# HKUST-Aerial-Robotics/MIND

Hardware: AMD Instinct MI355X
Metric: sim steps/sec (whole node) + scenario-tree nodes expanded/sec, AV2 demo scenes (higher is better)
Workload: dtype f32-class (bf16 hi+mid+lo split operands = 24 significand bits, six products, fp32 accumulate) pair kernel + ActorNet, f32 elsewhere in the predictor, f64 iLQR

## Files before the change

### include/mind_hip.h

```cpp
#ifndef MIND_HIP_H
#define MIND_HIP_H

#include <stddef.h>
#include <stdint.h>

#ifdef __cplusplus
extern "C" {
#endif

#define MIND_OK 0
#define MIND_EINVAL (-1)
#define MIND_ENOMEM (-2)
#define MIND_EHIP (-3)
#define MIND_ESTATE (-4)
#define MIND_ENOTFOUND (-5)

typedef struct mind_ctx mind_ctx;

int mind_ctx_create(int device, void *stream, mind_ctx **out);
int mind_ctx_destroy(mind_ctx *ctx);
const char *mind_last_error_string(mind_ctx *ctx);
int mind_ctx_synchronize(mind_ctx *ctx);

typedef struct {
  const char *name;
  const float *data;
  int64_t numel;
} mind_tensor_desc;

int mind_weights_load(mind_ctx *ctx, const mind_tensor_desc *tensors, int n_tensors);

typedef struct {
  int n_scenes;
  const int32_t *actor_off;
  const int32_t *lane_off;
  const float *actors;
  const float *lanes;
  const float *lane_feat;
  const float *actor_ctrs;
  const float *actor_vecs;
  const float *lane_ctrs;
  const float *lane_vecs;
  const float *const *rpe;
  const float *tgt_nodes;
  const float *tgt_rpe;
} mind_scene_batch;

typedef struct {
  float *cls;
  float *reg;
  float *vel;
  float *lane_feat;
  float *actor_emb;
  float *cls_emb;
} mind_pred_out;

int mind_predict_batch(mind_ctx *ctx, const mind_scene_batch *in, mind_pred_out *out);

typedef struct {
  float *cov_vel;
  float *param;
} mind_pred_aux;
int mind_predict_batch_aux(mind_ctx *ctx, const mind_scene_batch *in, mind_pred_out *out, const mind_pred_aux *aux);

#define MIND_BASIS_BEZIER 0
#define MIND_BASIS_MONOMIAL 1
int mind_set_decoder_basis(mind_ctx *ctx, int basis);
int mind_get_decoder_basis(mind_ctx *ctx);

#define MIND_CURVE_MAX_POINTS (1LL << 26)
int mind_curve_eval(mind_ctx *ctx, int basis, const float *param, long long n_rows, const double *tau, int n_tau,
                    float *reg, float *vel, float *cov_vel);
int mind_debug_curve_basis(int basis, const double *tau, int n_tau, float *T, float *Tp);

int mind_last_fusion_stats(mind_ctx *ctx, int *n_launches, float *total_ms, double *pairs_processed);
int mind_last_actor_stats(mind_ctx *ctx, int *layerwise, int *n_launches, int *n_chunks, float *total_ms);
int mind_last_token_stats(mind_ctx *ctx, int *layerwise, int *n_launches, int *n_chunks, float *total_ms);
int mind_last_token_stage_ms(mind_ctx *ctx, float *out_ms, int cap);
int mind_last_ilqr_stats(mind_ctx *ctx, float *kernel_ms, int *n_trees, int *workgroups_per_tree);
int mind_last_ilqr_profile(mind_ctx *ctx, double *out9);
int mind_last_ilqr_trace(mind_ctx *ctx, int tree, int phase, double *out, int cap_rows, int *n_rows);
int mind_set_profiling(mind_ctx *ctx, int enable);
int mind_debug_launch_times(mind_ctx *ctx, int kind, float *clock_ms, float *event_ms, int cap, int *n_clock, int *n_event);
int mind_debug_launch_clock(int n_blocks, int block_slots, int rate_khz, const long long *ops, int n_ops, const unsigned long long *stamps,
                            long long n_slots, double *out, int cap);

#define MIND_PAIR_F32 0
#define MIND_PAIR_BF16X3 1
#define MIND_PAIR_BF16 2
#define MIND_PAIR_BF16X6 3
int mind_set_pair_precision(mind_ctx *ctx, int mode);

int mind_set_tuning(mind_ctx *ctx, const char *name, int value);
int mind_get_tuning(mind_ctx *ctx, const char *name, int *value);
int mind_debug_tuning(int index, const char *name, const char *text, int value, const char **out_name, const char **out_env, int *out_value);
int mind_debug_live_handles(void);
int mind_get_pair_precision(mind_ctx *ctx);
int mind_debug_pack_bfrag(const float *w, int row_stride, uint32_t *out);

int mind_debug_pair_schedule(const int *scene_tokens, const int *scene_actors, int n_scenes, int n_cu, int last_layer, int *out_jobs, int cap,
                             int *out_info);

int mind_debug_predict_choice(const char *const *knob_names, const int *knob_values, int n_knobs, int pair_prec, int n_cu, int have_side,
                              const int *scene_actors, const int *scene_lanes, int n_scenes, long long *out, int cap);

int mind_debug_ilqr_plan(const char *const *knob_names, const int *knob_values, int n_knobs, int n_cu, int mode, int n_trees, const int *n_nodes,
                         const int32_t *parents, long long *out, int cap, int *bad);

int mind_debug_aime_book(int pred_len, int max_depth, int max_rounds, int n_agents, int world, int rank, int force, int n_rounds, const int *dec_len,
                         const float *dec, int n_tokens, int bytes_per_pair, int plan_chunk_mb, int per_scene, long long *out, int cap, char *msg,
                         int msg_cap);

int mind_debug_wait_word(const unsigned *word, unsigned want, double timeout_s, double (*clock)(void *user), void *user, int spins_per_look);

int mind_debug_actor_lw_plan(int n_actors, int np, int chunk, long long *out_launches, int cap, long long *out_info);

int mind_debug_token_lw_plan(int n_tokens, int mode, int chunk, long long *out_launches, int cap, long long *out_info);

int mind_debug_pack_conv_frag(const float *w, int co, int ci, int ksz, uint32_t *out, size_t cap);

int mind_debug_pack(const char *what, const float *w, int a, int b, int c, float *out, size_t cap);
int mind_debug_weight_image(const mind_tensor_desc *tensors, int n_tensors, float *blob, size_t blob_cap, char *names, size_t names_cap,
                            long long *entries, int entries_cap, long long *out_info, char *msg, int msg_cap);
int mind_debug_weight_bind(const mind_tensor_desc *tensors, int n_tensors, const char *drop, char *msg, int msg_cap);

int mind_debug_trig(mind_ctx *ctx, const double *x, int n, double *out);

int mind_debug_set_layers(mind_ctx *ctx, int n);
int64_t mind_debug_read(mind_ctx *ctx, const char *name, float *host, int64_t max_floats);

typedef struct {
  int n_nodes;
  const int32_t *parent;
  const float *prob;
  int n_agents;
  const float *agent_mean;
  const float *agent_cov;
  const double *field;
  const double *node_w;
} mind_cost_tree;

typedef struct {
  double dt, wheelbase;
  double w_des_state[6];
  double w_state_con[6];
  double state_lower[6], state_upper[6];
  double w_ctrl[2];
  double w_tgt, w_ego, w_ego_cov_offset, w_exo, w_exo_cov_offset, w_exo_cost_offset;
  double grid_res; int grid_w, grid_h;
  int max_iter;
} mind_ilqr_cfg;

typedef struct { int iterations; int converged; double J; double mu; } mind_ilqr_stats;

int mind_ilqr_solve_trees(mind_ctx *ctx, const mind_ilqr_cfg *cfg, const mind_cost_tree *trees,
                          int n_trees, const double *x0, const double *target_lane, int n_lane_pts,
                          double target_vel, int use_exo, const double *us_init, double *xs,
                          double *us, mind_ilqr_stats *stats);

int mind_ilqr_contingency(mind_ctx *ctx, const mind_ilqr_cfg *cfg_warm, const mind_ilqr_cfg *cfg_full,
                          const mind_cost_tree *trees, int n_trees, const double *x0,
                          const double *target_lane, int n_lane_pts, double target_vel, double *xs,
                          double *us, mind_ilqr_stats *stats_warm, mind_ilqr_stats *stats_full);
int mind_ilqr_contingency_begin(mind_ctx *ctx, const mind_ilqr_cfg *cfg_warm, const mind_ilqr_cfg *cfg_full,
                                const mind_cost_tree *trees, int n_trees, const double *x0,
                                const double *target_lane, int n_lane_pts, double target_vel, double *xs,
                                double *us, mind_ilqr_stats *stats_warm, mind_ilqr_stats *stats_full);
int mind_ilqr_contingency_begin_plan(mind_ctx *ctx, const mind_ilqr_cfg *cfg_warm, const mind_ilqr_cfg *cfg_full, const double *x0,
                                     const double *target_lane, int n_lane_pts, double target_vel, double *xs, double *us,
                                     mind_ilqr_stats *stats_warm, mind_ilqr_stats *stats_full);
int mind_ilqr_finish(mind_ctx *ctx);

typedef struct {
  int n_scenes;
  const int32_t *actor_off;
  const float *reg, *vel;
  const float *actor_ctrs, *actor_vecs;
  const float *rot, *orig;
  const float *cov_last;
  const int32_t *last;
  const float *target_lane;
  int n_lane_pts;
  const float *cls;
  const float *scen_prob;
  int lane_check;
  float dist_thres;
} mind_world_in;

typedef struct {
  float *world;
  float *topo;
  float *ego_end;
  float *sel, *sel_prob;
} mind_world_out;

int mind_aime_world(mind_ctx *ctx, const mind_world_in *in, const mind_world_out *out);

int mind_debug_aime_decide(mind_ctx *ctx, int n_scenes, const int32_t *actor_off, const int32_t *cmp, const float *cls, const float *scen_prob,
                           const float *topo, const float *ego_end, const float *world, int lane_check, float dist_thres, float prob_floor,
                           int fused, int by_value, float *sel, float *sel_prob, uint32_t *hit);

typedef struct {
  int n_scenes, n_agents, n_lanes;
  const float *pos, *ang, *vel;
  const float *types;
  const float *pad;
  const float *lane_ctrs, *lane_vecs;
  const float *target_lane;
  const float *target_lane_info;
  int n_lane_pts;
  float time_ahead, min_vel;
  const float *rows_dev;
  const int32_t *parent_slot;
  const int32_t *row0;
  const int32_t *dur;
  int prev_gen;
} mind_rebase_in;

typedef struct {
  float *actors;
  float *actor_ctrs, *actor_vecs;
  float *lane_ctrs, *lane_vecs;
  float *tgt_nodes, *tgt_rpe;
  float *frames;
  int32_t *gen;
} mind_rebase_out;

int mind_aime_rebase(mind_ctx *ctx, const mind_rebase_in *in, const mind_rebase_out *out);

typedef struct {
  int n_agents, n_lanes, n_lane_pts;
  const float *actors;
  const float *actor_ctrs, *actor_vecs;
  const float *lanes;
  const float *lane_ctrs, *lane_vecs;
  const float *tgt_nodes, *tgt_rpe;
  const float *rot, *orig, *tgt_pts;
  const float *hist;
  const float *types;
  const float *target_lane;
  const float *target_lane_info;
  float time_ahead, min_vel, dist_thres;
  int max_depth;
  int max_rounds;
  int pred_len;
  const float *raw_pos, *raw_ang, *raw_vel;
  const float *raw_pad;
  const double *lane_pts;
  const int32_t *lane_flags;
  float travel0;
  const float *script_cls, *script_reg, *script_vel;
  float prob_floor;
  const mind_ilqr_cfg *solve_cfg_warm, *solve_cfg_full;
  const double *solve_x0, *solve_lane;
  int solve_n_lane_pts;
  double solve_target_vel;
} mind_aime_plan_in;

#define MIND_AIME_BRANCH 1
#define MIND_AIME_END 2
#define MIND_AIME_TERMINATE 4
typedef struct {
  int round, scene, mode;
  int parent;
  float prob;
  int cur_t, end_t;
  int flags;
  int dur;
  int64_t row_off;
  float tgt_pts[22];
} mind_aime_node;

typedef struct {
  const mind_aime_node *nodes;
  int n_nodes;
  const float *rows;
  int64_t n_row_floats;
  int n_expanded, n_rounds;
  int root_flags;
// ... 235 lines not shown
```

### mind_amd/_lib.py

```python
import ctypes as C
import os

_HERE = os.path.dirname(os.path.abspath(__file__))
LIB_PATH = os.environ.get("MIND_HIP_LIB", os.path.join(_HERE, "libmind_hip.so"))

WAIT_CLOCK = C.CFUNCTYPE(C.c_double, C.c_void_p)
MIND_OK = 0
MIND_EINVAL, MIND_ENOMEM, MIND_EHIP, MIND_ESTATE, MIND_ENOTFOUND = -1, -2, -3, -4, -5


class TensorDesc(C.Structure):
    _fields_ = [("name", C.c_char_p), ("data", C.POINTER(C.c_float)), ("numel", C.c_int64)]


class SceneBatch(C.Structure):
    _fields_ = [("n_scenes", C.c_int), ("actor_off", C.POINTER(C.c_int32)), ("lane_off", C.POINTER(C.c_int32)),
                ("actors", C.c_void_p), ("lanes", C.c_void_p), ("lane_feat", C.c_void_p),
                ("actor_ctrs", C.c_void_p), ("actor_vecs", C.c_void_p), ("lane_ctrs", C.c_void_p),
                ("lane_vecs", C.c_void_p), ("rpe", C.POINTER(C.c_void_p)), ("tgt_nodes", C.c_void_p),
                ("tgt_rpe", C.c_void_p)]


class PredOut(C.Structure):
    _fields_ = [("cls", C.c_void_p), ("reg", C.c_void_p), ("vel", C.c_void_p), ("lane_feat", C.c_void_p),
# ... 48 lines not shown
class AuditRoadEpisodeOut(C.Structure):
    _fields_ = [("step_margin", C.POINTER(C.c_double)), ("step_corner", C.POINTER(C.c_int32)), ("step_ring", C.POINTER(C.c_int32)),
                ("step_edge", C.POINTER(C.c_int32)), ("ego_min", C.POINTER(C.c_double)), ("ego_step", C.POINTER(C.c_int32)),
                ("ego_corner", C.POINTER(C.c_int32)), ("ego_hits", C.POINTER(C.c_int32)), ("ego_first", C.POINTER(C.c_int32))]


class AuditTtcCfg(C.Structure):
    _fields_ = [("horizon", C.c_double), ("bound", C.c_double), ("lanes", C.c_int)]


class AuditTtcOut(C.Structure):
    _fields_ = [("step_ttc", C.POINTER(C.c_double)), ("step_track", C.POINTER(C.c_int32)), ("ego_min", C.POINTER(C.c_double)),
                ("ego_step", C.POINTER(C.c_int32)), ("ego_track", C.POINTER(C.c_int32)), ("ego_hits", C.POINTER(C.c_int32)),
                ("ego_first", C.POINTER(C.c_int32))]


class ForecastCfg(C.Structure):
    _fields_ = [("K", C.c_int), ("T", C.c_int), ("n_h", C.c_int), ("horizon", C.POINTER(C.c_int32)), ("miss_radius", C.c_double),
                ("disc_scale", C.c_double), ("disc_offset", C.c_double)]


FORECAST_OUT = (("ade", "f8", "a", True), ("fde", "f8", "a", True), ("cover", "i4", "a", True), ("first_out", "i4", "a", True),
                ("n_valid", "i4", "a", False), ("last", "i4", "a", False), ("k_ade", "i4", "a", False), ("k_fde", "i4", "a", False),
                ("brier_fde", "f8", "a", False), ("s_n_scored", "i4", "s", False), ("s_ade", "f8", "s", True), ("s_fde", "f8", "s", True),
                ("s_k_ade", "i4", "s", False), ("s_k_fde", "i4", "s", False), ("s_k_top", "i4", "s", False), ("s_brier_fde", "f8", "s", False),
                ("s_miss_rate", "f8", "s", False), ("s_miss_top", "f8", "s", False))


class ForecastOut(C.Structure):
    _fields_ = [(n, C.POINTER(C.c_double if dt == "f8" else C.c_int32)) for n, dt, _, _ in FORECAST_OUT]


class WorldIn(C.Structure):
    _fields_ = [("n_scenes", C.c_int), ("actor_off", C.POINTER(C.c_int32)), ("reg", C.c_void_p), ("vel", C.c_void_p),
                ("actor_ctrs", C.c_void_p), ("actor_vecs", C.c_void_p), ("rot", C.POINTER(C.c_float)),
                ("orig", C.POINTER(C.c_float)), ("cov_last", C.POINTER(C.c_float)), ("last", C.POINTER(C.c_int32)),
                ("target_lane", C.POINTER(C.c_float)), ("n_lane_pts", C.c_int), ("cls", C.c_void_p),
                ("scen_prob", C.POINTER(C.c_float)), ("lane_check", C.c_int), ("dist_thres", C.c_float)]


class WorldOut(C.Structure):
    _fields_ = [("world", C.c_void_p), ("topo", C.c_void_p), ("ego_end", C.c_void_p), ("sel", C.c_void_p), ("sel_prob", C.c_void_p)]


class RebaseIn(C.Structure):
    _fields_ = [("n_scenes", C.c_int), ("n_agents", C.c_int), ("n_lanes", C.c_int), ("pos", C.POINTER(C.c_float)),
                ("ang", C.POINTER(C.c_float)), ("vel", C.POINTER(C.c_float)), ("types", C.POINTER(C.c_float)),
                ("pad", C.POINTER(C.c_float)), ("lane_ctrs", C.POINTER(C.c_float)), ("lane_vecs", C.POINTER(C.c_float)),
                ("target_lane", C.POINTER(C.c_float)), ("target_lane_info", C.POINTER(C.c_float)), ("n_lane_pts", C.c_int),
                ("time_ahead", C.c_float), ("min_vel", C.c_float), ("rows_dev", C.c_void_p), ("parent_slot", C.POINTER(C.c_int32)),
                ("row0", C.POINTER(C.c_int32)), ("dur", C.POINTER(C.c_int32)), ("prev_gen", C.c_int)]


class RebaseOut(C.Structure):
    _fields_ = [("actors", C.c_void_p), ("actor_ctrs", C.c_void_p), ("actor_vecs", C.c_void_p), ("lane_ctrs", C.c_void_p),
                ("lane_vecs", C.c_void_p), ("tgt_nodes", C.c_void_p), ("tgt_rpe", C.c_void_p), ("frames", C.c_void_p),
                ("gen", C.POINTER(C.c_int32))]


class AimePlanIn(C.Structure):
    _fields_ = [("n_agents", C.c_int), ("n_lanes", C.c_int), ("n_lane_pts", C.c_int)] + \
               [(k, C.POINTER(C.c_float)) for k in ("actors", "actor_ctrs", "actor_vecs", "lanes", "lane_ctrs", "lane_vecs", "tgt_nodes", "tgt_rpe",
                                                    "rot", "orig", "tgt_pts", "hist", "types", "target_lane", "target_lane_info")] + \
               [("time_ahead", C.c_float), ("min_vel", C.c_float), ("dist_thres", C.c_float), ("max_depth", C.c_int), ("max_rounds", C.c_int), ("pred_len", C.c_int),
                ("raw_pos", C.POINTER(C.c_float)), ("raw_ang", C.POINTER(C.c_float)), ("raw_vel", C.POINTER(C.c_float)), ("raw_pad", C.POINTER(C.c_float)),
                ("lane_pts", C.POINTER(C.c_double)), ("lane_flags", C.POINTER(C.c_int32)), ("travel0", C.c_float),
                ("script_cls", C.c_void_p), ("script_reg", C.c_void_p), ("script_vel", C.c_void_p), ("prob_floor", C.c_float),
                ("solve_cfg_warm", C.c_void_p), ("solve_cfg_full", C.c_void_p), ("solve_x0", C.c_void_p), ("solve_lane", C.c_void_p),
                ("solve_n_lane_pts", C.c_int), ("solve_target_vel", C.c_double)]


class AimeNode(C.Structure):
    _fields_ = [("round", C.c_int), ("scene", C.c_int), ("mode", C.c_int), ("parent", C.c_int), ("prob", C.c_float),
                ("cur_t", C.c_int), ("end_t", C.c_int), ("flags", C.c_int), ("dur", C.c_int), ("row_off", C.c_int64),
                ("tgt_pts", C.c_float * 22)]


class AimePlanOut(C.Structure):
    _fields_ = [("nodes", C.POINTER(AimeNode)), ("n_nodes", C.c_int), ("rows", C.POINTER(C.c_float)), ("n_row_floats", C.c_int64),
                ("n_expanded", C.c_int), ("n_rounds", C.c_int), ("root_flags", C.c_int), ("round_scenes", C.c_int * 32),
                ("pair_ms", C.c_float), ("pair_launches", C.c_int), ("n_trees", C.c_int), ("tree_top", C.POINTER(C.c_int32)),
                ("tree_off", C.POINTER(C.c_int32)), ("flat_parent", C.POINTER(C.c_int32)), ("flat_prob", C.POINTER(C.c_float)),
                ("flat_mean", C.POINTER(C.c_float)), ("flat_cov", C.POINTER(C.c_float)), ("solves_begun", C.c_int)]


class IlqrCfg(C.Structure):
    _fields_ = [("dt", C.c_double), ("wheelbase", C.c_double), ("w_des_state", C.c_double * 6),
                ("w_state_con", C.c_double * 6), ("state_lower", C.c_double * 6), ("state_upper", C.c_double * 6),
                ("w_ctrl", C.c_double * 2), ("w_tgt", C.c_double), ("w_ego", C.c_double),
                ("w_ego_cov_offset", C.c_double), ("w_exo", C.c_double), ("w_exo_cov_offset", C.c_double),
                ("w_exo_cost_offset", C.c_double), ("grid_res", C.c_double), ("grid_w", C.c_int), ("grid_h", C.c_int),
                ("max_iter", C.c_int)]


class IlqrStats(C.Structure):
    _fields_ = [("iterations", C.c_int), ("converged", C.c_int), ("J", C.c_double), ("mu", C.c_double)]


LOOP_TAN_FN = C.CFUNCTYPE(C.c_double, C.c_double)
LOOP_SINCOS_FN = C.CFUNCTYPE(None, C.c_double, C.POINTER(C.c_double))


class LoopDesc(C.Structure):
    _fields_ = [("n_tracks", C.c_int), ("n_steps", C.c_int), ("clamp_last", C.c_int), ("ego_state", C.c_void_p), ("ego_state_is_f32", C.c_int), ("ego_obs", C.c_void_p), ("ego_trig32", C.c_void_p),
                ("tan_fn", C.c_void_p), ("sincos_fn", C.c_void_p), ("exo_obs", C.c_void_p),
                ("exo_valid", C.c_void_p), ("timestep", C.c_void_p), ("type_slot", C.c_void_p),
                ("sim_step", C.c_double), ("plan_step", C.c_double), ("enable_time", C.c_double),
                ("wheelbase", C.c_double), ("max_speed", C.c_double), ("max_steer", C.c_double), ("max_acc", C.c_double), ("max_dec", C.c_double),
                ("n_lanes", C.c_int), ("lane_pts", C.c_void_p), ("lane_flags", C.c_void_p),
                ("n_lane_pts", C.c_int), ("target_lane", C.c_void_p), ("target_lane_info", C.c_void_p),
                ("time_ahead", C.c_double), ("min_vel", C.c_float), ("dist_thres", C.c_float), ("max_depth", C.c_int), ("max_rounds", C.c_int),
                ("pred_len", C.c_int), ("prob_floor", C.c_float),
                ("cfg_warm", C.c_void_p), ("cfg_full", C.c_void_p), ("solve_n_lane_pts", C.c_int), ("solve_lane", C.c_void_p), ("target_vel", C.c_double),
                ("eval_n_lane_pts", C.c_int), ("eval_lane_is_f32", C.c_int), ("eval_lane", C.c_void_p), ("speculative", C.c_int)]


class LoopTotals(C.Structure):
    _fields_ = [("plans", C.c_longlong), ("expansions", C.c_longlong), ("scen_trees", C.c_longlong), ("rounds", C.c_longlong),
                ("aime_s", C.c_double), ("ilqr_s", C.c_double), ("total_s", C.c_double),
                ("iterations", C.c_longlong), ("node_iterations", C.c_longlong), ("node_iterations_exo", C.c_longlong),
                ("warm_speculated", C.c_longlong), ("warm_hits", C.c_longlong),
                ("pair_ms", C.c_double), ("pair_launches", C.c_longlong), ("scene_n2", C.c_double), ("scene_n_a1", C.c_double),
                ("ilqr_ms", C.c_double), ("ilqr_launches", C.c_longlong), ("ilqr_trees", C.c_longlong), ("ilqr_workgroups_per_tree", C.c_int),
                ("ilqr_prof", C.c_double * 9), ("ilqr_node_steps", C.c_double)]


class LoopOut(C.Structure):
    _fields_ = [("planned", C.c_int), ("enabled", C.c_int), ("n_steps", C.c_longlong), ("n_plans", C.c_longlong), ("episode_steps", C.c_longlong),
                ("sim_time", C.c_double), ("last_trigger", C.c_double), ("state", C.c_double * 4), ("ctrl", C.c_double * 2),
                ("n_agents", C.c_int), ("n_trees", C.c_int), ("best", C.c_int), ("n_expanded", C.c_int), ("n_rounds", C.c_int), ("n_traj_nodes", C.c_int),
                ("costs", C.POINTER(C.c_double)), ("aime_s", C.c_double), ("ilqr_s", C.c_double), ("total_s", C.c_double),
                ("tot", LoopTotals)]


PLANNER_EGO_KEY = -(1 << 63)


class PlannerDesc(C.Structure):
    _fields_ = [("time_ahead", C.c_double), ("min_vel", C.c_float), ("dist_thres", C.c_float), ("max_depth", C.c_int), ("max_rounds", C.c_int),
                ("pred_len", C.c_int), ("prob_floor", C.c_float), ("cfg_warm", C.c_void_p), ("cfg_full", C.c_void_p), ("speculative", C.c_int),
                ("ego_type_slot", C.c_int)]


class PlannerOut(C.Structure):
    _fields_ = [("n_plans", C.c_longlong),
                ("n_agents", C.c_int), ("n_trees", C.c_int), ("best", C.c_int), ("n_expanded", C.c_int), ("n_rounds", C.c_int), ("n_traj_nodes", C.c_int),
                ("costs", C.POINTER(C.c_double)), ("ctrl", C.c_double * 2), ("aime_s", C.c_double), ("ilqr_s", C.c_double), ("total_s", C.c_double),
                ("tot", LoopTotals)]


EXPORTS = ["mind_ctx_create", "mind_ctx_destroy", "mind_last_error_string", "mind_ctx_synchronize",
           "mind_weights_load", "mind_predict_batch", "mind_last_fusion_stats", "mind_last_actor_stats", "mind_debug_actor_lw_plan", "mind_last_token_stats", "mind_last_token_stage_ms", "mind_debug_token_lw_plan", "mind_set_profiling", "mind_debug_launch_times", "mind_debug_launch_clock",
           "mind_ilqr_solve_trees", "mind_ilqr_contingency", "mind_ilqr_solve_fields", "mind_cost_eval", "mind_ilqr_score_trees", "mind_ilqr_gains", "mind_ilqr_policy_rollouts", "mind_lane_dist_field", "mind_aime_world", "mind_aime_rebase", "mind_debug_aime_decide", "mind_debug_set_layers",
           "mind_debug_read", "mind_set_pair_precision", "mind_get_pair_precision", "mind_debug_pack_bfrag", "mind_debug_pack_conv_frag", "mind_debug_pack", "mind_debug_weight_image", "mind_debug_weight_bind", "mind_debug_pair_schedule", "mind_debug_predict_choice", "mind_debug_ilqr_plan", "mind_debug_aime_book", "mind_set_tuning", "mind_get_tuning", "mind_debug_tuning", "mind_debug_live_handles", "mind_last_ilqr_stats", "mind_aime_plan", "mind_last_ilqr_profile", "mind_eval_traj_trees", "mind_last_ilqr_trace", "mind_ilqr_contingency_begin", "mind_ilqr_finish", "mind_fill_tracks", "mind_ilqr_contingency_begin_plan", "mind_debug_trig", "mind_aime_plan_begin", "mind_aime_plan_poll", "mind_aime_plan_finish", "mind_ctx_busy", "mind_ilqr_finish_plan",
           "mind_set_exchange", "mind_last_exchange_stats", "mind_debug_wait_word",
           "mind_predict_batch_aux", "mind_set_decoder_basis", "mind_get_decoder_basis", "mind_curve_eval", "mind_debug_curve_basis",
           "mind_audit_plan", "mind_audit_episode", "mind_debug_box_clearance",
           "mind_forecast_score", "mind_debug_forecast_score",
           "mind_audit_road_plan", "mind_audit_road_episode", "mind_debug_road_margin",
           "mind_audit_ttc", "mind_debug_box_ttc",
           "mind_loop_create", "mind_loop_destroy", "mind_loop_reset", "mind_loop_advance", "mind_loop_state", "mind_loop_last_plan", "mind_loop_export",
           "mind_planner_create", "mind_planner_destroy", "mind_planner_reset", "mind_planner_observe", "mind_planner_set_lanes", "mind_planner_set_target_lane",
           "mind_planner_set_solve_lane", "mind_planner_set_eval_lane", "mind_planner_plan", "mind_planner_last_plan", "mind_planner_export"]

EXCHANGE_FN = C.CFUNCTYPE(C.c_int, C.c_void_p, C.c_int, C.c_void_p, C.c_void_p, C.c_int64)
XCHG_ALLGATHER, XCHG_ALLREDUCE, XCHG_ALLTOALLV = 0, 1, 2

_lib = None


def load():
    global _lib
    if _lib is not None:
        return _lib
    if not os.path.exists(LIB_PATH):
        raise ImportError(f"{LIB_PATH} is missing: the HIP extension must be built (hipcc --offload-arch=gfx950); "
                          "there is no CPU fallback for the product path")
    lib = C.CDLL(LIB_PATH)
    lib.mind_ctx_create.argtypes = [C.c_int, C.c_void_p, C.POINTER(C.c_void_p)]
    lib.mind_ctx_destroy.argtypes = [C.c_void_p]
    lib.mind_last_error_string.argtypes = [C.c_void_p]
    lib.mind_last_error_string.restype = C.c_char_p
    lib.mind_ctx_synchronize.argtypes = [C.c_void_p]
    lib.mind_weights_load.argtypes = [C.c_void_p, C.POINTER(TensorDesc), C.c_int]
    lib.mind_predict_batch.argtypes = [C.c_void_p, C.POINTER(SceneBatch), C.POINTER(PredOut)]
    lib.mind_predict_batch_aux.argtypes = [C.c_void_p, C.POINTER(SceneBatch), C.POINTER(PredOut), C.POINTER(PredAux)]
    lib.mind_set_decoder_basis.argtypes = [C.c_void_p, C.c_int]
    lib.mind_get_decoder_basis.argtypes = [C.c_void_p]
    lib.mind_curve_eval.argtypes = [C.c_void_p, C.c_int, C.c_void_p, C.c_longlong, C.POINTER(C.c_double), C.c_int, C.c_void_p, C.c_void_p, C.c_void_p]
    lib.mind_debug_curve_basis.argtypes = [C.c_int, C.POINTER(C.c_double), C.c_int, C.POINTER(C.c_float), C.POINTER(C.c_float)]
    lib.mind_last_fusion_stats.argtypes = [C.c_void_p, C.POINTER(C.c_int), C.POINTER(C.c_float), C.POINTER(C.c_double)]
    lib.mind_last_actor_stats.argtypes = [C.c_void_p, C.POINTER(C.c_int), C.POINTER(C.c_int), C.POINTER(C.c_int), C.POINTER(C.c_float)]
    lib.mind_debug_actor_lw_plan.argtypes = [C.c_int, C.c_int, C.c_int, C.POINTER(C.c_longlong), C.c_int, C.POINTER(C.c_longlong)]
    lib.mind_last_token_stats.argtypes = [C.c_void_p, C.POINTER(C.c_int), C.POINTER(C.c_int), C.POINTER(C.c_int), C.POINTER(C.c_float)]
    lib.mind_last_token_stage_ms.argtypes = [C.c_void_p, C.POINTER(C.c_float), C.c_int]
    lib.mind_debug_token_lw_plan.argtypes = [C.c_int, C.c_int, C.c_int, C.POINTER(C.c_longlong), C.c_int, C.POINTER(C.c_longlong)]
    lib.mind_set_profiling.argtypes = [C.c_void_p, C.c_int]
    lib.mind_debug_launch_times.argtypes = [C.c_void_p, C.c_int, C.POINTER(C.c_float), C.POINTER(C.c_float), C.c_int, C.POINTER(C.c_int), C.POINTER(C.c_int)]
    lib.mind_debug_launch_clock.argtypes = [C.c_int, C.c_int, C.c_int, C.POINTER(C.c_longlong), C.c_int, C.POINTER(C.c_ulonglong), C.c_longlong,
                                            C.POINTER(C.c_double), C.c_int]
    lib.mind_ilqr_solve_trees.argtypes = [C.c_void_p, C.POINTER(IlqrCfg), C.POINTER(CostTree), C.c_int,
                                          C.POINTER(C.c_double), C.POINTER(C.c_double), C.c_int, C.c_double, C.c_int,
                                          C.POINTER(C.c_double), C.POINTER(C.c_double), C.POINTER(C.c_double),
                                          C.POINTER(IlqrStats)]
    lib.mind_ilqr_contingency.argtypes = [C.c_void_p, C.POINTER(IlqrCfg), C.POINTER(IlqrCfg), C.POINTER(CostTree), C.c_int,
                                          C.POINTER(C.c_double), C.POINTER(C.c_double), C.c_int, C.c_double,
                                          C.POINTER(C.c_double), C.POINTER(C.c_double), C.POINTER(IlqrStats), C.POINTER(IlqrStats)]
    lib.mind_ilqr_contingency_begin.argtypes = [C.c_void_p, C.POINTER(IlqrCfg), C.POINTER(IlqrCfg), C.POINTER(CostTree), C.c_int,
                                          C.POINTER(C.c_double), C.POINTER(C.c_double), C.c_int, C.c_double,
                                          C.POINTER(C.c_double), C.POINTER(C.c_double), C.POINTER(IlqrStats), C.POINTER(IlqrStats)]
    lib.mind_ilqr_finish.argtypes = [C.c_void_p]
    lib.mind_ilqr_contingency_begin_plan.argtypes = [C.c_void_p, C.POINTER(IlqrCfg), C.POINTER(IlqrCfg), C.c_void_p, C.c_void_p, C.c_int, C.c_double,
                                                     C.c_void_p, C.c_void_p, C.c_void_p, C.c_void_p]
    lib.mind_fill_tracks.argtypes = [C.c_void_p, C.c_int, C.c_int, C.c_void_p, C.c_void_p, C.c_void_p, C.c_void_p, C.c_void_p, C.c_void_p]
    lib.mind_ilqr_solve_fields.argtypes = [C.c_void_p, C.POINTER(IlqrCfg), C.POINTER(FieldGrid), C.POINTER(CostTree), C.c_int,
                                           C.POINTER(C.c_double), C.POINTER(C.c_double), C.POINTER(C.c_double),
                                           C.POINTER(C.c_double), C.POINTER(IlqrStats)]
    lib.mind_cost_eval.argtypes = [C.c_void_p, C.POINTER(IlqrCfg), C.POINTER(FieldGrid), C.POINTER(CostTree),
                                   C.POINTER(C.c_double), C.POINTER(C.c_double), C.c_int, C.c_double, C.c_int, C.c_int,
                                   C.POINTER(C.c_int32), C.POINTER(C.c_double), C.POINTER(C.c_double), C.POINTER(C.c_double)]
    lib.mind_ilqr_score_trees.argtypes = [C.c_void_p, C.POINTER(IlqrCfg), C.POINTER(FieldGrid), C.POINTER(CostTree), C.c_int,
                                          C.POINTER(C.c_double), C.POINTER(C.c_double), C.c_int, C.c_double, C.c_int, C.c_int,
                                          C.POINTER(C.c_double), C.POINTER(C.c_double), C.POINTER(C.c_double), C.POINTER(C.c_double)]
    lib.mind_ilqr_gains.argtypes = [C.c_void_p, C.POINTER(IlqrCfg), C.POINTER(FieldGrid), C.POINTER(CostTree), C.c_int,
                                    C.POINTER(C.c_double), C.POINTER(C.c_double), C.c_int, C.c_double, C.c_int,
                                    C.POINTER(C.c_double), C.POINTER(C.c_double), C.POINTER(IlqrGainsOut)]
    lib.mind_ilqr_policy_rollouts.argtypes = [C.c_void_p, C.POINTER(IlqrCfg), C.POINTER(FieldGrid), C.POINTER(CostTree), C.c_int,
                                              C.POINTER(C.c_double), C.POINTER(C.c_double), C.c_int, C.c_double, C.c_int,
                                              C.POINTER(C.c_double), C.POINTER(C.c_double), C.POINTER(C.c_double), C.c_int,
                                              C.POINTER(C.c_double), C.POINTER(C.c_double), C.POINTER(C.c_double), C.POINTER(C.c_double),
                                              C.POINTER(C.c_double), C.POINTER(C.c_double)]
    lib.mind_lane_dist_field.argtypes = [C.c_void_p, C.POINTER(C.c_double), C.POINTER(C.c_double), C.c_int, C.c_int, C.c_int,
                                         C.c_double] + [C.POINTER(C.c_double)] * 4
    lib.mind_aime_world.argtypes = [C.c_void_p, C.POINTER(WorldIn), C.POINTER(WorldOut)]
    lib.mind_aime_rebase.argtypes = [C.c_void_p, C.POINTER(RebaseIn), C.POINTER(RebaseOut)]
    lib.mind_debug_aime_decide.argtypes = [C.c_void_p, C.c_int, C.POINTER(C.c_int32), C.POINTER(C.c_int32), C.c_void_p, C.POINTER(C.c_float), C.c_void_p,
                                           C.c_void_p, C.c_void_p, C.c_int, C.c_float, C.c_float, C.c_int, C.c_int, C.c_void_p, C.c_void_p, C.c_void_p]
    lib.mind_aime_plan.argtypes = [C.c_void_p, C.POINTER(AimePlanIn), C.POINTER(AimePlanOut)]
    lib.mind_aime_plan_begin.argtypes = [C.c_void_p, C.POINTER(AimePlanIn)]
    lib.mind_aime_plan_poll.argtypes = [C.c_void_p]
    lib.mind_aime_plan_finish.argtypes = [C.c_void_p, C.POINTER(AimePlanOut)]
    lib.mind_ctx_busy.argtypes = [C.c_void_p]
    lib.mind_ilqr_finish_plan.argtypes = [C.c_void_p, C.c_int, C.c_int, C.c_void_p, C.c_void_p, C.c_void_p, C.c_void_p]
    lib.mind_set_pair_precision.argtypes = [C.c_void_p, C.c_int]
    lib.mind_set_tuning.argtypes = [C.c_void_p, C.c_char_p, C.c_int]
    lib.mind_get_tuning.argtypes = [C.c_void_p, C.c_char_p, C.POINTER(C.c_int)]
    lib.mind_debug_tuning.argtypes = [C.c_int, C.c_char_p, C.c_char_p, C.c_int, C.POINTER(C.c_char_p), C.POINTER(C.c_char_p), C.POINTER(C.c_int)]
    lib.mind_debug_live_handles.argtypes = []
    lib.mind_last_ilqr_stats.argtypes = [C.c_void_p, C.POINTER(C.c_float), C.POINTER(C.c_int), C.POINTER(C.c_int)]
    lib.mind_last_ilqr_profile.argtypes = [C.c_void_p, C.POINTER(C.c_double)]
    lib.mind_last_ilqr_trace.argtypes = [C.c_void_p, C.c_int, C.c_int, C.POINTER(C.c_double), C.c_int, C.POINTER(C.c_int)]
    lib.mind_eval_traj_trees.argtypes = [C.POINTER(C.c_double), C.POINTER(C.c_double), C.POINTER(C.c_int32), C.c_int, C.c_void_p, C.c_int, C.c_int,
                                         C.c_double, C.POINTER(C.c_double)]
    lib.mind_get_pair_precision.argtypes = [C.c_void_p]
    lib.mind_debug_pack_bfrag.argtypes = [C.POINTER(C.c_float), C.c_int, C.POINTER(C.c_uint32)]
    lib.mind_debug_pair_schedule.argtypes = [C.POINTER(C.c_int), C.POINTER(C.c_int), C.c_int, C.c_int, C.c_int, C.POINTER(C.c_int), C.c_int, C.POINTER(C.c_int)]
    lib.mind_debug_predict_choice.argtypes = [C.POINTER(C.c_char_p), C.POINTER(C.c_int), C.c_int, C.c_int, C.c_int, C.c_int, C.POINTER(C.c_int), C.POINTER(C.c_int),
                                              C.c_int, C.POINTER(C.c_longlong), C.c_int]
    lib.mind_debug_ilqr_plan.argtypes = [C.POINTER(C.c_char_p), C.POINTER(C.c_int), C.c_int, C.c_int, C.c_int, C.c_int, C.POINTER(C.c_int), C.POINTER(C.c_int32),
                                         C.POINTER(C.c_longlong), C.c_int, C.POINTER(C.c_int)]
    lib.mind_debug_wait_word.argtypes = [C.POINTER(C.c_uint), C.c_uint, C.c_double, WAIT_CLOCK, C.c_void_p, C.c_int]
    lib.mind_debug_aime_book.argtypes = [C.c_int] * 8 + [C.POINTER(C.c_int), C.POINTER(C.c_float)] + [C.c_int] * 4 + [C.POINTER(C.c_longlong), C.c_int, C.c_char_p, C.c_int]
    lib.mind_debug_trig.argtypes = [C.c_void_p, C.POINTER(C.c_double), C.c_int, C.POINTER(C.c_double)]
    lib.mind_debug_pack_conv_frag.argtypes = [C.POINTER(C.c_float), C.c_int, C.c_int, C.c_int, C.POINTER(C.c_uint32), C.c_size_t]
    lib.mind_debug_pack.argtypes = [C.c_char_p, C.POINTER(C.c_float), C.c_int, C.c_int, C.c_int, C.POINTER(C.c_float), C.c_size_t]
    lib.mind_debug_weight_image.argtypes = [C.POINTER(TensorDesc), C.c_int, C.POINTER(C.c_float), C.c_size_t, C.c_char_p, C.c_size_t,
                                            C.POINTER(C.c_longlong), C.c_int, C.POINTER(C.c_longlong), C.c_char_p, C.c_int]
    lib.mind_debug_weight_bind.argtypes = [C.POINTER(TensorDesc), C.c_int, C.c_char_p, C.c_char_p, C.c_int]
    lib.mind_debug_set_layers.argtypes = [C.c_void_p, C.c_int]
    lib.mind_debug_read.argtypes = [C.c_void_p, C.c_char_p, C.POINTER(C.c_float), C.c_int64]
    lib.mind_set_exchange.argtypes = [C.c_void_p, C.c_int, C.c_int, EXCHANGE_FN, C.c_void_p, C.c_int]
    lib.mind_last_exchange_stats.argtypes = [C.c_void_p, C.POINTER(C.c_longlong), C.POINTER(C.c_longlong)]
    lib.mind_loop_create.argtypes = [C.c_void_p, C.POINTER(LoopDesc), C.POINTER(C.c_void_p)]
    lib.mind_loop_destroy.argtypes = [C.c_void_p]
    lib.mind_loop_reset.argtypes = [C.c_void_p]
    lib.mind_loop_advance.argtypes = [C.c_void_p, C.c_int, C.c_double, C.c_longlong, C.POINTER(LoopOut)]
    lib.mind_loop_state.argtypes = [C.c_void_p, C.POINTER(LoopOut)]
    lib.mind_loop_last_plan.argtypes = [C.c_void_p, C.POINTER(AimePlanOut)] + [C.POINTER(C.c_void_p)] * 6 + [C.c_void_p]
    lib.mind_loop_export.argtypes = [C.c_void_p, C.c_int, C.POINTER(C.c_int), C.c_void_p, C.c_void_p, C.c_void_p]
    lib.mind_planner_create.argtypes = [C.c_void_p, C.POINTER(PlannerDesc), C.POINTER(C.c_void_p)]
    lib.mind_planner_destroy.argtypes = [C.c_void_p]
    lib.mind_planner_reset.argtypes = [C.c_void_p]
    lib.mind_planner_observe.argtypes = [C.c_void_p, C.c_int, C.c_void_p, C.c_int, C.c_void_p, C.c_void_p, C.c_void_p]
    lib.mind_planner_set_lanes.argtypes = [C.c_void_p, C.c_int, C.c_void_p, C.c_void_p]
    lib.mind_planner_set_target_lane.argtypes = [C.c_void_p, C.c_int, C.c_void_p, C.c_void_p]
    lib.mind_planner_set_solve_lane.argtypes = [C.c_void_p, C.c_int, C.c_void_p, C.c_double]
    lib.mind_planner_set_eval_lane.argtypes = [C.c_void_p, C.c_int, C.c_void_p, C.c_int]
    lib.mind_planner_plan.argtypes = [C.c_void_p, C.c_void_p, C.c_void_p, C.POINTER(PlannerOut)]
    lib.mind_planner_last_plan.argtypes = [C.c_void_p, C.POINTER(AimePlanOut)] + [C.POINTER(C.c_void_p)] * 6 + [C.c_void_p]
    lib.mind_planner_export.argtypes = [C.c_void_p, C.c_int, C.POINTER(C.c_int), C.c_void_p, C.c_void_p, C.c_void_p]
    lib.mind_audit_plan.argtypes = [C.c_void_p, C.POINTER(AuditBox), C.c_double, C.POINTER(CostTree), C.c_int, C.c_int, C.POINTER(C.c_double),
                                    C.POINTER(AuditPlanOut)]
    lib.mind_audit_episode.argtypes = [C.c_void_p, C.POINTER(AuditBox), C.c_int, C.c_int, C.c_int, C.POINTER(C.c_double), C.POINTER(C.c_double),
                                       C.POINTER(C.c_uint8), C.POINTER(C.c_double), C.POINTER(AuditEpisodeOut)]
    lib.mind_debug_box_clearance.argtypes = [C.c_int, C.c_int, C.POINTER(C.c_double), C.POINTER(C.c_double), C.POINTER(C.c_double), C.POINTER(C.c_double)]
    fc_tail = [C.POINTER(ForecastCfg), C.c_int, C.POINTER(C.c_int32), C.c_void_p, C.c_void_p, C.POINTER(C.c_double), C.POINTER(C.c_uint8),
               C.POINTER(C.c_uint8), C.POINTER(ForecastOut)]
    lib.mind_forecast_score.argtypes = [C.c_void_p] + fc_tail
    lib.mind_debug_forecast_score.argtypes = fc_tail
    road = [C.POINTER(C.c_double), C.POINTER(C.c_int32), C.c_int]
    lib.mind_audit_road_plan.argtypes = [C.c_void_p, C.POINTER(AuditBox)] + road + [C.POINTER(CostTree), C.c_int, C.c_int, C.POINTER(C.c_double),
                                                                                   C.POINTER(AuditRoadPlanOut)]
    lib.mind_audit_road_episode.argtypes = [C.c_void_p, C.POINTER(AuditBox)] + road + [C.c_int, C.c_int, C.POINTER(C.c_double),
                                                                                      C.POINTER(AuditRoadEpisodeOut)]
    lib.mind_debug_road_margin.argtypes = [C.c_int, C.POINTER(C.c_double), C.POINTER(AuditBox)] + road + [C.POINTER(C.c_double), C.POINTER(C.c_double)] + \
        [C.POINTER(C.c_int32)] * 3
    lib.mind_audit_ttc.argtypes = [C.c_void_p, C.POINTER(AuditBox), C.POINTER(AuditTtcCfg), C.c_int, C.c_int, C.c_int, C.POINTER(C.c_double),
                                   C.POINTER(C.c_double), C.POINTER(C.c_uint8), C.POINTER(C.c_double), C.POINTER(AuditTtcOut)]
    lib.mind_debug_box_ttc.argtypes = [C.c_int, C.POINTER(C.c_double), C.POINTER(C.c_double), C.POINTER(C.c_double), C.POINTER(C.c_double)]
    for n in EXPORTS:
        getattr(lib, n)
        if n not in ("mind_last_error_string", "mind_debug_read"):
            getattr(lib, n).restype = C.c_int
    lib.mind_debug_read.restype = C.c_int64
    _lib = lib
    return lib


PRED_CHOICE_FIELDS = ("header", "n_runs", "np", "actor_form", "actor_arg", "actor_grid", "actor_chunk", "actor_chunks", "actor_launches", "qsplit", "qk_stride",
                      "tiled", "edge_bf16", "edge_pair_bytes", "tok_chunk", "tok_lw", "tok_chunks", "pair_family", "pair_np", "l5_jobs5", "xcd_lanes",
                      "xcd_lanes5", "dec_actor", "dec_np", "fp32_dec", "split_dec", "want_mw", "mw_blocks", "cls_on_side", "tgt_wait_first",
                      "dec_head_ra")
PAIR_PREC = ("f32", "bf16x3", "bf16", "bf16x6")


def predict_choice(knobs, prec, scenes, n_cu=256, have_side=True):
    lib = load()
    names = (C.c_char_p * max(1, len(knobs)))(*[k.encode() for k in knobs])
    vals = (C.c_int * max(1, len(knobs)))(*[int(v) for v in knobs.values()])
    sa = (C.c_int * len(scenes))(*[a for a, _ in scenes])
    sl = (C.c_int * len(scenes))(*[l for _, l in scenes])
    cap = 32 + 6 * len(scenes)
    out = (C.c_longlong * cap)()
    n = lib.mind_debug_predict_choice(names, vals, len(knobs), PAIR_PREC.index(prec) if isinstance(prec, str) else prec, n_cu, int(have_side),
                                      sa, sl, len(scenes), out, cap)
    if n == MIND_EINVAL:
        return None
    assert 0 < n <= cap and out[0] == 32 and n == 32 + 6 * out[1], n
    d = dict(zip(PRED_CHOICE_FIELDS, out[:31]))
    d["runs"] = [tuple(out[32 + 6 * i:38 + 6 * i]) for i in range(out[1])]
    return d


def knobs():
    lib = load()
    name, env, val = C.c_char_p(), C.c_char_p(), C.c_int()
    rows = []
    while not rows or len(rows) < n:
        n = lib.mind_debug_tuning(len(rows), None, None, 0, C.byref(name), C.byref(env), C.byref(val))
        assert n > 0, n
        rows.append((name.value.decode(), env.value.decode() if env.value else None, val.value))
    return rows


def knob_stored(name, value=None, text=None):
    val = C.c_int()
    rc = load().mind_debug_tuning(-1, name.encode(), None if text is None else text.encode(), 0 if value is None else int(value), None, None, C.byref(val))
    return val.value if rc == MIND_OK else None


ILQR_PLAN_FIELDS = ("header", "n_trees", "form", "G", "GS", "spec", "nslot", "grid", "workgroups_per_tree", "host_out", "early", "starve_followers")
ILQR_TREE_FIELDS = ("M", "nl", "nseg", "nsl", "maxls", "nfs")
ILQR_TREE_TABLES = ("level_start", "level_nodes", "child_start", "child_list", "seg_start", "seg_nodes", "slevel_start", "slevel_segs", "seg_rec",
                    "fstep_start", "fstep_items", "fstep_q1", "fstep_nstart", "fstep_nodes")


def ilqr_plan(knobs, parents, n_cu=256, generic=False, evaluate=False, two_fits=False):
    lib = load()
    names = (C.c_char_p * max(1, len(knobs)))(*[k.encode() for k in knobs])
    vals = (C.c_int * max(1, len(knobs)))(*[int(v) for v in knobs.values()])
    nn = (C.c_int * len(parents))(*[len(p) for p in parents])
    flat = [int(v) for p in parents for v in p]
    par = (C.c_int32 * max(1, len(flat)))(*flat)
    bad = (C.c_int * 2)()
    mode = int(generic) | int(evaluate) << 1 | int(two_fits) << 2
    n = lib.mind_debug_ilqr_plan(names, vals, len(knobs), n_cu, mode, len(parents), nn, par, None, 0, bad)
    if n == MIND_EINVAL:
        return {"bad": (bad[0], bad[1])} if bad[0] >= 0 else None
    out = (C.c_longlong * n)()
    assert lib.mind_debug_ilqr_plan(names, vals, len(knobs), n_cu, mode, len(parents), nn, par, out, n, bad) == n and out[0] == 16
    d = dict(zip(ILQR_PLAN_FIELDS, out[:12]))
    d["trees"], o = [], 16
    for _ in parents:
        tr = dict(zip(ILQR_TREE_FIELDS, out[o:o + 6]))
        lens, o = out[o + 6:o + 20], o + 20
        for name, ln in zip(ILQR_TREE_TABLES, lens):
            tr[name], o = list(out[o:o + ln]), o + ln
        d["trees"].append(tr)
    assert o == n
    return d


AIME_ROUND_FIELDS = ("B", "lo", "hi", "Bmax", "chunk", "S", "s0", "Sm", "any")
AIME_NODE_FIELDS = ("round", "scene", "mode", "parent", "prob", "cur_t", "end_t", "flags", "dur", "row_off", "owner", "lscene")


def aime_book(pred_len, max_depth, n_agents, rounds, world=1, rank=0, force=False, max_rounds=32, n_tokens=0, bytes_per_pair=512, plan_chunk_mb=96 * 1024,
              per_scene=1):
    import numpy as np
    lib = load()
    arrs = [np.ascontiguousarray(r, np.float32).ravel() for r in rounds]
    lens = (C.c_int * max(1, len(arrs)))(*[a.size for a in arrs])
    dec = np.concatenate(arrs + [np.zeros(1, np.float32)])
    msg = C.create_string_buffer(256)
    args = [pred_len, max_depth, max_rounds, n_agents, world, rank, int(force), len(arrs), lens, dec.ctypes.data_as(C.POINTER(C.c_float)), n_tokens,
            bytes_per_pair, plan_chunk_mb, per_scene]
    n = lib.mind_debug_aime_book(*args, None, 0, msg, 256)
    if n == MIND_EINVAL:
        return None
    out = (C.c_longlong * n)()
    assert lib.mind_debug_aime_book(*args, out, n, msg, 256) == n and out[0] == 16
    o, take = [16], lambda k: (list(out[o[0]:o[0] + k]), o.__setitem__(0, o[0] + k))[0]
    d = dict(code=out[1], error=msg.value.decode() if out[1] else None, args=(out[2], out[3]), n_rows=out[8], root_flags=out[9], rounds=[])
    for _ in range(out[4]):
        r = dict(zip(AIME_ROUND_FIELDS, take(9)))
        for k, ln in (("todo", r["S"]), ("cnt_r", world), ("s0_r", world + 1), ("win", 3 * r["Sm"]), ("tab", 2 * world), ("snd", 2 * world), ("rcv", 2 * world)):
            r[k] = take(ln)
        d["rounds"].append(r)
    if not out[1]:
        d["nodes"] = [dict(zip(AIME_NODE_FIELDS, take(12))) for _ in range(out[5])]
        for name in ("gather", "flat"):
            nj, nb, nbytes = take(3)
            d[name] = dict(jobs=[tuple(take(5)) for _ in range(nj)], job_of_block=take(nb), agent_of_block=take(nb), bytes=nbytes)
        d["tree_top"], d["tree_off"], d["flat_parent"], d["flat_prob"] = take(out[6]), take(out[6] + 1), take(out[7]), take(out[7])
    assert o[0] == n
    return d


def tensor_descs(sd):
    import numpy as np
    descs = (TensorDesc * max(1, len(sd)))()
    keep = []
    for i, (k, v) in enumerate(sd.items()):
        a = np.ascontiguousarray(v.detach().cpu().numpy() if hasattr(v, "detach") else np.asarray(v), dtype=np.float32)
        keep.append(a)
        descs[i].name = k.encode()
        descs[i].data = a.ctypes.data_as(C.POINTER(C.c_float))
        descs[i].numel = a.size
    return descs, keep


def weight_image(sd):
    import numpy as np
    lib = load()
    descs, keep = tensor_descs(sd)
    msg = C.create_string_buffer(256)
    info = (C.c_longlong * 3)()
    rc = lib.mind_debug_weight_image(descs, len(sd), None, 0, None, 0, None, 0, info, msg, 256)
    if rc == MIND_ENOTFOUND:
        raise KeyError(msg.value.decode())
    assert rc == MIND_OK, rc
    ne, nf, nb = info
    blob, names, ents = np.zeros(nf, np.float32), C.create_string_buffer(nb), (C.c_longlong * (2 * ne))()
    assert lib.mind_debug_weight_image(descs, len(sd), blob.ctypes.data_as(C.POINTER(C.c_float)), nf, names, nb, ents, ne, info, msg, 256) == MIND_OK
    keys = names.value.decode().split("\n")[:-1]
    assert len(keys) == ne
    return blob, [(k, ents[2 * i], ents[2 * i + 1]) for i, k in enumerate(keys)]


def curve_basis(basis, tau):
    import numpy as np
    lib = load()
    tau = np.ascontiguousarray(tau, np.float64).ravel()
    b = BASIS.index(basis) if isinstance(basis, str) else int(basis)
    T, Tp = np.zeros((max(1, tau.size), 8), np.float32), np.zeros((max(1, tau.size), 7), np.float32)
    rc = lib.mind_debug_curve_basis(b, tau.ctypes.data_as(C.POINTER(C.c_double)), tau.size, T.ctypes.data_as(C.POINTER(C.c_float)),
                                    Tp.ctypes.data_as(C.POINTER(C.c_float)))
    if rc == MIND_EINVAL:
        raise ValueError(f"mind_debug_curve_basis rejects basis {basis!r}, tau {tau!r}")
    assert rc == MIND_OK, rc
    return T[:tau.size], Tp[:tau.size]


def weight_bind(sd, drop=None):
    lib = load()
    descs, keep = tensor_descs(sd)
    msg = C.create_string_buffer(256)
    rc = lib.mind_debug_weight_bind(descs, len(sd), drop.encode() if drop else None, msg, 256)
    assert rc in (MIND_OK, MIND_ENOTFOUND), rc
    return None if rc == MIND_OK else msg.value.decode()


def pack(what, w, a=0, b=0, c=0, cap=1 << 20):
    import numpy as np
    lib = load()
    w = np.ascontiguousarray(w, np.float32)
    out = np.zeros(cap, np.float32)
    n = lib.mind_debug_pack(what.encode(), w.ctypes.data_as(C.POINTER(C.c_float)), a, b, c, out.ctypes.data_as(C.POINTER(C.c_float)), cap)
    assert n > 0, (what, n)
    return out[:n].copy()


def box_clearance(kind, a, b, trig=None):
    import numpy as np
# ... 139 lines not shown
```

### mind_amd/csrc/encdec_kernels.hip

```cpp
#include <hip/hip_runtime.h>
#include <stdint.h>

#include "weight_tables.h"
#include "dec_curve.h"
#include "launch_clock.h"

typedef float f32x4 __attribute__((ext_vector_type(4)));

#define NT 256

__device__ __forceinline__ float wave_sum(float v) {
  v += __shfl_xor(v, 32, 64);
  v += __shfl_xor(v, 16, 64);
  v += __shfl_xor(v, 8, 64);
  v += __shfl_xor(v, 4, 64);
  v += __shfl_xor(v, 2, 64);
  v += __shfl_xor(v, 1, 64);
  return v;
}

__device__ __forceinline__ float block_sum(float v, float *red) {
  v = wave_sum(v);
  __syncthreads();
  if ((threadIdx.x & 63) == 0) red[threadIdx.x >> 6] = v;
  __syncthreads();
  return red[0] + red[1] + red[2] + red[3];
}

#ifndef DB
#define DB 16
#endif
#define DENSE_ROW_FENCE() __builtin_amdgcn_sched_barrier(0)
#define DBQ 8
template <int R>
__device__ __forceinline__ void dense_quads(const float *in, int ldi, int K, const float *__restrict__ WT,
                                            const float *__restrict__ b, int NOUT, float *out, int ldo,
                                            float *part, int part_floats) {
  const int nthr = blockDim.x;
  const int NQ = NOUT >> 2;
  int KP = 1;
  while (KP * 2 * NQ <= nthr && KP * 2 * R * NOUT <= part_floats && KP * 2 <= (K >> 2)) KP *= 2;
  const int Kc = ((K / 4 + KP - 1) / KP) * 4;
  for (int item = threadIdx.x; item < KP * NQ; item += nthr) {
    const int kp = item / NQ, o = (item % NQ) * 4;
    float acc[R][4];
#pragma unroll
    for (int r = 0; r < R; ++r)
#pragma unroll
      for (int c = 0; c < 4; ++c) acc[r][c] = (KP == 1 && b) ? b[o + c] : 0.f;
    const int k0 = kp * Kc, k1 = min(K, k0 + Kc);
    int k = k0;
    for (; k + DBQ <= k1; k += DBQ) {
      f32x4 w[DBQ];
#pragma unroll
      for (int q = 0; q < DBQ; ++q) w[q] = *(const f32x4 *)(WT + (size_t)(k + q) * NOUT + o);
#pragma unroll
      for (int r = 0; r < R; ++r) {
#pragma unroll
        for (int q4 = 0; q4 < DBQ / 4; ++q4) {
          const f32x4 x = *(const f32x4 *)(in + r * ldi + k + 4 * q4);
#pragma unroll
          for (int j = 0; j < 4; ++j)
#pragma unroll
            for (int c = 0; c < 4; ++c) acc[r][c] = fmaf(w[4 * q4 + j][c], x[j], acc[r][c]);
        }
        DENSE_ROW_FENCE();
      }
    }
    for (; k < k1; k += 4) {
#pragma unroll
      for (int j = 0; j < 4; ++j) {
        const f32x4 w = *(const f32x4 *)(WT + (size_t)(k + j) * NOUT + o);
#pragma unroll
        for (int r = 0; r < R; ++r) {
          const float x = in[r * ldi + k + j];
#pragma unroll
          for (int c = 0; c < 4; ++c) acc[r][c] = fmaf(w[c], x, acc[r][c]);
        }
      }
    }
#pragma unroll
    for (int r = 0; r < R; ++r)
#pragma unroll
      for (int c = 0; c < 4; ++c) {
        if (KP == 1) out[r * ldo + o + c] = acc[r][c];
        else part[(kp * R + r) * NOUT + o + c] = acc[r][c];
      }
  }
  if (KP == 1) return;
  __syncthreads();
  for (int i = threadIdx.x; i < R * NOUT; i += nthr) {
    const int r = i / NOUT, oo = i % NOUT;
    float v = b ? b[oo] : 0.f;
    for (int q = 0; q < KP; ++q) v += part[(q * R + r) * NOUT + oo];
    out[r * ldo + oo] = v;
  }
}

#ifndef DT
#define DT 1024
#endif
template <int R>
__device__ __forceinline__ void dense_quads_part(const float *in, int ldi, int K, const float *__restrict__ WT, const float *__restrict__ b, int NOUT,
                                                 float *out, int ldo, float *part, int part_floats, int wg, int G) {
  const int nthr = blockDim.x;
  const int NQ = NOUT >> 2;
  int KP = 1;
  while (KP * 2 * NQ <= DT && KP * 2 * R * NOUT <= part_floats && KP * 2 <= (K >> 2)) KP *= 2;
  const int Kc = ((K / 4 + KP - 1) / KP) * 4;
  const int q_lo = NQ * wg / G, q_hi = NQ * (wg + 1) / G, NQg = q_hi - q_lo;
  for (int item = threadIdx.x; item < KP * NQg; item += nthr) {
    const int kp = item / NQg, o = (q_lo + item % NQg) * 4;
    float acc[R][4];
#pragma unroll
    for (int r = 0; r < R; ++r)
#pragma unroll
      for (int c = 0; c < 4; ++c) acc[r][c] = (KP == 1 && b) ? b[o + c] : 0.f;
    const int k0 = kp * Kc, k1 = min(K, k0 + Kc);
    int k = k0;
    for (; k + DBQ <= k1; k += DBQ) {
      f32x4 w[DBQ];
#pragma unroll
      for (int q = 0; q < DBQ; ++q) w[q] = *(const f32x4 *)(WT + (size_t)(k + q) * NOUT + o);
#pragma unroll
      for (int r = 0; r < R; ++r) {
#pragma unroll
        for (int q4 = 0; q4 < DBQ / 4; ++q4) {
          const f32x4 x = *(const f32x4 *)(in + r * ldi + k + 4 * q4);
#pragma unroll
          for (int j = 0; j < 4; ++j)
#pragma unroll
            for (int c = 0; c < 4; ++c) acc[r][c] = fmaf(w[4 * q4 + j][c], x[j], acc[r][c]);
        }
        DENSE_ROW_FENCE();
      }
    }
    for (; k < k1; k += 4) {
#pragma unroll
      for (int j = 0; j < 4; ++j) {
        const f32x4 w = *(const f32x4 *)(WT + (size_t)(k + j) * NOUT + o);
#pragma unroll
        for (int r = 0; r < R; ++r) {
          const float x = in[r * ldi + k + j];
#pragma unroll
          for (int c = 0; c < 4; ++c) acc[r][c] = fmaf(w[c], x, acc[r][c]);
        }
      }
    }
#pragma unroll
    for (int r = 0; r < R; ++r)
#pragma unroll
      for (int c = 0; c < 4; ++c) {
        if (KP == 1) out[r * ldo + o + c] = acc[r][c];
        else part[(kp * R + r) * NOUT + o + c] = acc[r][c];
      }
  }
  if (KP == 1) return;
  __syncthreads();
// ... 404 lines not shown
__device__ __forceinline__ float block_sum_a(float v, float *red, int flip) {
  v = wave_sum(v);
  float *r = red + (flip & 1) * 16;
  if ((threadIdx.x & 63) == 0) r[threadIdx.x >> 6] = v;
  __syncthreads();
  float s = 0.f;
#pragma unroll
  for (int w = 0; w < AT / 64; ++w) s += r[w];
  return s;
}

#define GN_NE 6
__device__ __forceinline__ void gn(float *buf, int C, int T, const float *__restrict__ g,
                                   const float *__restrict__ b, const float *resid, bool relu, float *red) {
  const int n = C * T;
  float x[GN_NE], gg[GN_NE], bb[GN_NE];
  float s = 0.f;
#pragma unroll
  for (int e = 0; e < GN_NE; ++e) {
    const int i = threadIdx.x + e * AT;
    if (i < n) {
      const int c = i / T;
      x[e] = buf[i];
      gg[e] = g[c];
      bb[e] = b[c];
      s += x[e];
    }
  }
  const float mean = block_sum_a(s, red, 0) / (float)n;
  float v = 0.f;
#pragma unroll
  for (int e = 0; e < GN_NE; ++e)
    if ((int)threadIdx.x + e * AT < n) { const float d = x[e] - mean; v = fmaf(d, d, v); }
  const float rstd = 1.0f / sqrtf(block_sum_a(v, red, 1) / (float)n + 1e-5f);
#pragma unroll
  for (int e = 0; e < GN_NE; ++e) {
    const int i = threadIdx.x + e * AT;
    if (i < n) {
      float y = (x[e] - mean) * rstd * gg[e] + bb[e];
      if (resid) y += resid[i];
      if (relu) y = fmaxf(y, 0.f);
      buf[i] = y;
    }
  }
  __syncthreads();
}

__device__ __forceinline__ void res1d(const float *in, int Cin, int Tin, const ResW &w, int Cout, int stride,
                                      float *out, float *t1, float *t2, float *red, float *part, int pf) {
  const int Tout = Tin / stride;
  if (stride == 1) conv<1, 3>(in, Cin, Tin, w.c1, Cout, Tout, t1, part, pf);
  else conv<2, 3>(in, Cin, Tin, w.c1, Cout, Tout, t1, part, pf);
  __syncthreads();
  gn(t1, Cout, Tout, w.g1, w.b1, nullptr, true, red);
  conv<1, 3>(t1, Cout, Tout, w.c2, Cout, Tout, out, part, pf);
  __syncthreads();
  const float *resid = in;
  if (w.ds) {
    if (stride == 1) conv<1, 1>(in, Cin, Tin, w.ds, Cout, Tout, t2, part, pf);
    else conv<2, 1>(in, Cin, Tin, w.ds, Cout, Tout, t2, part, pf);
    __syncthreads();
      gn(t2, Cout, Tout, w.gd, w.bd, nullptr, false, red);
      resid = t2;
  }
  gn(out, Cout, Tout, w.g2, w.b2, resid, true, red);
}

#define ACT_PART 12288
#define ACT_LDS_FLOATS (672 + 7 * 1536 + 2 * 6144 + 32 + ACT_PART)
__global__ __launch_bounds__(AT) void k_actor_net(const float *__restrict__ actors, int n_actors,
                                                  float *__restrict__ out, ActorW W, LcSlot *clk) {
  lc_stamp_in(clk);
  extern __shared__ float sm[];
  float *xin = sm;
  float *o0 = sm + 672, *o1 = o0 + 1536, *o2 = o1 + 1536, *o3 = o2 + 1536;
  float *ta = o3 + 1536, *tb = ta + 1536, *tc = tb + 1536;
  float *fa = tc + 1536, *fb = fa + 6144;
  float *red = fb + 6144;
  float *part = red + 32;
  const int pf = ACT_PART;
  float *fo = o0;
  const int tid = threadIdx.x;
  const int a = blockIdx.x;
  if (a >= n_actors) { lc_stamp_both(clk); return; }
#ifdef MIND_ENC_TRACE
  long long at_[12], aq_ = clock64();
  int an_ = 0;
#define AT_MARK() do { const long long n_ = clock64(); at_[an_++] = n_ - aq_; aq_ = n_; } while (0)
#else
#define AT_MARK() do {} while (0)
#endif
  for (int i = tid; i < 14 * 48; i += AT) xin[i] = actors[(size_t)a * 14 * 48 + i];
  __syncthreads();
  AT_MARK();
  res1d(xin, 14, 48, W.res[0], 32, 1, ta, tb, tc, red, part, pf);
  res1d(ta, 32, 48, W.res[1], 32, 1, o0, tb, tc, red, part, pf);
  AT_MARK();
  res1d(o0, 32, 48, W.res[2], 64, 2, ta, tb, tc, red, part, pf);
  res1d(ta, 64, 24, W.res[3], 64, 1, o1, tb, tc, red, part, pf);
  AT_MARK();
  res1d(o1, 64, 24, W.res[4], 128, 2, ta, tb, tc, red, part, pf);
  res1d(ta, 128, 12, W.res[5], 128, 1, o2, tb, tc, red, part, pf);
  AT_MARK();
  res1d(o2, 128, 12, W.res[6], 256, 2, ta, tb, tc, red, part, pf);
  res1d(ta, 256, 6, W.res[7], 256, 1, o3, tb, tc, red, part, pf);
  AT_MARK();
  conv<1, 3>(o3, 256, 6, W.latW[3], 128, 6, fa, part, pf);
  __syncthreads();
  gn(fa, 128, 6, W.latG[3], W.latB[3], nullptr, false, red);
  float *cur = fa, *nxt = fb;
  for (int g = 2; g >= 0; --g) {
    const float *src_o = g == 2 ? o2 : (g == 1 ? o1 : o0);
    const int C = g == 2 ? 128 : (g == 1 ? 64 : 32);
    const int T = g == 2 ? 12 : (g == 1 ? 24 : 48);
    const int Th = T / 2;
    conv<1, 3>(src_o, C, T, W.latW[g], 128, T, nxt, part, pf);
    __syncthreads();
    gn(nxt, 128, T, W.latG[g], W.latB[g], nullptr, false, red);
    for (int i = tid; i < 128 * T; i += AT) {
      const int c = i / T, t = i % T;
      float src = (t + 0.5f) * 0.5f - 0.5f;
      src = src < 0.f ? 0.f : src;
      const int i0 = (int)src;
      const int i1 = i0 + 1 < Th ? i0 + 1 : Th - 1;
      const float l1 = src - (float)i0;
      nxt[i] += (1.0f - l1) * cur[c * Th + i0] + l1 * cur[c * Th + i1];
    }
    __syncthreads();
    float *t = cur; cur = nxt; nxt = t;
  }
  AT_MARK();
  {
    const ResW &w = W.res[8];
    conv<1, 3>(cur, 128, 48, w.c1, 128, 48, nxt, part, pf);
    __syncthreads();
    gn(nxt, 128, 48, w.g1, w.b1, nullptr, true, red);
    conv<1, 3>(nxt, 128, 48, w.c2, 128, 48, fo, part, pf);
    __syncthreads();
    gn(fo, 128, 48, w.g2, w.b2, cur, true, red);
  }
  AT_MARK();
  if (tid < 128) out[(size_t)a * 128 + tid] = fo[tid * 48 + 47];
#ifdef MIND_ENC_TRACE
  if (a == 0 && tid == 0)
    printf("[k_actor_net n=%d] cycles: load %lld group0 %lld group1 %lld group2 %lld group3 %lld fpn %lld out-res %lld\n", n_actors, at_[0], at_[1], at_[2],
           at_[3], at_[4], at_[5], at_[6]);
#endif
  lc_stamp_out(clk);
}
extern "C" size_t mind_actor_lds_bytes() { return (size_t)ACT_LDS_FLOATS * sizeof(float); }

#define DEC_SCENE_PART 24576
#define DEC_SCENE_LDS_FLOATS (256 + 768 + 768 + 2304 + 768 + 9216 + 768 + 144 + DEC_SCENE_PART)
__global__ __launch_bounds__(DT) void k_dec_tgt(const float *__restrict__ tgt_feat , const float *__restrict__ tgt_rpe ,
                                                float *__restrict__ tgt_out , DecW W) {
  extern __shared__ __attribute__((aligned(16))) float dsm[];
  float (*v0)[256] = (float (*)[256])(dsm);
  float (*v1)[768] = (float (*)[768])(dsm + 256);
  float *part = dsm + 14992;
  const int PF = DEC_SCENE_PART;
  const int tid = threadIdx.x;
  const int b = blockIdx.x;
  if (tid < 20) v1[0][tid] = tgt_rpe[(size_t)b * 20 + tid];
  __syncthreads();
  dense<1>(&v1[0][0], 768, 20, W.rpeW, W.rpeb, 128, &v0[0][128], 256, part, PF);
  if (tid < 128) v0[0][tid] = tgt_feat[(size_t)b * 128 + tid];
  __syncthreads();
  ln_rows(&v0[0][128], 256, 1, 128, W.rpeg, W.rpebe, true);
  __syncthreads();
  dense<1>(&v0[0][0], 256, 256, W.t0W, W.t0b, 128, &v1[0][0], 768, part, PF);
  __syncthreads();
  ln_rows(&v1[0][0], 768, 1, 128, W.t0g, W.t0be, true);
  __syncthreads();
  dense<1>(&v1[0][0], 768, 128, W.t3W, W.t3b, 128, &v0[0][0], 256, part, PF);
  __syncthreads();
  ln_rows(&v0[0][0], 256, 1, 128, W.t3g, W.t3be, true);
  __syncthreads();
  if (tid < 128) tgt_out[(size_t)b * 128 + tid] = v0[0][tid];
}

#ifdef MIND_DEC_TRACE
__device__ long long dec_tr_[64];
__device__ int dec_trn_;
#define DEC_MARK() do { if (blockIdx.x == 0 && threadIdx.x == 0) { dec_tr_[dec_trn_ & 63] = clock64(); ++dec_trn_; } } while (0)
#else
#define DEC_MARK() do {} while (0)
#endif
template <bool MW, int PART = 0>
__device__ __forceinline__ void k_dec_scene_body(const float *__restrict__ x ,
                                                 const int *__restrict__ cls_row ,
                                                 float *__restrict__ Cout ,
                                                 float *__restrict__ cls_out , const DecW &W, int b, int wg, int G,
                                                 float *xbuf, unsigned *bar, unsigned *abort_word) {
  extern __shared__ __attribute__((aligned(16))) float dsm[];
  float (*v0)[256] = (float (*)[256])(dsm);
  float (*v1)[768] = (float (*)[768])(dsm + 256);
  float (*C)[128] = (float (*)[128])(dsm + 1024);
  float (*qkv)[384] = (float (*)[384])(dsm + 1792);
  float (*att)[128] = (float (*)[128])(dsm + 4096);
  float (*ff)[1536] = (float (*)[1536])(dsm + 4864);
  float (*t2)[128] = (float (*)[128])(dsm + 14080);
  float (*sc)[6][6] = (float (*)[6][6])(dsm + 14848);
  float *part = dsm + 14992;
  const int PF = DEC_SCENE_PART;
  const int tid = threadIdx.x;
  int xstage = 0;
  float *xb0 = xbuf, *xb1 = xbuf + 6 * 1536;
#ifdef MIND_DEC_TRACE
  if (blockIdx.x == 0 && tid == 0) dec_trn_ = 0;
#endif
  DEC_MARK();
  if (PART == 2) {
    for (int i = tid; i < 768; i += blockDim.x) C[i / 128][i % 128] = Cout[(size_t)b * 768 + i];
    __syncthreads();
  }
  if (PART != 2) {
  if (tid < 128) v0[0][tid] = x[(size_t)cls_row[b] * 128 + tid];
  __syncthreads();
  dense<1>(&v0[0][0], 256, 128, W.c0W, W.c0b, 384, &v1[0][0], 768, part, PF);
  DEC_MARK();
  __syncthreads();
  ln_rows(&v1[0][0], 768, 1, 384, W.c0g, W.c0be, true);
  DEC_MARK();
  __syncthreads();
  if (MW) {
    dense_quads_part<1>(&v1[0][0], 768, 384, W.c3W, W.c3b, 768, &ff[0][0], 1536, part, PF, wg, G);
    if (dec_exchange<1>(&ff[0][0], 1536, 768, wg, G, (xstage++ & 1) ? xb1 : xb0, bar, abort_word)) return;
  } else
    dense<1>(&v1[0][0], 768, 384, W.c3W, W.c3b, 768, &ff[0][0], 1536, part, PF);
  DEC_MARK();
  __syncthreads();
  ln_rows(&ff[0][0], 1536, 1, 768, W.c3g, W.c3be, true);
  DEC_MARK();
  __syncthreads();
  for (int i = tid; i < 768; i += blockDim.x) C[i / 128][i % 128] = ff[0][i];
  __syncthreads();
  for (int L = 0; L < 2; ++L) {
    dense<6>(&C[0][0], 128, 128, W.inW[L], W.inb[L], 384, &qkv[0][0], 384, part, PF);
  DEC_MARK();
    __syncthreads();
    if (tid < 4 * 36) {
      const int hd = tid / 36, s = (tid % 36) / 6, t = tid % 6;
      float d = 0.f;
      for (int k = 0; k < 32; ++k) d = fmaf(qkv[s][hd * 32 + k], qkv[t][128 + hd * 32 + k], d);
      sc[hd][s][t] = d / sqrtf(32.0f);
    }
    __syncthreads();
    if (tid < 24) {
      const int hd = tid / 6, s = tid % 6;
      float m = -INFINITY;
      for (int t = 0; t < 6; ++t) m = fmaxf(m, sc[hd][s][t]);
      float e[6], sum = 0.f;
      for (int t = 0; t < 6; ++t) { e[t] = expf(sc[hd][s][t] - m); sum += e[t]; }
      for (int t = 0; t < 6; ++t) sc[hd][s][t] = e[t] / sum;
    }
    __syncthreads();
    for (int i = tid; i < 6 * 128; i += blockDim.x) {
      const int s = i / 128, c = i % 128, hd = c / 32;
      float o = 0.f;
      for (int t = 0; t < 6; ++t) o = fmaf(sc[hd][s][t], qkv[t][256 + c], o);
      att[s][c] = o;
    }
    __syncthreads();
    dense<6>(&att[0][0], 128, 128, W.outW[L], W.outb[L], 128, &t2[0][0], 128, part, PF);
  DEC_MARK();
    __syncthreads();
    for (int i = tid; i < 768; i += blockDim.x) C[i / 128][i % 128] += t2[i / 128][i % 128];
    __syncthreads();
    ln_rows(&C[0][0], 128, 6, 128, W.n1g[L], W.n1b[L], false);
  DEC_MARK();
    __syncthreads();
    if (MW) {
      dense_quads_part<6>(&C[0][0], 128, 128, W.l1W[L], W.l1b[L], 1536, &ff[0][0], 1536, part, PF, wg, G);
      if (dec_exchange<6>(&ff[0][0], 1536, 1536, wg, G, (xstage++ & 1) ? xb1 : xb0, bar, abort_word)) return;
    } else
      dense<6>(&C[0][0], 128, 128, W.l1W[L], W.l1b[L], 1536, &ff[0][0], 1536, part, PF);
  DEC_MARK();
    __syncthreads();
    for (int i = tid; i < 6 * 1536; i += blockDim.x) ff[i / 1536][i % 1536] = fmaxf(ff[i / 1536][i % 1536], 0.f);
    __syncthreads();
    if (MW) {
      dense_quads_part<6>(&ff[0][0], 1536, 1536, W.l2W[L], W.l2b[L], 128, &t2[0][0], 128, part, PF, wg, G);
      if (dec_exchange<6>(&t2[0][0], 128, 128, wg, G, (xstage++ & 1) ? xb1 : xb0, bar, abort_word)) return;
    } else
      dense<6>(&ff[0][0], 1536, 1536, W.l2W[L], W.l2b[L], 128, &t2[0][0], 128, part, PF);
  DEC_MARK();
    __syncthreads();
    for (int i = tid; i < 768; i += blockDim.x) C[i / 128][i % 128] += t2[i / 128][i % 128];
    __syncthreads();
    ln_rows(&C[0][0], 128, 6, 128, W.n2g[L], W.n2b[L], false);
  DEC_MARK();
    __syncthreads();
  }
  if (!MW || wg == 0)
    for (int i = tid; i < 768; i += blockDim.x) Cout[(size_t)b * 768 + i] = C[i / 128][i % 128];
  }
  if (PART == 1) return;
  dense<6>(&C[0][0], 128, 128, W.k0W, W.k0b, 128, &att[0][0], 128, part, PF);
  DEC_MARK();
  __syncthreads();
  ln_rows(&att[0][0], 128, 6, 128, W.k0g, W.k0be, true);
  DEC_MARK();
  __syncthreads();
  dense<6>(&att[0][0], 128, 128, W.k3W, W.k3b, 128, &t2[0][0], 128, part, PF);
  DEC_MARK();
  __syncthreads();
  ln_rows(&t2[0][0], 128, 6, 128, W.k3g, W.k3be, true);
  DEC_MARK();
  __syncthreads();
  for (int k = tid >> 6; k < 6; k += (int)(blockDim.x >> 6)) {
    const int lane = tid & 63;
    float s = t2[k][lane] * W.k6W[lane] + t2[k][lane + 64] * W.k6W[lane + 64];
    s = wave_sum(s);
    if (lane == 0) sc[0][0][k] = s + W.k6b[0];
  }
  __syncthreads();
  if (tid == 0 && (!MW || wg == 0)) {
    float m = -INFINITY;
    for (int k = 0; k < 6; ++k) m = fmaxf(m, sc[0][0][k]);
    float e[6], sum = 0.f;
    for (int k = 0; k < 6; ++k) { e[k] = expf(sc[0][0][k] - m); sum += e[k]; }
    for (int k = 0; k < 6; ++k) cls_out[(size_t)b * 6 + k] = e[k] / sum;
  }
  DEC_MARK();
#ifdef MIND_DEC_TRACE
  if (blockIdx.x == 0 && tid == 0) {
    printf("[k_dec_scene] cycles between marks (dense / LayerNorm stages in program order):");
    for (int q = 1; q < dec_trn_ && q < 64; ++q) printf(" %lld", dec_tr_[q] - dec_tr_[q - 1]);
    printf("\n");
  }
#endif
}

__global__ __launch_bounds__(DT) void k_dec_scene(const float *__restrict__ x, const int *__restrict__ cls_row, float *__restrict__ Cout,
                                                  float *__restrict__ cls_out, DecW W) {
  k_dec_scene_body<false>(x, cls_row, Cout, cls_out, W, (int)blockIdx.x, 0, 1, nullptr, nullptr, nullptr);
}
__global__ __launch_bounds__(DT) void k_dec_scene_c(const float *__restrict__ x, const int *__restrict__ cls_row, float *__restrict__ Cout, DecW W) {
  k_dec_scene_body<false, 1>(x, cls_row, Cout, nullptr, W, (int)blockIdx.x, 0, 1, nullptr, nullptr, nullptr);
}
__global__ __launch_bounds__(DT) void k_dec_cls(float *__restrict__ Cout, float *__restrict__ cls_out, DecW W) {
  k_dec_scene_body<false, 2>(nullptr, nullptr, Cout, cls_out, W, (int)blockIdx.x, 0, 1, nullptr, nullptr, nullptr);
}
#define DEC_MW_G 8
__global__ __launch_bounds__(DT) void k_dec_scene_mw(const float *__restrict__ x, const int *__restrict__ cls_row, float *__restrict__ Cout,
                                                     float *__restrict__ cls_out, DecW W, int n_scenes, float *__restrict__ xbuf,
                                                     unsigned *__restrict__ bars, unsigned *abort_word) {
  const int r = (int)blockIdx.x % (8 * DEC_MW_G);
  const int b = 8 * ((int)blockIdx.x / (8 * DEC_MW_G)) + (r & 7), wg = r >> 3;
  if (b >= n_scenes) return;
  k_dec_scene_body<true>(x, cls_row, Cout, cls_out, W, b, wg, DEC_MW_G, xbuf + (size_t)b * 2 * 6 * 1536, bars + 4 * (size_t)b, abort_word);
}

#define RA 4
#define DEC_ACTOR_LDS_FLOATS (512 + 1536 + 3072 + 3072 + 3072 + 960 + 6144)
template <int PART, int RAT = RA>
__global__ __launch_bounds__(DT) void k_dec_actor(const float *__restrict__ x ,
                                                  const int *__restrict__ actor_row ,
                                                  const int *__restrict__ actor_scene , int n_actors,
                                                  const float *__restrict__ Cmode ,
                                                  const float *__restrict__ tgt ,
                                                  float *__restrict__ reg, float *__restrict__ vel, DecW W, float *__restrict__ h2g,
                                                  float *__restrict__ cov_vel , float *__restrict__ param ) {
  extern __shared__ __attribute__((aligned(16))) float dsm[];
  float (*xin)[128] = (float (*)[128])(dsm);
  float (*h1)[384] = (float (*)[384])(dsm + 512);
  float (*h2)[768] = (float (*)[768])(dsm + 2048);
  float (*E)[128] = (float (*)[128])(dsm + 5120);
  float (*t1)[128] = (float (*)[128])(dsm + 8192);
  float (*prm)[40] = (float (*)[40])(dsm + 11264);
  float *part = dsm + 12224;
  const int PF = 6144;
  static_assert(RAT == RA || (PART == 2 && (RAT == 1 || RAT == 2)), "only the head runs with fewer agents per workgroup");
  constexpr int HEAD_KP = dense_scalar_kp(RA * 6, 128, 128, DT, 6144);
  const int tid = threadIdx.x;
  const int a0 = blockIdx.x * RAT;
  if (PART != 2) {
    for (int i = tid; i < RAT * 128; i += blockDim.x) {
      const int r = i / 128, a = a0 + r;
      xin[r][i % 128] = a < n_actors ? x[(size_t)actor_row[a] * 128 + i % 128] : 0.f;
    }
    __syncthreads();
    dense<RAT>(&xin[0][0], 128, 128, W.a0W, W.a0b, 384, &h1[0][0], 384, part, PF);
    __syncthreads();
    ln_rows(&h1[0][0], 384, RAT, 384, W.a0g, W.a0be, true);
    __syncthreads();
    dense<RAT>(&h1[0][0], 384, 384, W.a3W, W.a3b, 768, &h2[0][0], 768, part, PF);
    __syncthreads();
    ln_rows(&h2[0][0], 768, RAT, 768, W.a3g, W.a3be, true);
    __syncthreads();
    if (PART == 1) {
      for (int i = tid; i < RAT * 768; i += blockDim.x) {
        const int r = i / 768, a = a0 + r;
        if (a < n_actors) h2g[(size_t)a * 768 + i % 768] = h2[r][i % 768];
      }
      return;
    }
  } else {
    for (int i = tid; i < RAT * 768; i += blockDim.x) {
      const int r = i / 768, a = a0 + r;
      h2[r][i % 768] = a < n_actors ? h2g[(size_t)a * 768 + i % 768] : 0.f;
    }
    __syncthreads();
  }
  for (int i = tid; i < RAT * 768; i += blockDim.x) {
    const int r = i / 768, k = (i % 768) / 128, c = i % 128;
    const int a = a0 + r;
    float v = 0.f;
    if (a < n_actors) {
      const int sc = actor_scene[a];
      v = h2[r][k * 128 + c] + Cmode[((size_t)sc * 6 + k) * 128 + c];
      if (k == 0) v += tgt[(size_t)sc * 128 + c];
    }
    E[r * 6 + k][c] = v;
  }
  __syncthreads();
  if (RAT == RA) dense<RA * 6>(&E[0][0], 128, 128, W.r0W, W.r0b, 128, &t1[0][0], 128, part, PF);
  else dense_ksplit<RAT * 6, RAT + 1>(&E[0][0], 128, 128, W.r0W, W.r0b, 128, &t1[0][0], 128, part, HEAD_KP);
  __syncthreads();
  ln_rows(&t1[0][0], 128, RAT * 6, 128, W.r0g, W.r0be, true);
  __syncthreads();
  if (RAT == RA) dense<RA * 6>(&t1[0][0], 128, 128, W.r3W, W.r3b, 128, &E[0][0], 128, part, PF);
  else dense_ksplit<RAT * 6, RAT + 1>(&t1[0][0], 128, 128, W.r3W, W.r3b, 128, &E[0][0], 128, part, HEAD_KP);
  __syncthreads();
  ln_rows(&E[0][0], 128, RAT * 6, 128, W.r3g, W.r3be, true);
  __syncthreads();
  for (int i = tid; i < RAT * 6 * 40; i += blockDim.x) {
    const int r = i / 40, o = i % 40;
    float acc = W.r6b[o];
    for (int k = 0; k < 128; ++k) acc = fmaf(W.r6W[k * 40 + o], E[r][k], acc);
    prm[r][o] = acc;
  }
  __syncthreads();
  if (param)
    for (int i = tid; i < RAT * 6 * 40; i += blockDim.x) {
      const int r = i / 40, a = a0 + r / 6;
      if (a < n_actors) param[((size_t)a * 6 + r % 6) * 40 + i % 40] = prm[r][i % 40];
    }
  for (int i = tid; i < RAT * 6 * 60; i += blockDim.x) {
    const int r = i / 60, t = i % 60;
    const int a = a0 + r / 6, k = r % 6;
    if (a >= n_actors) continue;
    const size_t o = ((size_t)a * 6 + k) * 60 + t;
    dec_curve_point(&prm[r][0], W.T + t * 8, W.Tp + t * 7, W.monomial, reg + o * 5, vel + o * 2, cov_vel ? cov_vel + o * 3 : nullptr);
  }
}

extern "C" size_t mind_dec_scene_lds_bytes() { return (size_t)DEC_SCENE_LDS_FLOATS * sizeof(float); }
extern "C" size_t mind_dec_actor_lds_bytes() { return (size_t)DEC_ACTOR_LDS_FLOATS * sizeof(float); }
```

### mind_amd/csrc/mind_hip.hip

```cpp
#include <hip/hip_runtime.h>

#include <cmath>
#include <cstdarg>
#include <cstdio>
#include <cstdlib>
#include <algorithm>
#include <cstring>
#include <map>
#include <memory>
#include <string>
#include <thread>
#include <atomic>
#include <functional>
#include <vector>

#include "../../include/mind_hip.h"
#include "encdec_kernels.hip"
#include "fusion_kernels.hip"
#include "pair_bf16_kernels.hip"
#include "pair_tile_kernels.hip"
#include "pair_tile6_kernels.hip"
#include "token_mfma_kernels.hip"
#include "actor_mfma_kernels.hip"
#include "actor_lw_kernels.hip"
#include "token_lw_kernels.hip"
#include "actor_f32_kernels.hip"
#include "dec_mfma_kernels.hip"
#include "dec_curve_kernels.hip"
#include "ilqr_kernels.hip"
#include "ilqr_score_kernels.hip"
#include "ilqr_policy_kernels.hip"
#include "audit_kernels.hip"
#include "forecast_kernels.hip"
#include "road_kernels.hip"
#include "ttc_kernels.hip"
#include "pair_jobs.h"
#include "pred_choice.h"
#include "ilqr_choice.h"
#include "aime_book.h"
#include "audit_arena.h"
#include "weight_pack.h"
#include "aime_kernels.hip"

static_assert(TN_RA == RA && TN_IL_SLOTS == IL_SLOTS, "tuning.h restates the two kernel constants its clamps need");

static std::atomic<long> live_handles{0};

template <class H, hipError_t (*Release)(H)> struct Owned {
  H p = nullptr;
  size_t cap = 0;
  Owned() = default;
  Owned(Owned &&o) noexcept : p(o.p), cap(o.cap) { o.p = nullptr; o.cap = 0; }
  Owned &operator=(Owned &&o) noexcept { if (this != &o) { reset(); p = o.p; cap = o.cap; o.p = nullptr; o.cap = 0; } return *this; }
  ~Owned() { reset(); }
  operator H() const { return p; }
  template <class T> T *as() const { return (T *)p; }
  void reset() {
    if (p) { (void)Release(p); live_handles.fetch_sub(1, std::memory_order_relaxed); }
    p = nullptr; cap = 0;
  }
  hipError_t took(hipError_t e, size_t bytes = 0) {
    if (e == hipSuccess) { live_handles.fetch_add(1, std::memory_order_relaxed); cap = bytes; } else p = nullptr;
    return e;
  }
};
struct Event : Owned<hipEvent_t, hipEventDestroy> { hipError_t create(unsigned flags = hipEventDefault) { reset(); return took(hipEventCreateWithFlags(&p, flags)); } };
struct Stream : Owned<hipStream_t, hipStreamDestroy> { hipError_t create() { reset(); return took(hipStreamCreateWithFlags(&p, hipStreamNonBlocking)); } };
struct Pinned : Owned<void *, hipHostFree> {
  hipError_t alloc(size_t bytes, unsigned flags = hipHostMallocDefault) { reset(); return took(hipHostMalloc(&p, bytes, flags), bytes); }
};
struct DevBuf : Owned<void *, hipFree> {
  hipError_t alloc(size_t bytes) { reset(); return took(hipMalloc(&p, bytes), bytes); }
};

struct TableSet {
  std::vector<int> key;
  DevBuf meta, jobs, jobs5, rows;
  std::vector<int> actor_row, cls_row, scene_n;
  long long edge_pairs = 0, edge_pairs_t = 0, stamp = 0;
  int ntok = 0, slot = 0, njobs = 0, njobs5 = 0;
  double pairs_full = 0, pairs_l5 = 0;
};
#define MIND_TABLE_SETS 8

struct mind_ctx {
  int device = 0;
  hipStream_t stream = nullptr;
  Stream side;
  Event ev_side, ev_main, ev_stage, ev_tgt, ev_cls;
  std::vector<char> aime_stage;
  bool aime_stage_busy = false;
  std::string err;
  DevBuf wdev;
  bool have_weights = false;
  WeightTables W = {};
  PredTuning pt; IlqrTuning it; CtxTuning ct;
  TnRefs knobs() { return {&pt, &it, &ct}; }
  int dec_basis = MIND_BASIS_BEZIER;
  DevBuf curve_tab;
  std::vector<double> curve_tau;
  int curve_tab_basis = -1;
  DevBuf tok_lw_arena;
  std::vector<TlLaunch> tok_lw_plan;
  int last_tok_lw = 0, last_tok_launches = 0, last_tok_chunks = 0;
  float tok_ms = 0.f, tok_stage_ms[TL_NSTAGE + 1] = {};
  std::vector<Event> ev_tok;
  std::vector<int> ev_tok_tag;
  TableSet tabs[MIND_TABLE_SETS];
  long long tab_clock = 0;
  long long n_table_hits = 0;
  unsigned dec_gen = 0;
  DevBuf pl_cnt;
  std::function<int(hipStream_t)> enc_pre, enc_post;
  std::vector<IlTables> il_tab;
  struct IlImage { std::vector<double> hD; std::vector<float> hF; std::vector<int> hI; } il_img;
  struct IlEarly { const double *xs = nullptr, *us = nullptr; volatile unsigned *done = nullptr; unsigned gen = 0; int n_trees = 0; long nodes = 0; } il_early;
  unsigned il_gen = 0;
  long long il_spec_req = 0, il_spec_hit = 0;
  DevBuf actor_lw_arena;
  std::vector<LwLaunch> actor_lw_plan;
  int last_actor_lw = 0, last_actor_launches = 0, last_actor_chunks = 0;
  float actor_ms = 0.f;
  Event ev_act0, ev_act1;
  int pair_prec = 3;
  std::vector<int> last_scene_n;
  bool last_edge_tiled = false, last_edge_bf16 = false;
  DevBuf edge, x, ST, QK, part, tokpos, meta, jobs, actor_feat, lane_feat, tgt_feat, cmode, tgt_emb,
      rows, rpe_ptrs;
  DevBuf ilqr_dev, aime_dev, rebase_dev2[2], dec_h2;
  DevBuf audit_dev;
  DevBuf pl_root, pl_in[2], pl_lf, pl_lrep, pl_pred, pl_small, pl_tab[2], pl_win[2];
  std::vector<DevBuf> pl_world;
  Pinned pl_pin[8];
  Event ev_pl, ev_tab, ev_root;
  DevBuf il_field;
  Pinned il_field_pin;
  Event ev_field;
  bool il_field_valid = false;
  double il_field_key[5] = {0, 0, 0, 0, 0};
  std::vector<double> il_field_lane;
  int xr = 0, xw = 1;
  mind_exchange_fn xfn = nullptr;
  void *xuser = nullptr;
  bool xforce = false;
  DevBuf x_send, x_recv, x_seg;
  long long x_collectives = 0, x_bytes = 0;
  Stream pl_copy;
  std::vector<double> pl_sol_xs, pl_sol_us;
  std::vector<mind_ilqr_stats> pl_sol_stw, pl_sol_stf;
  std::thread pa_thread;
  std::atomic<int> pa_state{0};
  mind_aime_plan_in pa_in;
  mind_aime_plan_out pa_out;
  int pa_rc = 0;
  struct Plan {
    AimeBook book;
    int agents = 0;
    long long gen = 0;
    const float *rows_p = nullptr, *fmean_p = nullptr, *fcov_p = nullptr;
    const float *dev_fmean = nullptr, *dev_fcov = nullptr;
  } plan;
  DevBuf pl_flat;
  DevBuf dec_xbuf, dec_bars;
  Pinned dec_abort;
  int rb_cur = 0, rb_gen = 0;
  size_t rb_S = 0, rb_a = 0;
  bool profiling = false;
  Event ev_il0, ev_il1;
  float ilqr_ms = 0.f;
  int ilqr_multi = 0, ilqr_trees = 0;
  std::function<int()> il_finish;
  bool il_finish_owned = false;
  Event ev_rows;
  std::vector<const double *> il_trace_dev;
  std::vector<int> il_trace_its;
  int il_trace_cap = 0, il_trace_phases = 0;
  double il_prof[9] = {0, 0, 0, 0, 0, 0, 0, 0, 0};
  long long n_ilqr_fallbacks = 0;
  int n_pair_launch = 0;
  float pair_ms = 0.f;
  double pairs_done = 0.0;
  std::vector<Event> ev;
  bool ev_defer = false;
  std::vector<Event> ev_pool;
  size_t ev_pool_used = 0;
  std::vector<size_t> ev_pending;
  int wall_khz = 0;
  LcRing lc;
  DevBuf lc_dev;
  Pinned lc_host;
  double lc_carry_ms[LC_KINDS] = {0, 0, 0};
  int lc_carry_n[LC_KINDS] = {0, 0, 0};
  std::vector<float> lc_last[LC_KINDS], ev_last[LC_KINDS];
  int n_cu = 256;
  int debug_layers = 6;
  int last_ntok = 0;
  size_t il_dbg[6] = {0, 0, 0, 0, 0, 0};
  long long last_edge_pairs = 0;
  int last_slots = 0, last_A = 0, last_B = 0;
};

static int fail(mind_ctx *c, int code, const char *fmt, ...) {
  char buf[512];
  va_list ap;
  va_start(ap, fmt);
  vsnprintf(buf, sizeof(buf), fmt, ap);
  va_end(ap);
  if (c) c->err = buf;
  return code;
}

#define HIPCHK(c, call)                                                                        \
  do {                                                                                         \
    hipError_t e_ = (call);                                                                    \
    if (e_ != hipSuccess)                                                                      \
      return fail(c, MIND_EHIP, "%s failed: %s (%s:%d)", #call, hipGetErrorString(e_), __FILE__, __LINE__); \
  } while (0)

static int ensure(mind_ctx *c, DevBuf &b, size_t bytes) {
  if (bytes <= b.cap) return MIND_OK;
  b.reset();
  const size_t want = bytes < ((size_t)64 << 20) ? std::max<size_t>(2 * bytes, (size_t)1 << 20) : bytes + bytes / 4 + 4096;
  if (b.alloc(want) != hipSuccess) {
    const hipError_t e = b.alloc(bytes);
    if (e != hipSuccess) return fail(c, MIND_ENOMEM, "hipMalloc(%zu) failed: %s", bytes, hipGetErrorString(e));
  }
  return MIND_OK;
}

static int ensure_exact(mind_ctx *c, DevBuf &b, size_t bytes, const char *what) {
  if (bytes <= b.cap) return MIND_OK;
  HIPCHK(c, hipStreamSynchronize(c->stream));
  if (b.alloc(bytes) != hipSuccess) return fail(c, MIND_ENOMEM, "hipMalloc(%zu) for %s failed", bytes, what);
  return MIND_OK;
}

struct KernelLds {
  const void *kernel; size_t bytes;
  template <class K> KernelLds(K *k, size_t b) : kernel((const void *)k), bytes(b) {}
};
static void set_kernel_attributes() {
  const size_t pair = mind_pair_lds_bytes(), pair_bf = mind_pair_bf_lds_bytes(), actor_m = mind_actor_mfma_lds_bytes(), dec_m = mind_dec_actor_mfma_lds_bytes(),
               il = il_lds_bytes(0), tok_m = mind_token_mfma_lds_bytes(), dec_s = mind_dec_scene_lds_bytes(), dec_a = mind_dec_actor_lds_bytes();
  const KernelLds lds[] = {
      {k_pair<0>, pair}, {k_pair<1>, pair}, {k_pair_bf<0, 3>, pair_bf}, {k_pair_bf<1, 3>, pair_bf}, {k_pair_bf<0, 1>, pair_bf}, {k_pair_bf<1, 1>, pair_bf},
      {k_pair_t<0, 3>, pair_bf}, {k_pair_t<1, 3>, pair_bf}, {k_pair_t<0, 1>, pair_bf}, {k_pair_t<1, 1>, pair_bf}, {k_pair_t6<0>, pair_bf}, {k_pair_t6<1>, pair_bf},
      {k_actor_net, mind_actor_lds_bytes()}, {k_actor_mfma<3>, actor_m}, {k_actor_mfma<6>, actor_m}, {k_actor_mfma<1>, actor_m},
      {k_dec_actor_mfma<1>, dec_m}, {k_dec_actor_mfma<3>, dec_m}, {k_dec_actor_mfma<6>, dec_m}, {k_actor_f32<1>, mind_actor_f32_lds_bytes(1)}, {k_actor_f32<2>, mind_actor_f32_lds_bytes(2)},
      {k_ilqr<true, 0>, il}, {k_ilqr<false, 1>, il}, {k_ilqr<false, 0>, il}, {k_ilqr<false, 2>, il}, {k_token_mfma<0>, tok_m}, {k_token_mfma<1>, tok_m},
      {k_dec_scene, dec_s}, {k_dec_scene_mw, dec_s}, {k_dec_scene_c, dec_s}, {k_dec_cls, dec_s}, {k_dec_tgt, dec_s},
      {k_dec_actor<0>, dec_a}, {k_dec_actor<1>, dec_a}, {k_dec_actor<2>, dec_a}, {k_dec_actor<2, 1>, dec_a}, {k_dec_actor<2, 2>, dec_a},
  };
  for (const KernelLds &k : lds) (void)hipFuncSetAttribute(k.kernel, hipFuncAttributeMaxDynamicSharedMemorySize, (int)k.bytes);
  lw_set_attributes();
}

static const char *const PAIR_PREC_NAMES[4] = {"f32", "bf16x3", "bf16", "bf16x6"};

extern "C" int mind_ctx_create(int device, void *stream, mind_ctx **out) {
  if (!out) return MIND_EINVAL;
  *out = nullptr;
  int n = 0;
  if (hipGetDeviceCount(&n) != hipSuccess || n <= 0) return MIND_EHIP;
  if (device < 0 || device >= n) return MIND_EINVAL;
  std::unique_ptr<mind_ctx> c(new mind_ctx());
  c->device = device;
  if (hipSetDevice(device) != hipSuccess) return MIND_EHIP;
  c->stream = (hipStream_t)stream;
  if (c->side.create() != hipSuccess || c->ev_side.create(hipEventDisableTiming) != hipSuccess || c->ev_main.create(hipEventDisableTiming) != hipSuccess ||
      c->ev_tgt.create(hipEventDisableTiming) != hipSuccess)
    c->side.reset();
  if (c->ev_stage.create(hipEventDisableTiming) != hipSuccess) return MIND_EHIP;
  hipDeviceProp_t prop;
  if (hipGetDeviceProperties(&prop, device) == hipSuccess) c->n_cu = prop.multiProcessorCount;
  if (hipDeviceGetAttribute(&c->wall_khz, hipDeviceAttributeWallClockRate, device) != hipSuccess || c->wall_khz < 0) c->wall_khz = 0;
  set_kernel_attributes();
  tn_apply_env(c->knobs(), [](const char *name) -> const char * { return getenv(name); });
  if (const char *pe = getenv("MIND_PAIR_PREC"))
    for (int m = 0; m < 4; ++m)
      if (!strcmp(pe, PAIR_PREC_NAMES[m]) || (pe[0] == '0' + m && !pe[1])) (void)mind_set_pair_precision(c.get(), m);
  *out = c.release();
  return MIND_OK;
}

extern "C" int mind_ctx_destroy(mind_ctx *c) {
  if (!c) return MIND_EINVAL;
  if (c->pa_thread.joinable()) c->pa_thread.join();
  (void)hipSetDevice(c->device);
  (void)hipStreamSynchronize(c->stream);
  if (c->side) (void)hipStreamSynchronize(c->side);
  if (c->pl_copy) (void)hipStreamSynchronize(c->pl_copy);
  c->il_finish = nullptr;
  delete c;
  return MIND_OK;
}

extern "C" const char *mind_last_error_string(mind_ctx *c) { return c ? c->err.c_str() : "null context"; }

extern "C" int mind_ctx_synchronize(mind_ctx *c) {
  if (!c) return MIND_EINVAL;
  HIPCHK(c, hipStreamSynchronize(c->stream));
  return MIND_OK;
}

extern "C" int mind_set_tuning(mind_ctx *c, const char *name, int value) {
  if (!c || !name) return MIND_EINVAL;
  if (!tn_set(c->knobs(), name, value)) return fail(c, MIND_EINVAL, "mind_set_tuning: unknown knob '%s'", name);
  return MIND_OK;
}

extern "C" int mind_get_tuning(mind_ctx *c, const char *name, int *value) {
  if (!c || !name || !value) return MIND_EINVAL;
  if (!tn_get(c->knobs(), name, value)) return fail(c, MIND_EINVAL, "mind_get_tuning: unknown knob '%s'", name);
  return MIND_OK;
}

extern "C" int mind_debug_tuning(int index, const char *name, const char *text, int value, const char **out_name, const char **out_env, int *out_value) {
  PredTuning pt; IlqrTuning it; CtxTuning ct;
  const TnRefs fresh{&pt, &it, &ct};
  const TnRow *row = name ? tn_find(name) : (index >= 0 && index < TN_ROWS) ? &TN_TABLE[index] : nullptr;
  if (!row || !out_value || (name && text && !row->env)) return MIND_EINVAL;
  if (name && text) tn_apply_env(fresh, [&](const char *var) { return strcmp(var, row->env) ? nullptr : text; });
  else if (name) (void)tn_set(fresh, name, value);
  if (out_name) *out_name = row->name;
  if (out_env) *out_env = row->env;
  (void)tn_get(fresh, row->name, out_value);
  return name ? MIND_OK : TN_ROWS;
}

extern "C" int mind_debug_live_handles(void) { return (int)live_handles.load(std::memory_order_relaxed); }

extern "C" int mind_set_exchange(mind_ctx *c, int rank, int world, mind_exchange_fn fn, void *user, int force) {
  if (!c) return MIND_EINVAL;
  if (fn && (world < 1 || rank < 0 || rank >= world)) return fail(c, MIND_EINVAL, "mind_set_exchange: rank %d of %d", rank, world);
  c->xfn = fn; c->xuser = user;
  c->xr = fn ? rank : 0; c->xw = fn ? world : 1; c->xforce = fn && force != 0;
  return MIND_OK;
}

extern "C" int mind_last_exchange_stats(mind_ctx *c, long long *collectives, long long *bytes) {
  if (!c) return MIND_EINVAL;
  if (collectives) *collectives = c->x_collectives;
  if (bytes) *bytes = c->x_bytes;
  return MIND_OK;
}

extern "C" int mind_set_pair_precision(mind_ctx *c, int mode) {
  if (!c || mode < 0 || mode > 3) return MIND_EINVAL;
  c->pair_prec = mode;
  return MIND_OK;
}

extern "C" int mind_get_pair_precision(mind_ctx *c) { return c ? c->pair_prec : MIND_EINVAL; }

extern "C" int mind_debug_pack_bfrag(const float *w, int row_stride, uint32_t *out) {
  if (!w || !out || row_stride < 128) return MIND_EINVAL;
  std::vector<float> v(w, w + (size_t)127 * row_stride + 128);
  v.resize((size_t)128 * row_stride, 0.f);
  const std::vector<float> t = pack_bfrag(v, row_stride);
  memcpy(out, t.data(), 16384 * sizeof(uint32_t));
  return MIND_OK;
}

static int lc_reserve(mind_ctx *c, int records, int grid);
extern "C" int mind_set_profiling(mind_ctx *c, int enable) {
  if (!c) return MIND_EINVAL;
  c->profiling = enable != 0;
  if (c->profiling && c->ct.prof_clock != 0 && c->wall_khz > 0 && c->lc.n_blocks == 0) {
    HIPCHK(c, hipSetDevice(c->device));
    return lc_reserve(c, 12, c->n_cu);
  }
  return MIND_OK;
}

extern "C" int mind_last_ilqr_stats(mind_ctx *c, float *kernel_ms, int *n_trees, int *workgroups_per_tree) {
  if (!c) return MIND_EINVAL;
  if (kernel_ms) *kernel_ms = c->ilqr_ms;
  if (n_trees) *n_trees = c->ilqr_trees;
  if (workgroups_per_tree) *workgroups_per_tree = c->ilqr_multi;
  return MIND_OK;
}

extern "C" int mind_last_ilqr_trace(mind_ctx *c, int tree, int phase, double *out, int cap_rows, int *n_rows) {
  if (!c || !n_rows || (cap_rows > 0 && !out)) return MIND_EINVAL;
  if (tree < 0 || tree >= (int)c->il_trace_dev.size() || phase < 0 || phase >= c->il_trace_phases || !c->il_trace_dev[tree])
    return fail(c, MIND_ESTATE, "mind_last_ilqr_trace: no trace for tree %d phase %d (the last tree-iLQR call had %d trees, %d phases)", tree, phase,
                (int)c->il_trace_dev.size(), c->il_trace_phases);
  const int rows = std::min(c->il_trace_its[2 * tree + phase], c->il_trace_cap);
  *n_rows = rows;
  const int take = std::min(rows, cap_rows);
  if (take > 0) {
    HIPCHK(c, hipMemcpyAsync(out, c->il_trace_dev[tree] + (size_t)phase * c->il_trace_cap * IL_TRACE_W, (size_t)take * IL_TRACE_W * sizeof(double),
                             hipMemcpyDeviceToHost, c->stream));
    HIPCHK(c, hipStreamSynchronize(c->stream));
  }
  return MIND_OK;
}

extern "C" int mind_last_ilqr_profile(mind_ctx *c, double *out9) {
  if (!c || !out9) return MIND_EINVAL;
  memcpy(out9, c->il_prof, sizeof(c->il_prof));
  return MIND_OK;
}
// ... 521 lines not shown
    for (i = 8; i < n - (n % 8); i += 8)
      for (int j = 0; j < 8; ++j) r[j] += a[i + j];
    double res = ((r[0] + r[1]) + (r[2] + r[3])) + ((r[4] + r[5]) + (r[6] + r[7]));
    for (; i < n; ++i) res += a[i];
    return res;
  }
  long n2 = n / 2;
  n2 -= n2 % 8;
  return np_pairwise(a, n2) + np_pairwise(a + n2, n - n2);
}
template <class T>
void eval_nodes(const double *st, const double *ct, long N, const T *lane, int P, double tv, double *per_node) {
  const int S = P - 1;
  std::vector<T> dx(S), dy(S), l2(S);
  for (int q = 0; q < S; ++q) {
    dx[q] = lane[2 * q + 2] - lane[2 * q];
    dy[q] = lane[2 * q + 3] - lane[2 * q + 1];
    l2[q] = dx[q] * dx[q] + dy[q] * dy[q];
  }
  constexpr int BS = 8;
  const int NB = (S + BS - 1) / BS;
  std::vector<double> sx_(S), sy_(S), sr_(S), bx(NB), by(NB), br(NB);
  for (int q = 0; q < S; ++q) {
    const double ax = (double)lane[2 * q], ay = (double)lane[2 * q + 1], ex = (double)lane[2 * q + 2], ey = (double)lane[2 * q + 3];
    sx_[q] = 0.5 * (ax + ex); sy_[q] = 0.5 * (ay + ey);
    sr_[q] = 0.5 * sqrt((ex - ax) * (ex - ax) + (ey - ay) * (ey - ay)) * (1.0 + 1e-9) + 1e-9;
  }
  for (int b = 0; b < NB; ++b) {
    const int q0 = b * BS, q1 = std::min(S, q0 + BS);
    double cx = 0.0, cy = 0.0;
    for (int q = q0; q < q1; ++q) { cx += sx_[q]; cy += sy_[q]; }
    cx /= (double)(q1 - q0); cy /= (double)(q1 - q0);
    double r = 0.0;
    for (int q = q0; q < q1; ++q) r = std::max(r, sqrt((sx_[q] - cx) * (sx_[q] - cx) + (sy_[q] - cy) * (sy_[q] - cy)) + sr_[q]);
    bx[b] = cx; by[b] = cy; br[b] = r * (1.0 + 1e-9) + 1e-9;
  }
  int b_prev = 0;
  for (long i = 0; i < N; ++i) {
    const double px = st[6 * i], py = st[6 * i + 1];
    double emin = INFINITY, rmin = INFINITY;
    bool saw_nan = false;
    int b_best = b_prev;
    auto price_block = [&](int b) {
      const int q0 = b * BS, q1 = std::min(S, q0 + BS);
      for (int q = q0; q < q1; ++q) {
        if (emin < INFINITY) {
          const double cxq = px - sx_[q], cyq = py - sy_[q], lim = rmin + sr_[q];
          if (cxq * cxq + cyq * cyq > lim * lim) continue;
        }
        const double sx = (double)lane[2 * q], sy = (double)lane[2 * q + 1], ddx = (double)dx[q], ddy = (double)dy[q];
        double t = ((px - sx) * ddx + (py - sy) * ddy) / (double)l2[q];
        t = t < 0.0 ? 0.0 : (t > 1.0 ? 1.0 : t);
        const double ex = px - (sx + t * ddx), ey = py - (sy + t * ddy);
        const double e = ex * ex + ey * ey;
        if (e < emin) { emin = e; rmin = sqrt(e) * (1.0 + 1e-9) + 1e-9; b_best = b; }
        else if (e != e) saw_nan = true;
      }
    };
    price_block(b_prev);
    for (int b = 0; b < NB; ++b) {
      if (b == b_prev) continue;
      if (emin < INFINITY) {
        const double cxb = px - bx[b], cyb = py - by[b], lim = rmin + br[b];
        if (cxb * cxb + cyb * cyb > lim * lim) continue;
      }
      price_block(b);
    }
    b_prev = b_best;
    const double dmin = saw_nan ? (double)NAN : sqrt(emin);
    const double c0 = ct[2 * i], c1 = ct[2 * i + 1], dv = tv - st[6 * i + 2];
    per_node[i] = ((0.1 * (c0 * c0) + 5.0 * (c1 * c1)) + 0.01 * (dv * dv)) + 0.01 * dmin;
  }
}
}

extern "C" int mind_fill_tracks(const double *raw , int a, int T, const int32_t *slot ,
                                float *pos , float *ang , float *vel , int16_t *typ ,
                                int16_t *have ) {
  if (!raw || !slot || !pos || !ang || !vel || !typ || !have || a < 0 || T <= 0) return MIND_EINVAL;
  for (int i = 0; i < a; ++i) {
    const double *r = raw + (size_t)i * T * 6;
    int first = 0;
    for (int t = 0; t < T; ++t)
      if (r[t * 6] != 0.0) { first = t; break; }
    int src = -1;
    for (int t = 0; t < T; ++t) {
      const bool h = r[t * 6] != 0.0;
      if (h) src = t;
      const int f = src < 0 ? first : src;
      const bool hf = r[f * 6] != 0.0;
      const size_t o = (size_t)i * T + t;
      pos[2 * o] = hf ? (float)r[f * 6 + 1] : 0.f;
      pos[2 * o + 1] = hf ? (float)r[f * 6 + 2] : 0.f;
      ang[o] = hf ? (float)r[f * 6 + 3] : 0.f;
      vel[2 * o] = h ? (float)r[t * 6 + 4] : 0.f;
      vel[2 * o + 1] = h ? (float)r[t * 6 + 5] : 0.f;
      have[o] = h ? 1 : 0;
      for (int k = 0; k < 7; ++k) typ[o * 7 + k] = (h && k == slot[i]) ? 1 : 0;
    }
  }
  return MIND_OK;
}

extern "C" int mind_eval_traj_trees(const double *states, const double *ctrls, const int32_t *counts, int n_trees, const void *lane,
                                    int lane_is_f32, int n_lane_pts, double target_vel, double *out) {
  if (!states || !ctrls || !counts || n_trees <= 0 || !lane || n_lane_pts < 2 || !out) return MIND_EINVAL;
  long N = 0;
  for (int t = 0; t < n_trees; ++t) { if (counts[t] <= 0) return MIND_EINVAL; N += counts[t]; }
  std::vector<double> per(N);
  auto run = [&](long lo, long hi) {
    if (lane_is_f32) eval_nodes<float>(states + 6 * lo, ctrls + 2 * lo, hi - lo, (const float *)lane, n_lane_pts, target_vel, per.data() + lo);
    else eval_nodes<double>(states + 6 * lo, ctrls + 2 * lo, hi - lo, (const double *)lane, n_lane_pts, target_vel, per.data() + lo);
  };
  const long nth = std::min<long>(std::min<long>(8, (long)std::max(1u, std::thread::hardware_concurrency())), N / 8192);
  if (nth <= 1) run(0, N);
  else {
    std::vector<std::thread> th;
    for (long k = 0; k < nth; ++k) th.emplace_back(run, N * k / nth, N * (k + 1) / nth);
    for (std::thread &t : th) t.join();
  }
  long o = 0;
  for (int t = 0; t < n_trees; ++t) {
    const long n = counts[t];
    out[t] = (n > 1 ? per[o] + np_pairwise(per.data() + o + 1, n - 1) : per[o]) / (double)n;
    o += n;
  }
  return MIND_OK;
}

__global__ void k_debug_trig(const double *__restrict__ x, int n, double *__restrict__ out) {
  const int i = blockIdx.x * blockDim.x + threadIdx.x;
  const double v = i < n ? x[i] : 0.0;
  double s, c, t, c2;
  mind_sincos(v, &s, &c);
  mind_tan_cos(v, &t, &c2);
  if (i < n) { out[4 * i] = s; out[4 * i + 1] = c; out[4 * i + 2] = t; out[4 * i + 3] = c2; }
}
extern "C" int mind_debug_trig(mind_ctx *c, const double *x, int n, double *out) {
  if (!c || !x || !out || n <= 0) return MIND_EINVAL;
  HIPCHK(c, hipSetDevice(c->device));
  double *d = nullptr;
  HIPCHK(c, hipMalloc((void **)&d, (size_t)n * 5 * sizeof(double)));
  hipError_t e = hipMemcpy(d, x, (size_t)n * sizeof(double), hipMemcpyHostToDevice);
  if (e == hipSuccess) {
    hipLaunchKernelGGL(k_debug_trig, dim3((n + 63) / 64), dim3(64), 0, c->stream, d, n, d + n);
    e = hipStreamSynchronize(c->stream);
  }
  if (e == hipSuccess) e = hipMemcpy(out, d + n, (size_t)n * 4 * sizeof(double), hipMemcpyDeviceToHost);
  (void)hipFree(d);
  if (e != hipSuccess) return fail(c, MIND_EHIP, "mind_debug_trig: %s", hipGetErrorString(e));
  return MIND_OK;
}

extern "C" int mind_debug_set_layers(mind_ctx *c, int n) {
  if (!c || n < 0 || n > 6) return MIND_EINVAL;
  c->debug_layers = n;
  return MIND_OK;
}
extern "C" int64_t mind_debug_read(mind_ctx *c, const char *name, float *host, int64_t max_floats) {
  if (!c || !name) return MIND_EINVAL;
  const void *src = nullptr;
  int64_t n = 0;
  std::string k = name;
  if (k == "x") { src = c->x.p; n = (int64_t)c->last_ntok * 128; }
  else if (k == "ST") { src = c->ST.p; n = (int64_t)c->last_ntok * 256; }
  else if (k == "QK") { src = c->QK.p; n = (int64_t)c->last_ntok * 1024; }
  else if (k == "edge") { src = c->edge.p; n = c->last_edge_pairs * 128; }
  else if (k == "part") { src = c->part.p; n = (int64_t)c->last_slots * PART_STRIDE; }
  else if (k == "actor_feat") { src = c->actor_feat.p; n = (int64_t)c->last_A * 128; }
  else if (k == "tokpos") { src = c->tokpos.p; n = (int64_t)c->last_ntok * 4; }
  else if (k == "cmode") { src = c->cmode.p; n = (int64_t)c->last_B * 768; }
  else if (k == "tgt_emb") { src = c->tgt_emb.p; n = (int64_t)c->last_B * 128; }
  else if (k == "tgt_feat") { src = c->tgt_feat.p; n = (int64_t)c->last_B * 128; }
  else if (k == "pl_root") { src = c->pl_root.p; n = (int64_t)(c->pl_root.cap / sizeof(float)); }
  else if (k == "il_spec") {
    if (!host) return 2;
    if (max_floats < 2) return MIND_EINVAL;
    host[0] = (float)c->il_spec_req; host[1] = (float)c->il_spec_hit;
    return 2;
  }
  else if (k.rfind("il_", 0) == 0 && c->il_dbg[5]) {
    const size_t M = c->il_dbg[5];
    int w = -1; size_t per = 0;
    if (k == "il_L") { w = 0; per = 1; } else if (k == "il_Lx") { w = 1; per = 6; } else if (k == "il_Lxx") { w = 2; per = 36; }
    else if (k == "il_Fx") { w = 3; per = 36; } else if (k == "il_xs") { w = 4; per = 6; }
    if (w < 0) return MIND_EINVAL;
    src = (const char *)c->ilqr_dev.p + c->il_dbg[w];
    n = (int64_t)(M * per * 2);
  }
  else return MIND_EINVAL;
  if (!host) return n;
  if (n > max_floats) n = max_floats;
  if (hipStreamSynchronize(c->stream) != hipSuccess) return MIND_EHIP;
  if (k == "edge" && c->last_edge_tiled) {
    long long pt = 0;
    for (int N : c->last_scene_n) pt += (long long)N * (((N + 15) / 16) * 16);
    const bool eb = c->last_edge_bf16;
    std::vector<float> raw((size_t)pt * (eb ? 64 : 128));
    if (hipMemcpy(raw.data(), src, raw.size() * sizeof(float), hipMemcpyDeviceToHost) != hipSuccess) return MIND_EHIP;
    int64_t o = 0;
    size_t sb = 0;
    for (int N : c->last_scene_n) {
      const int rows = ((N + 15) / 16) * 16;
      for (int j = 0; j < N; ++j)
        for (int i = 0; i < N; ++i)
          for (int f = 0; f < 128 && o < n; ++f, ++o) {
            const int t = i >> 4, pp = i & 15, b = f >> 4, qq = (f >> 2) & 3, r = f & 3;
            const size_t tile0 = sb + (size_t)j * rows + (size_t)t * 16;
            if (!eb) host[o] = raw[tile0 * 128 + ((b * 64 + qq * 16 + pp) * 4 + r)];
            else {
              uint32_t w;
              memcpy(&w, &raw[tile0 * 64 + (((b >> 1) * 64 + qq * 16 + pp) * 4 + 2 * (b & 1) + (r >> 1))], 4);
              w = (r & 1) ? (w & 0xffff0000u) : (w << 16);
              memcpy(&host[o], &w, 4);
            }
          }
      sb += (size_t)N * rows;
    }
    return n;
  }
  if (hipMemcpy(host, src, (size_t)n * sizeof(float), hipMemcpyDeviceToHost) != hipSuccess) return MIND_EHIP;
  return n;
}

#include "loop.hip"

#include "audit_host.hip"

#include "forecast_host.hip"

#include "road_host.hip"

#include "ttc_host.hip"
```

### mind_amd/csrc/pred_choice.h

```cpp
#pragma once
#include <vector>

#include "tuning.h"

static inline int pred_mfma_parts(const PredTuning &t, int pair_prec) {
  return (pair_prec == 3 || (pair_prec == 1 && t.actor_np == 6)) ? 6 : (pair_prec == 1 ? 3 : 1);
}

static inline bool pred_edge_tiled(const PredTuning &t, int pair_prec) { return pair_prec == 3 || (pair_prec != 0 && t.pair_tile); }

static inline int pred_edge_pair_bytes(const PredTuning &t, int pair_prec) { return pred_edge_tiled(t, pair_prec) && pair_prec == 2 ? 256 : 512; }

enum PredActorForm { PRED_ACTOR_VALU = 0, PRED_ACTOR_F32 = 1, PRED_ACTOR_MFMA = 2, PRED_ACTOR_LW = 3 };
enum PredPairFamily { PRED_PAIR_F32 = 0, PRED_PAIR_BF = 1, PRED_PAIR_T = 2, PRED_PAIR_T6 = 3 };
enum PredDecActor { PRED_DEC_ONE = 0, PRED_DEC_SPLIT = 1, PRED_DEC_MFMA = 2 };

struct PredTokRun {
  int t0, n, kind;
  bool layerwise;
  bool small, merged;
};

struct PredChoice {
  int np = 1;
  int actor_form = PRED_ACTOR_VALU, actor_arg = 0, actor_grid = 0, actor_chunk = 0, actor_chunks = 1, actor_launches = 1;
  int qsplit = 0, qk_stride = 1024;
  bool tiled = false, edge_bf16 = false;
  std::vector<PredTokRun> tok_runs;
  int tok_chunk = 0;
  bool tok_lw = false;
  int last_tok_chunks = 0;
  int pair_family = PRED_PAIR_F32, pair_np = 0;
  bool l5_jobs5 = false;
  int xcd_lanes = 1, xcd_lanes5 = 1;
  int dec_actor = PRED_DEC_ONE;
  int dec_head_ra = RA;
  bool fp32_dec = true, split_dec = false, want_mw = false, cls_side = false;
  int mw_blocks = 0;
  bool tgt_wait_first = false;
};

static PredChoice pred_choose(const PredTuning &t, int pair_prec, int n_cu, bool have_side, int n_scenes, const int *scene_actors, const int *scene_lanes) {
  PredChoice ch;
  int A = 0;
  for (int b = 0; b < n_scenes; ++b) A += scene_actors[b];
  ch.np = pred_mfma_parts(t, pair_prec);

  ch.actor_grid = A;
  if (t.actor_f32 && A >= (pair_prec == 0 ? t.actor_f32_pair_min : t.actor_f32_min)) {
    ch.actor_form = PRED_ACTOR_F32; ch.actor_arg = 2; ch.actor_grid = (A + 1) / 2;
  } else if (pair_prec == 0 && t.actor_f32 && t.enc_mfma) {
    ch.actor_form = PRED_ACTOR_F32; ch.actor_arg = 1;
  } else if (pair_prec == 0 || !t.enc_mfma) {
    ch.actor_form = PRED_ACTOR_VALU;
  } else if (A >= t.actor_lw_min) {
    ch.actor_form = PRED_ACTOR_LW; ch.actor_arg = ch.np;
    ch.actor_chunk = t.actor_lw_chunk > 0 ? t.actor_lw_chunk : LW_CHUNK;
    ch.actor_chunks = (A + ch.actor_chunk - 1) / ch.actor_chunk;
    ch.actor_grid = ch.actor_chunks;
    ch.actor_launches = ch.actor_chunks * (1 + 2 * LW_NSTAGE);
  } else {
    ch.actor_form = PRED_ACTOR_MFMA; ch.actor_arg = ch.np;
  }

  ch.qsplit = pair_prec == 3 ? 48 : pair_prec != 0 ? 16 : 0;
  ch.qk_stride = pair_prec == 3 ? P6_QK_STRIDE : 1024;
  ch.tiled = pred_edge_tiled(t, pair_prec);
  ch.edge_bf16 = pred_edge_pair_bytes(t, pair_prec) == 256;

  ch.tok_chunk = t.tok_lw_chunk > 0 ? t.tok_lw_chunk : TL_CHUNK;
  long long njobs = 0, njobs5 = 0;
  int t0 = 0;
  for (int b = 0; b < n_scenes; ++b) {
    const int N = scene_actors[b] + scene_lanes[b] + 1;
    const int kind = t.tok_mfma ? 1 : (pair_prec != 0 && pair_prec != 3 && t.tok_bf_min_n > 0 && N >= t.tok_bf_min_n) ? 2 : N >= t.tok_lw_min_n ? 1 : 0;
    if (!ch.tok_runs.empty() && ch.tok_runs.back().kind == kind) ch.tok_runs.back().n += N;
    else ch.tok_runs.push_back({t0, N, kind, false, false, false});
    t0 += N;
    njobs += (long long)N * pair_column_splits(N);
    njobs5 += (long long)(scene_actors[b] + 1) * pair_column_splits(N);
  }
  for (PredTokRun &r : ch.tok_runs) {
    r.layerwise = r.kind == 1 && r.n >= t.tok_lw_min;
    r.small = r.kind == 0 && r.n <= t.tok_small_max;
    r.merged = r.small && t.tok_merge;
    if (r.layerwise) {
      ch.tok_lw = true;
      ch.last_tok_chunks += (r.n + ch.tok_chunk - 1) / ch.tok_chunk;
    }
  }

  ch.pair_family = pair_prec == 0 ? PRED_PAIR_F32 : pair_prec == 3 ? PRED_PAIR_T6 : ch.tiled ? PRED_PAIR_T : PRED_PAIR_BF;
  ch.pair_np = (ch.pair_family == PRED_PAIR_T || ch.pair_family == PRED_PAIR_BF) ? (pair_prec == 1 ? 3 : 1) : 0;
  ch.l5_jobs5 = ch.tiled;
  ch.xcd_lanes = pair_xcd_lanes(t.xcd_order, n_scenes, pair_grid(njobs, n_cu));
  ch.xcd_lanes5 = pair_xcd_lanes(t.xcd_order, n_scenes, pair_grid(njobs5, n_cu));

  ch.fp32_dec = pair_prec == 0 || !t.enc_mfma || A < t.dec_mfma_min;
  ch.split_dec = ch.fp32_dec && have_side && t.dec_overlap;
  ch.dec_actor = ch.split_dec ? PRED_DEC_SPLIT : ch.fp32_dec ? PRED_DEC_ONE : PRED_DEC_MFMA;
  if (ch.split_dec) ch.dec_head_ra = t.dec_head_ra ? t.dec_head_ra : A <= n_cu ? 1 : (A + 1) / 2 <= n_cu ? 2 : RA;
  ch.mw_blocks = ((n_scenes + 7) / 8) * 8 * DEC_MW_G;
  ch.want_mw = t.dec_mw && ch.mw_blocks <= n_cu;
  ch.cls_side = ch.split_dec && t.dec_cls_side;
  ch.tgt_wait_first = have_side && !t.tgt_side;
  return ch;
}
```

### mind_amd/csrc/predict.hip

```cpp
__global__ void k_tokpos(const TokMeta *__restrict__ meta, int n_tok, const float *__restrict__ actr,
                         const float *__restrict__ avec, const float *__restrict__ lctr,
                         const float *__restrict__ lvec, float *__restrict__ tokpos) {
  const int t = blockIdx.x * blockDim.x + threadIdx.x;
  if (t >= n_tok) return;
  const TokMeta m = meta[t];
  float4 o = make_float4(0.f, 0.f, 0.f, 0.f);
  if (m.type == 0 && actr) o = make_float4(actr[m.src * 2], actr[m.src * 2 + 1], avec[m.src * 2], avec[m.src * 2 + 1]);
  if (m.type == 1 && lctr) o = make_float4(lctr[m.src * 2], lctr[m.src * 2 + 1], lvec[m.src * 2], lvec[m.src * 2 + 1]);
  ((float4 *)tokpos)[t] = o;
}

struct PairTables {
  std::vector<TokMeta> meta;
  std::vector<PairJob> jobs, jobs5;
  std::vector<int> actor_row, actor_scene, cls_row, scene_n;
  long long edge_pairs = 0, edge_pairs_t = 0;
  int ntok = 0, slot = 0;
  double pairs_full = 0, pairs_l5 = 0;
};

static void pair_tables_build(int Bn, const int *scene_actors, const int *scene_lanes, bool xcd_order, int n_cu, PairTables &T) {
  int A = 0;
  for (int b = 0; b < Bn; ++b) A += scene_actors[b];
  T.actor_row.assign(A, 0); T.actor_scene.assign(A, 0); T.cls_row.assign(Bn, 0); T.scene_n.assign(Bn, 0);
  int a0 = 0, l0 = 0;
  for (int b = 0; b < Bn; ++b) {
    const int a = scene_actors[b], l = scene_lanes[b];
    const int N = a + l + 1;
    const int tiles = (N + 15) / 16;
    const int ns = pair_column_splits(N);
    for (int j = 0; j < N; ++j) {
      TokMeta m;
      memset(&m, 0, sizeof(m));
      m.type = j < a ? 0 : (j < a + l ? 1 : 2);
      m.src = j < a ? a0 + j : (j < a + l ? l0 + (j - a) : 0);
      m.slot0 = T.slot;
      m.nsplit = ns;
      m.flags = (j < a || j == N - 1) ? 1 : 0;
      T.meta.push_back(m);
      for (int s_ = 0; s_ < ns; ++s_) {
        PairJob J;
        memset(&J, 0, sizeof(J));
        J.edge_base = T.edge_pairs;
        J.edge_base_t = T.edge_pairs_t;
        J.N = N;
        J.j = j;
        pair_job_range(tiles, ns, s_, &J.t0, &J.t1);
        J.tok_base = T.ntok;
        J.slot = T.slot++;
        J.flags = m.flags;
        J.scene = b;
        T.jobs.push_back(J);
      }
      if (j < a) { T.actor_row[a0 + j] = T.ntok + j; T.actor_scene[a0 + j] = b; }
    }
    T.cls_row[b] = T.ntok + N - 1;
    T.scene_n[b] = N;
    T.ntok += N;
    T.edge_pairs += (long long)N * N;
    T.edge_pairs_t += (long long)N * tiles * 16;
    T.pairs_full += (double)N * N;
    T.pairs_l5 += (double)N * (a + 1);
    a0 += a; l0 += l;
  }
  for (const PairJob &J : T.jobs)
    if (J.flags & 1) T.jobs5.push_back(J);
  for (std::vector<PairJob> *jl : {&T.jobs, &T.jobs5}) {
    const int grid = pair_grid((long long)jl->size(), n_cu);
    pair_jobs_deal(*jl, grid, PAIR_WAVES, pair_xcd_lanes(xcd_order, Bn, grid));
  }
}

extern "C" int mind_debug_pair_schedule(const int *scene_tokens, const int *scene_actors, int n_scenes, int n_cu, int last_layer, int *out_jobs, int cap,
                                        int *out_info) {
  if (!scene_tokens || !scene_actors || n_scenes <= 0 || n_cu <= 0 || !out_jobs || !out_info) return MIND_EINVAL;
  std::vector<int> lanes(n_scenes);
  for (int b = 0; b < n_scenes; ++b) {
    const int N = scene_tokens[b], a = scene_actors[b];
    if (N <= 0 || a < 0 || a >= N) return MIND_EINVAL;
    lanes[b] = N - a - 1;
  }
  PairTables T;
  pair_tables_build(n_scenes, scene_actors, lanes.data(), true, n_cu, T);
  const std::vector<PairJob> &jl = last_layer ? T.jobs5 : T.jobs;
  const int grid = pair_grid((long long)jl.size(), n_cu);
  const int stride = grid * PAIR_WAVES;
  int n = 0;
  for (size_t i = 0; i < jl.size(); ++i) {
    const PairJob &J = jl[i];
    if (J.t1 <= J.t0) continue;
    if (n < cap) {
      int *o = out_jobs + (size_t)6 * n;
      o[0] = J.scene; o[1] = J.j; o[2] = J.t0; o[3] = J.t1; o[4] = J.slot; o[5] = (int)(i % stride);
    }
    ++n;
  }
  out_info[0] = pair_column_splits(scene_tokens[0]); out_info[1] = grid; out_info[2] = (int)jl.size(); out_info[3] = n;
  return n;
}

#define PRED_CHOICE_HEADER 32
extern "C" int mind_debug_predict_choice(const char *const *knob_names, const int *knob_values, int n_knobs, int pair_prec, int n_cu, int have_side,
                                         const int *scene_actors, const int *scene_lanes, int n_scenes, long long *out, int cap) {
  if (n_knobs < 0 || (n_knobs > 0 && (!knob_names || !knob_values)) || pair_prec < 0 || pair_prec > 3 || n_cu <= 0 || !scene_actors || !scene_lanes ||
      n_scenes <= 0 || cap < 0 || (cap > 0 && !out))
    return MIND_EINVAL;
  PredTuning t;
  const TnRefs own{&t, nullptr, nullptr};
  for (int k = 0; k < n_knobs; ++k)
    if (!knob_names[k] || !tn_set(own, knob_names[k], knob_values[k])) return MIND_EINVAL;
  for (int b = 0; b < n_scenes; ++b)
    if (scene_actors[b] <= 0 || scene_lanes[b] < 0) return MIND_EINVAL;
  const PredChoice ch = pred_choose(t, pair_prec, n_cu, have_side != 0, n_scenes, scene_actors, scene_lanes);
  const bool mfma_dec = ch.dec_actor == PRED_DEC_MFMA;
  const long long head[PRED_CHOICE_HEADER] = {
      PRED_CHOICE_HEADER, (long long)ch.tok_runs.size(), ch.np, ch.actor_form, ch.actor_arg, ch.actor_grid, ch.actor_chunk, ch.actor_chunks,
      ch.actor_launches, ch.qsplit, ch.qk_stride, ch.tiled, ch.edge_bf16, pred_edge_pair_bytes(t, pair_prec), ch.tok_chunk, ch.tok_lw,
      ch.last_tok_chunks, ch.pair_family, ch.pair_np, ch.l5_jobs5, ch.xcd_lanes, ch.xcd_lanes5, ch.dec_actor, mfma_dec ? ch.np : 0,
      ch.fp32_dec, ch.split_dec, ch.want_mw, ch.mw_blocks, ch.cls_side && !ch.want_mw, ch.tgt_wait_first, ch.split_dec ? ch.dec_head_ra : 0, 0};
  std::vector<long long> rec(head, head + PRED_CHOICE_HEADER);
  for (const PredTokRun &r : ch.tok_runs) rec.insert(rec.end(), {r.t0, r.n, r.kind, r.layerwise, r.small, r.merged});
  for (size_t i = 0; i < rec.size() && (int)i < cap; ++i) out[i] = rec[i];
  return (int)rec.size();
}

static bool lc_on(const mind_ctx *c) { return c->profiling && c->ct.prof_clock != 0 && c->wall_khz > 0; }
static bool lc_events(const mind_ctx *c) { return c->profiling && !(c->ct.prof_clock == 1 && c->wall_khz > 0); }

static void lc_account(mind_ctx *c, const LcRecord &r, double (&ms)[LC_KINDS], int (&n)[LC_KINDS]) {
  const double t = lc_ticks_ms(lc_reduce(c->lc_host.as<LcSlot>() + c->lc.slot_of(r.block), r.grid), c->wall_khz);
  ms[r.kind] += t; n[r.kind] += 1;
  c->lc_last[r.kind].push_back((float)t);
}

static int lc_flush(mind_ctx *c, bool keep) {
  const int n = (int)c->lc.pending.size();
  if (n > 0) {
    HIPCHK(c, hipStreamSynchronize(c->stream));
    if (c->pl_copy) HIPCHK(c, hipStreamSynchronize(c->pl_copy));
    int first[2], count[2];
    const int runs = c->lc.pending_runs(0, n, first, count);
    for (int k = 0; k < runs; ++k) {
      const size_t o = c->lc.slot_of(first[k]), b = (size_t)count[k] * c->lc.block_slots * sizeof(LcSlot);
      HIPCHK(c, hipMemcpy(c->lc_host.as<LcSlot>() + o, (const LcSlot *)c->lc_dev.p + o, b, hipMemcpyDeviceToHost));
    }
    if (keep)
      for (const LcRecord &r : c->lc.pending) lc_account(c, r, c->lc_carry_ms, c->lc_carry_n);
    c->lc.drained(n);
  }
  return MIND_OK;
}

static int lc_reserve(mind_ctx *c, int records, int grid) {
  if (c->lc.fits(records, grid)) return MIND_OK;
  int rc, blocks, slots;
  if ((rc = lc_flush(c, true))) return rc;
  c->lc.grown(records, grid, blocks, slots);
  if (blocks != c->lc.n_blocks || slots != c->lc.block_slots) {
    const size_t bytes = (size_t)blocks * slots * sizeof(LcSlot);
    if ((rc = ensure_exact(c, c->lc_dev, bytes, "the launch clock's ring"))) return rc;
    if (c->lc_host.alloc(bytes) != hipSuccess) { c->lc.reset(0, 0); return fail(c, MIND_ENOMEM, "hipHostMalloc(%zu) for the launch clock failed", bytes); }
    c->lc.reset(blocks, slots);
  }
  return MIND_OK;
}

static LcSlot *lc_take(mind_ctx *c, int grid, int kind) {
  if (!lc_on(c)) return nullptr;
  const int b = c->lc.take(grid, kind);
  return b < 0 ? nullptr : (LcSlot *)c->lc_dev.p + c->lc.slot_of(b);
}

static int lc_copy_async(mind_ctx *c, hipStream_t s, int i0, int n) {
  int first[2], count[2];
  const int runs = c->lc.pending_runs(i0, n, first, count);
  for (int k = 0; k < runs; ++k) {
    const size_t o = c->lc.slot_of(first[k]), b = (size_t)count[k] * c->lc.block_slots * sizeof(LcSlot);
    HIPCHK(c, hipMemcpyAsync(c->lc_host.as<LcSlot>() + o, (const LcSlot *)c->lc_dev.p + o, b, hipMemcpyDeviceToHost, s));
  }
  if (runs > 0) c->lc.mark_copied(i0, n);
  return MIND_OK;
}

static int lc_resolve(mind_ctx *c, int n, unsigned kinds, double (&ms)[LC_KINDS], int (&cnt)[LC_KINDS]) {
  for (int k = 0; k < LC_KINDS; ++k) {
    ms[k] = 0.0; cnt[k] = 0;
    if (kinds >> k & 1u) c->lc_last[k].clear();
  }
  if (n < 0 || n > (int)c->lc.pending.size()) n = (int)c->lc.pending.size();
  if (!c->lc.copied(n)) {
    int rc;
    if ((rc = lc_flush(c, true))) return rc;
  } else {
    for (int i = 0; i < n; ++i) lc_account(c, c->lc.pending[i], c->lc_carry_ms, c->lc_carry_n);
    c->lc.drained(n);
  }
  for (int k = 0; k < LC_KINDS; ++k)
    if (kinds >> k & 1u) { ms[k] = c->lc_carry_ms[k]; cnt[k] = c->lc_carry_n[k]; c->lc_carry_ms[k] = 0.0; c->lc_carry_n[k] = 0; }
  return MIND_OK;
}

struct PredCall {
  mind_ctx *c;
  const mind_scene_batch *in;
  mind_pred_out *out;
  const mind_pred_aux *aux;
  const PredChoice &ch;
  int Bn, A, Ltot;
  hipStream_t st, ss;
  TableSet *ts = nullptr;
  const float *lane_feat = nullptr;
  const float *const *rpe_dev = nullptr;
  Event *evs = nullptr;
  bool tok_timed = false;
  bool act_ev = false, pair_ev = false;
  bool pair_clk = false;
  size_t ev_tok_used = 0;
  float *x() const { return (float *)c->x.p; }
  const int *rows() const { return (const int *)ts->rows.p; }
};

static int pred_tables(PredCall &p, const int *scene_actors, const int *scene_lanes) {
  mind_ctx *c = p.c;
  const int Bn = p.Bn, A = p.A;
  std::vector<int> key;
  key.reserve(2 * Bn + 3);
  key.push_back(Bn);
  for (int b = 0; b <= Bn; ++b) key.push_back(p.in->actor_off[b]);
  for (int b = 0; b <= Bn; ++b) key.push_back(p.in->lane_off[b]);
  TableSet *ts = nullptr;
  for (TableSet &t : c->tabs)
    if (t.key == key) ts = &t;
  const bool tab_hit = ts != nullptr;
  if (!ts) {
    ts = &c->tabs[0];
    for (TableSet &t : c->tabs)
      if (t.stamp < ts->stamp) ts = &t;
  }
  ts->stamp = ++c->tab_clock;
  p.ts = ts;
  if (tab_hit) {
    c->n_table_hits++;
    return MIND_OK;
  }
  PairTables T;
  pair_tables_build(Bn, scene_actors, scene_lanes, c->pt.xcd_order, c->n_cu, T);
  int rc;
  ts->key.clear();
  if ((rc = ensure(c, ts->meta, T.meta.size() * sizeof(TokMeta)))) return rc;
  if ((rc = ensure(c, ts->jobs, T.jobs.size() * sizeof(PairJob)))) return rc;
  if ((rc = ensure(c, ts->jobs5, T.jobs5.size() * sizeof(PairJob)))) return rc;
  if ((rc = ensure(c, ts->rows, (size_t)(2 * A + Bn) * sizeof(int)))) return rc;
  HIPCHK(c, hipMemcpyAsync(ts->meta.p, T.meta.data(), T.meta.size() * sizeof(TokMeta), hipMemcpyHostToDevice, p.st));
  HIPCHK(c, hipMemcpyAsync(ts->jobs.p, T.jobs.data(), T.jobs.size() * sizeof(PairJob), hipMemcpyHostToDevice, p.st));
  HIPCHK(c, hipMemcpyAsync(ts->jobs5.p, T.jobs5.data(), T.jobs5.size() * sizeof(PairJob), hipMemcpyHostToDevice, p.st));
  std::vector<int> rows(2 * A + Bn);
  memcpy(rows.data(), T.actor_row.data(), A * sizeof(int));
  memcpy(rows.data() + A, T.actor_scene.data(), A * sizeof(int));
  memcpy(rows.data() + 2 * A, T.cls_row.data(), Bn * sizeof(int));
  HIPCHK(c, hipMemcpyAsync(ts->rows.p, rows.data(), rows.size() * sizeof(int), hipMemcpyHostToDevice, p.st));
  HIPCHK(c, hipStreamSynchronize(p.st));
  ts->actor_row.swap(T.actor_row);
  ts->cls_row.swap(T.cls_row);
  ts->scene_n.swap(T.scene_n);
  ts->edge_pairs = T.edge_pairs; ts->edge_pairs_t = T.edge_pairs_t; ts->ntok = T.ntok; ts->slot = T.slot; ts->njobs = (int)T.jobs.size();
  ts->njobs5 = (int)T.jobs5.size();
  ts->pairs_full = T.pairs_full; ts->pairs_l5 = T.pairs_l5;
  ts->key.swap(key);
  return MIND_OK;
}

static int pred_workspaces(PredCall &p) {
// ... 88 lines not shown
  }
  p.lane_feat = in->lane_feat;
  if (!p.lane_feat) {
    float *lf = p.out->lane_feat ? p.out->lane_feat : (float *)c->lane_feat.p;
    if (Ltot > 0)
      hipLaunchKernelGGL(k_lane_net, dim3((Ltot + PL - 1) / PL), dim3(DT), 0, ss, in->lanes, Ltot, lf, c->W.lane);
    p.lane_feat = lf;
  } else if (p.out->lane_feat && p.out->lane_feat != in->lane_feat && Ltot > 0) {
    HIPCHK(c, hipMemcpyAsync(p.out->lane_feat, in->lane_feat, (size_t)Ltot * 128 * sizeof(float), hipMemcpyDeviceToDevice, ss));
  }
  hipLaunchKernelGGL(k_tokpos, dim3((ntok + 255) / 256), dim3(256), 0, ss, (const TokMeta *)p.ts->meta.p, ntok, in->actor_ctrs, in->actor_vecs,
                     in->lane_ctrs, in->lane_vecs, (float *)c->tokpos.p);
  if (c->side) {
    HIPCHK(c, hipEventRecord(c->ev_side, c->side));
    HIPCHK(c, hipStreamWaitEvent(st, c->ev_side, 0));
  }
  hipLaunchKernelGGL(k_lane_net, dim3((Bn + PL - 1) / PL), dim3(DT), 0, ss, in->tgt_nodes, Bn, (float *)c->tgt_feat.p, c->W.lane);
  hipLaunchKernelGGL(k_dec_tgt, dim3(Bn), dim3(DT), mind_dec_scene_lds_bytes(), ss, (const float *)c->tgt_feat.p, in->tgt_rpe, (float *)c->tgt_emb.p,
                     c->W.dec);
  if (c->enc_post) {
    const std::function<int(hipStream_t)> post = std::move(c->enc_post);
    c->enc_post = nullptr;
    if ((rc = post(ss))) return rc;
  }
  if (c->side) HIPCHK(c, hipEventRecord(c->ev_tgt, c->side));
  if (p.ch.tgt_wait_first) HIPCHK(c, hipStreamWaitEvent(st, c->ev_tgt, 0));
  return MIND_OK;
}

static hipError_t ev_grow(std::vector<Event> &v, size_t n) {
  hipError_t rc = hipSuccess;
  for (Event e; v.size() < n && (rc = e.create()) == hipSuccess;) v.push_back(std::move(e));
  return rc;
}

static hipError_t pred_tok_mark(PredCall &p, int tag) {
  mind_ctx *c = p.c;
  if (!p.tok_timed) return hipSuccess;
  if (p.ev_tok_used == c->ev_tok.size()) {
    const hipError_t rc_ = ev_grow(c->ev_tok, p.ev_tok_used + 1);
    if (rc_ != hipSuccess) return rc_;
    c->ev_tok_tag.push_back(0);
  }
  c->ev_tok_tag[p.ev_tok_used] = tag;
  return hipEventRecord(c->ev_tok[p.ev_tok_used++], p.st);
}

static int pred_token_step(PredCall &p, int mode, int Lw) {
  mind_ctx *c = p.c;
  hipStream_t st = p.st;
  const size_t qk_stride = p.ch.qk_stride, tokm_lds = mind_token_mfma_lds_bytes();
  const float *actor_feat = (const float *)c->actor_feat.p, *lane_feat = p.lane_feat;
  float *part = (float *)c->part.p;
  HIPCHK(c, pred_tok_mark(p, -1));
  for (const PredTokRun &r : p.ch.tok_runs) {
    const TokMeta *m_ = (const TokMeta *)p.ts->meta.p + r.t0;
    float *x_ = p.x() + (size_t)r.t0 * 128, *ST_ = (float *)c->ST.p + (size_t)r.t0 * 256, *QK_ = (float *)c->QK.p + (size_t)r.t0 * qk_stride;
    if (r.layerwise) {
      tl_build_plan(r.n, mode, p.ch.tok_chunk, c->n_cu, c->tok_lw_plan);
      for (const TlLaunch &L : c->tok_lw_plan) {
        if (tl_launch(L, st, mode, m_, actor_feat, lane_feat, x_, part, ST_, QK_, qk_stride, c->W.tok[Lw], c->W.tokM[Lw], (float *)c->tok_lw_arena.p, p.ch.tok_chunk))
          return fail(c, MIND_ESTATE, "layer-wise token stage: a stage has no kernel");
        HIPCHK(c, pred_tok_mark(p, L.stage));
      }
      c->last_tok_launches += (int)c->tok_lw_plan.size();
      continue;
    }
    c->last_tok_launches++;
    if (r.kind == 0) {
      const int tpw = r.small ? TOK_TPW_SMALL : TOK_TPW_BIG;
      hipLaunchKernelGGL(r.small ? (r.merged ? k_token_m : k_token<TOK_TPW_SMALL>) : k_token<TOK_TPW_BIG>, dim3((r.n + tpw - 1) / tpw), dim3(TT_THREADS), 0,
                         st, m_, r.n, mode, actor_feat, lane_feat, x_, part, ST_, QK_, c->W.tok[Lw]);
    } else if (r.kind == 1) {
      hipLaunchKernelGGL(k_token_mfma<0>, dim3((r.n + TM_TOK - 1) / TM_TOK), dim3(TM_THREADS), tokm_lds, st, m_, r.n, mode, actor_feat, lane_feat, x_,
                         part, ST_, QK_, c->W.tok[Lw], c->W.tokM[Lw]);
    } else {
      hipLaunchKernelGGL(k_token_mfma<1>, dim3((r.n + TM_TOK - 1) / TM_TOK), dim3(TM_THREADS), tokm_lds, st, m_, r.n, mode, actor_feat, lane_feat, x_,
                         part, ST_, QK_, c->W.tok[Lw], c->W.tokB[Lw]);
    }
    HIPCHK(c, pred_tok_mark(p, TL_NSTAGE));
  }
  return MIND_OK;
}

static int pred_pair_layer(PredCall &p, int L) {
  mind_ctx *c = p.c;
  const PredChoice &ch = p.ch;
  const TableSet *ts = p.ts;
  const bool last = L == 5, own5 = last && ch.l5_jobs5;
  const int um = L < 4 ? 0 : (L == 4 ? 1 : 2);
  const PairJob *jl = (const PairJob *)(own5 ? ts->jobs5.p : ts->jobs.p);
  const int nj = own5 ? ts->njobs5 : ts->njobs;
  const dim3 grid(pair_grid(nj, c->n_cu)), block(PAIR_THREADS);
  float *edge = (float *)c->edge.p, *ST = (float *)c->ST.p, *QK = (float *)c->QK.p, *part = (float *)c->part.p, *tokpos = (float *)c->tokpos.p;
  const size_t ldsb = mind_pair_bf_lds_bytes();
  const u32 *we = c->W.pair.WBe[L], *wp = last ? c->W.pair.WBe[L] : c->W.pair.WBp[L];
  LcSlot *clk = p.pair_clk ? lc_take(c, (int)grid.x, LC_PAIR) : nullptr;
  if (p.pair_ev) HIPCHK(c, hipEventRecord(p.evs[2 * L], p.st));
#define PAIR_GO(K0, K1, LDS, ...)                                                                                                             \
  do {                                                                                                                                        \
    if (L == 0) hipLaunchKernelGGL(K0, grid, block, LDS, p.st, jl, nj, edge, ST, QK, part, __VA_ARGS__, c->W.pair.vtab[L], c->W.pair.rtab, tokpos, p.rpe_dev, um, clk); \
    else hipLaunchKernelGGL(K1, grid, block, LDS, p.st, jl, nj, edge, ST, QK, part, __VA_ARGS__, c->W.pair.vtab[L], c->W.pair.rtab, tokpos, p.rpe_dev, um, clk);   \
  } while (0)
  switch (ch.pair_family) {
  case PRED_PAIR_F32: PAIR_GO((k_pair<0>), (k_pair<1>), mind_pair_lds_bytes(), c->W.pair.WAe[L], last ? c->W.pair.WAe[L] : c->W.pair.WAp[L]); break;
  case PRED_PAIR_T6: PAIR_GO((k_pair_t6<0>), (k_pair_t6<1>), ldsb, we, wp, c->W.pair.WLe[L], last ? c->W.pair.WLe[L] : c->W.pair.WLp[L]); break;
  case PRED_PAIR_T:
    if (ch.pair_np == 3) PAIR_GO((k_pair_t<0, 3>), (k_pair_t<1, 3>), ldsb, we, wp);
    else PAIR_GO((k_pair_t<0, 1>), (k_pair_t<1, 1>), ldsb, we, wp);
    break;
  default:
    if (ch.pair_np == 3) PAIR_GO((k_pair_bf<0, 3>), (k_pair_bf<1, 3>), ldsb, we, wp);
    else PAIR_GO((k_pair_bf<0, 1>), (k_pair_bf<1, 1>), ldsb, we, wp);
  }
#undef PAIR_GO
  if (p.pair_ev) HIPCHK(c, hipEventRecord(p.evs[2 * L + 1], p.st));
  c->n_pair_launch++;
  c->pairs_done += last ? ts->pairs_l5 : ts->pairs_full;
  return MIND_OK;
}

static int pred_fusion(PredCall &p) {
  mind_ctx *c = p.c;
  const PredChoice &ch = p.ch;
  const TableSet *ts = p.ts;
  int rc;
  c->last_tok_lw = ch.tok_lw; c->last_tok_launches = 0; c->last_tok_chunks = ch.last_tok_chunks; c->tok_ms = 0.f;
  for (float &v : c->tok_stage_ms) v = 0.f;
  if (ch.tok_lw && (rc = ensure_exact(c, c->tok_lw_arena, tl_arena_bytes(ch.tok_chunk), "the layer-wise token stage's arena"))) return rc;
  p.tok_timed = c->profiling && !c->ev_defer;
  if ((rc = pred_token_step(p, 1 | 4 | ch.qsplit, 0))) return rc;
  c->n_pair_launch = 0;
  c->pairs_done = 0;
  p.pair_clk = lc_on(c);
  p.pair_ev = lc_events(c);
  if (p.pair_clk && (rc = lc_reserve(c, c->debug_layers, std::max(pair_grid(ts->njobs, c->n_cu), pair_grid(ts->njobs5, c->n_cu))))) return rc;
  if (p.pair_ev) HIPCHK(c, ev_grow(c->ev, 12));
  p.evs = c->ev.data();
  if (p.pair_ev && c->ev_defer) {
    HIPCHK(c, ev_grow(c->ev_pool, c->ev_pool_used + 12));
    p.evs = c->ev_pool.data() + c->ev_pool_used;
    c->ev_pending.push_back(c->ev_pool_used);
    c->ev_pool_used += 12;
  }
  c->last_ntok = ts->ntok; c->last_edge_pairs = ts->edge_pairs; c->last_slots = ts->slot; c->last_A = p.A; c->last_B = p.Bn;
  c->last_scene_n = ts->scene_n; c->last_edge_tiled = ch.tiled; c->last_edge_bf16 = ch.edge_bf16;
  for (int L = 0; L < c->debug_layers; ++L) {
    if ((rc = pred_pair_layer(p, L))) return rc;
    if ((rc = pred_token_step(p, 2 | (L < 5 ? 4 : 8) | ch.qsplit, L + 1))) return rc;
  }
  return MIND_OK;
}

static int pred_decoder(PredCall &p) {
  mind_ctx *c = p.c;
  const PredChoice &ch = p.ch;
  mind_pred_out *out = p.out;
  hipStream_t st = p.st;
  const int A = p.A, Bn = p.Bn;
  const float *x = p.x();
  const int *d_actor_row = p.rows(), *d_actor_scene = d_actor_row + A, *d_cls_row = d_actor_row + 2 * A;
  const float *cmode = (const float *)c->cmode.p, *tgt_emb = (const float *)c->tgt_emb.p;
  const dim3 agrid((A + RA - 1) / RA), mgrid((A + DM_RA - 1) / DM_RA);
  float *cov_vel = p.aux ? p.aux->cov_vel : nullptr, *param = p.aux ? p.aux->param : nullptr;
  int rc;
  if (ch.split_dec) {
    if ((rc = ensure(c, c->dec_h2, (size_t)A * 768 * sizeof(float)))) return rc;
    HIPCHK(c, hipEventRecord(c->ev_main, st));
    HIPCHK(c, hipStreamWaitEvent(c->side, c->ev_main, 0));
    hipLaunchKernelGGL(k_dec_actor<1>, agrid, dim3(DT), mind_dec_actor_lds_bytes(), c->side, x, d_actor_row, d_actor_scene, A,
                       (const float *)nullptr, (const float *)nullptr, (float *)nullptr, (float *)nullptr, c->W.dec, (float *)c->dec_h2.p,
                       (float *)nullptr, (float *)nullptr);
    HIPCHK(c, hipEventRecord(c->ev_side, c->side));
  }
  bool cls_on_side = false;
  bool mw = ch.want_mw;
  if (mw) {
    if (c->dec_abort && *c->dec_abort.as<volatile unsigned>()) return fail(c, MIND_EHIP, "k_dec_scene_mw: a barrier of an earlier launch timed out (launch not resident)");
    if (!c->dec_abort) {
      if (c->dec_abort.alloc(64, hipHostMallocMapped) != hipSuccess) mw = false;
      else *c->dec_abort.as<unsigned>() = 0u;
    }
    const size_t need_x = (size_t)(c->n_cu / DEC_MW_G) * 2 * 6 * 1536 * sizeof(float), need_b = (size_t)(c->n_cu / DEC_MW_G) * 4 * sizeof(unsigned);
    if (mw && c->dec_xbuf.cap < need_x) {
      if ((rc = ensure(c, c->dec_xbuf, need_x))) return rc;
    }
    if (mw && c->dec_bars.cap < need_b) {
      if ((rc = ensure(c, c->dec_bars, need_b))) return rc;
      HIPCHK(c, hipMemsetAsync(c->dec_bars.p, 0, c->dec_bars.cap, st));
    }
  }
  if (mw)
    hipLaunchKernelGGL(k_dec_scene_mw, dim3(ch.mw_blocks), dim3(DT), mind_dec_scene_lds_bytes(), st, x, d_cls_row, (float *)c->cmode.p, out->cls, c->W.dec, Bn,
                       (float *)c->dec_xbuf.p, (unsigned *)c->dec_bars.p, c->dec_abort.as<unsigned>());
  else if (ch.cls_side) {
    hipLaunchKernelGGL(k_dec_scene_c, dim3(Bn), dim3(DT), mind_dec_scene_lds_bytes(), st, x, d_cls_row, (float *)c->cmode.p, c->W.dec);
    HIPCHK(c, hipEventRecord(c->ev_main, st));
    HIPCHK(c, hipStreamWaitEvent(c->side, c->ev_main, 0));
    hipLaunchKernelGGL(k_dec_cls, dim3(Bn), dim3(DT), mind_dec_scene_lds_bytes(), c->side, (float *)c->cmode.p, out->cls, c->W.dec);
    if (!c->ev_cls) HIPCHK(c, c->ev_cls.create(hipEventDisableTiming));
    HIPCHK(c, hipEventRecord(c->ev_cls, c->side));
    cls_on_side = true;
  } else
    hipLaunchKernelGGL(k_dec_scene, dim3(Bn), dim3(DT), mind_dec_scene_lds_bytes(), st, x, d_cls_row, (float *)c->cmode.p, out->cls, c->W.dec);
  if (c->side) HIPCHK(c, hipStreamWaitEvent(st, c->ev_tgt, 0));
  switch (ch.dec_actor) {
  case PRED_DEC_SPLIT:
    HIPCHK(c, hipStreamWaitEvent(st, c->ev_side, 0));
#define DEC_HEAD(RAV)                                                                                                                       \
  hipLaunchKernelGGL((k_dec_actor<2, RAV>), dim3((A + RAV - 1) / RAV), dim3(DT), mind_dec_actor_lds_bytes(), st, x, d_actor_row, d_actor_scene, A, \
                     cmode, tgt_emb, out->reg, out->vel, c->W.dec, (float *)c->dec_h2.p, cov_vel, param)
    if (ch.dec_head_ra == 1) DEC_HEAD(1);
    else if (ch.dec_head_ra == 2) DEC_HEAD(2);
    else DEC_HEAD(RA);
#undef DEC_HEAD
    break;
  case PRED_DEC_ONE:
    hipLaunchKernelGGL(k_dec_actor<0>, agrid, dim3(DT), mind_dec_actor_lds_bytes(), st, x, d_actor_row, d_actor_scene, A, cmode, tgt_emb, out->reg,
                       out->vel, c->W.dec, (float *)nullptr, cov_vel, param);
    break;
  default: {
#define DEC_MFMA(NPV)                                                                                                                     \
  hipLaunchKernelGGL(k_dec_actor_mfma<NPV>, mgrid, dim3(DM_T), mind_dec_actor_mfma_lds_bytes(), st, x, d_actor_row, d_actor_scene, A, cmode, \
                     tgt_emb, out->reg, out->vel, c->W.decB, cov_vel, param)
    if (ch.np == 6) DEC_MFMA(6);
    else if (ch.np == 3) DEC_MFMA(3);
    else DEC_MFMA(1);
#undef DEC_MFMA
  }
  }
  if (cls_on_side) HIPCHK(c, hipStreamWaitEvent(st, c->ev_cls, 0));
  return MIND_OK;
}

static int pred_finish(PredCall &p) {
  mind_ctx *c = p.c;
  mind_pred_out *out = p.out;
  const float *x = p.x();
  for (int a = 0; a < p.A && out->actor_emb; ++a)
    HIPCHK(c, hipMemcpyAsync(out->actor_emb + (size_t)a * 128, x + (size_t)p.ts->actor_row[a] * 128, 128 * sizeof(float), hipMemcpyDeviceToDevice, p.st));
  for (int b = 0; b < p.Bn && out->cls_emb; ++b)
    HIPCHK(c, hipMemcpyAsync(out->cls_emb + (size_t)b * 128, x + (size_t)p.ts->cls_row[b] * 128, 128 * sizeof(float), hipMemcpyDeviceToDevice, p.st));
  HIPCHK(c, hipGetLastError());
  if (c->profiling && c->ev_defer) {
    c->pair_ms = 0.f;
  } else if (c->profiling) {
    HIPCHK(c, hipStreamSynchronize(p.st));
    c->pair_ms = 0.f;
    for (int k : {LC_PAIR, LC_ACTOR}) { c->ev_last[k].clear(); c->lc_last[k].clear(); }
    for (int L = 0; L < c->debug_layers && p.pair_ev; ++L) {
      float ms = 0.f;
      HIPCHK(c, hipEventElapsedTime(&ms, c->ev[2 * L], c->ev[2 * L + 1]));
      c->pair_ms += ms;
      c->ev_last[LC_PAIR].push_back(ms);
    }
    if (p.act_ev) {
      HIPCHK(c, hipEventElapsedTime(&c->actor_ms, c->ev_act0, c->ev_act1));
      c->ev_last[LC_ACTOR].push_back(c->actor_ms);
    }
    if (lc_on(c)) {
      double ms[LC_KINDS];
      int n[LC_KINDS], rc;
      if ((rc = lc_resolve(c, -1, 1u << LC_PAIR | 1u << LC_ACTOR, ms, n))) return rc;
      if (n[LC_PAIR] > 0) c->pair_ms = (float)ms[LC_PAIR];
      if (n[LC_ACTOR] > 0) c->actor_ms = (float)ms[LC_ACTOR];
    }
    for (size_t i = 1; i < p.ev_tok_used; ++i) {
      if (c->ev_tok_tag[i] < 0) continue;
      float ms = 0.f;
      HIPCHK(c, hipEventElapsedTime(&ms, c->ev_tok[i - 1], c->ev_tok[i]));
      c->tok_stage_ms[c->ev_tok_tag[i]] += ms;
      c->tok_ms += ms;
    }
  }
  return MIND_OK;
}

extern "C" int mind_predict_batch_aux(mind_ctx *c, const mind_scene_batch *in, mind_pred_out *out, const mind_pred_aux *aux) {
  if (!c || !in || !out) return MIND_EINVAL;
  if (!c->have_weights) return fail(c, MIND_ESTATE, "weights not loaded");
  const int Bn = in->n_scenes;
  if (Bn <= 0 || !in->actor_off || !in->lane_off || !in->actors || !in->tgt_nodes || !in->tgt_rpe || !out->cls ||
      !out->reg || !out->vel)
    return fail(c, MIND_EINVAL, "null input/output pointer");
  if (!in->lanes && !in->lane_feat) return fail(c, MIND_EINVAL, "need lanes or lane_feat");
  if (!in->rpe && !(in->actor_ctrs && in->actor_vecs && in->lane_ctrs && in->lane_vecs))
    return fail(c, MIND_EINVAL, "need rpe or ctrs/vecs");
  HIPCHK(c, hipSetDevice(c->device));
  const int A = in->actor_off[Bn], Ltot = in->lane_off[Bn];
  if (A <= 0 || Ltot < 0) return fail(c, MIND_EINVAL, "empty batch");
  std::vector<int> sa(Bn), sl(Bn);
  for (int b = 0; b < Bn; ++b) {
    sa[b] = in->actor_off[b + 1] - in->actor_off[b]; sl[b] = in->lane_off[b + 1] - in->lane_off[b];
    if (sa[b] <= 0 || sl[b] < 0) return fail(c, MIND_EINVAL, "scene %d has %d agents, %d lanes", b, sa[b], sl[b]);
  }
  const PredChoice ch = pred_choose(c->pt, c->pair_prec, c->n_cu, c->side.p != nullptr, Bn, sa.data(), sl.data());
  PredCall p{c, in, out, aux, ch, Bn, A, Ltot, c->stream, c->side ? c->side.p : c->stream};
  int rc;
  if ((rc = pred_tables(p, sa.data(), sl.data()))) return rc;
  if ((rc = pred_workspaces(p))) return rc;
  if ((rc = pred_encoders(p))) return rc;
  if ((rc = pred_fusion(p))) return rc;
  if ((rc = pred_decoder(p))) return rc;
  return pred_finish(p);
}

extern "C" int mind_predict_batch(mind_ctx *c, const mind_scene_batch *in, mind_pred_out *out) { return mind_predict_batch_aux(c, in, out, nullptr); }
```

Before: 1878.

## Split scene decoder into a multi-kernel chain spreading each scene over G workgroups

Adds a four-kernel decoder chain in which each scene's big dense stages (context c3, FFN l1 and l2) are split across 8/16/32 workgroups per scene, with partial results passed through a global scratch buffer between launches. This replaces the single-workgroup-per-scene k_dec_scene when few scenes leave most CUs idle, and it is chosen automatically unless the mw or cls-side tunings are enabled. It adds extra launches, a global round trip and duplicated attention/LN work per workgroup. The change also factors the scene body into shared helpers and adds a debug entry point for timing the variants.

```diff
diff --git a/include/mind_hip.h b/include/mind_hip.h
--- a/include/mind_hip.h
+++ b/include/mind_hip.h
@@ -125,6 +125,8 @@
 int mind_debug_weight_bind(const mind_tensor_desc *tensors, int n_tensors, const char *drop, char *msg, int msg_cap);
 
 int mind_debug_trig(mind_ctx *ctx, const double *x, int n, double *out);
+
+int mind_debug_dec_scene(mind_ctx *ctx, const float *rows, int n_scenes, int form, float *Cout, float *cls, int reps, float *ms);
 
 int mind_debug_set_layers(mind_ctx *ctx, int n);
 int64_t mind_debug_read(mind_ctx *ctx, const char *name, float *host, int64_t max_floats);
diff --git a/mind_amd/_lib.py b/mind_amd/_lib.py
--- a/mind_amd/_lib.py
+++ b/mind_amd/_lib.py
@@ -224,7 +224,7 @@
 EXPORTS = ["mind_ctx_create", "mind_ctx_destroy", "mind_last_error_string", "mind_ctx_synchronize",
            "mind_weights_load", "mind_predict_batch", "mind_last_fusion_stats", "mind_last_actor_stats", "mind_debug_actor_lw_plan", "mind_last_token_stats", "mind_last_token_stage_ms", "mind_debug_token_lw_plan", "mind_set_profiling", "mind_debug_launch_times", "mind_debug_launch_clock",
            "mind_ilqr_solve_trees", "mind_ilqr_contingency", "mind_ilqr_solve_fields", "mind_cost_eval", "mind_ilqr_score_trees", "mind_ilqr_gains", "mind_ilqr_policy_rollouts", "mind_lane_dist_field", "mind_aime_world", "mind_aime_rebase", "mind_debug_aime_decide", "mind_debug_set_layers",
-           "mind_debug_read", "mind_set_pair_precision", "mind_get_pair_precision", "mind_debug_pack_bfrag", "mind_debug_pack_conv_frag", "mind_debug_pack", "mind_debug_weight_image", "mind_debug_weight_bind", "mind_debug_pair_schedule", "mind_debug_predict_choice", "mind_debug_ilqr_plan", "mind_debug_aime_book", "mind_set_tuning", "mind_get_tuning", "mind_debug_tuning", "mind_debug_live_handles", "mind_last_ilqr_stats", "mind_aime_plan", "mind_last_ilqr_profile", "mind_eval_traj_trees", "mind_last_ilqr_trace", "mind_ilqr_contingency_begin", "mind_ilqr_finish", "mind_fill_tracks", "mind_ilqr_contingency_begin_plan", "mind_debug_trig", "mind_aime_plan_begin", "mind_aime_plan_poll", "mind_aime_plan_finish", "mind_ctx_busy", "mind_ilqr_finish_plan",
+           "mind_debug_read", "mind_set_pair_precision", "mind_get_pair_precision", "mind_debug_pack_bfrag", "mind_debug_pack_conv_frag", "mind_debug_pack", "mind_debug_weight_image", "mind_debug_weight_bind", "mind_debug_pair_schedule", "mind_debug_predict_choice", "mind_debug_ilqr_plan", "mind_debug_aime_book", "mind_set_tuning", "mind_get_tuning", "mind_debug_tuning", "mind_debug_live_handles", "mind_last_ilqr_stats", "mind_aime_plan", "mind_last_ilqr_profile", "mind_eval_traj_trees", "mind_last_ilqr_trace", "mind_ilqr_contingency_begin", "mind_ilqr_finish", "mind_fill_tracks", "mind_ilqr_contingency_begin_plan", "mind_debug_trig", "mind_aime_plan_begin", "mind_aime_plan_poll", "mind_aime_plan_finish", "mind_ctx_busy", "mind_ilqr_finish_plan", "mind_debug_dec_scene",
            "mind_set_exchange", "mind_last_exchange_stats", "mind_debug_wait_word",
            "mind_predict_batch_aux", "mind_set_decoder_basis", "mind_get_decoder_basis", "mind_curve_eval", "mind_debug_curve_basis",
            "mind_audit_plan", "mind_audit_episode", "mind_debug_box_clearance",
@@ -339,6 +339,7 @@
     lib.mind_debug_weight_image.argtypes = [C.POINTER(TensorDesc), C.c_int, C.POINTER(C.c_float), C.c_size_t, C.c_char_p, C.c_size_t,
                                             C.POINTER(C.c_longlong), C.c_int, C.POINTER(C.c_longlong), C.c_char_p, C.c_int]
     lib.mind_debug_weight_bind.argtypes = [C.POINTER(TensorDesc), C.c_int, C.c_char_p, C.c_char_p, C.c_int]
+    lib.mind_debug_dec_scene.argtypes = [C.c_void_p, C.POINTER(C.c_float), C.c_int, C.c_int, C.POINTER(C.c_float), C.POINTER(C.c_float), C.c_int, C.POINTER(C.c_float)]
     lib.mind_debug_set_layers.argtypes = [C.c_void_p, C.c_int]
     lib.mind_debug_read.argtypes = [C.c_void_p, C.c_char_p, C.POINTER(C.c_float), C.c_int64]
     lib.mind_set_exchange.argtypes = [C.c_void_p, C.c_int, C.c_int, EXCHANGE_FN, C.c_void_p, C.c_int]
@@ -392,7 +393,7 @@
 PRED_CHOICE_FIELDS = ("header", "n_runs", "np", "actor_form", "actor_arg", "actor_grid", "actor_chunk", "actor_chunks", "actor_launches", "qsplit", "qk_stride",
                       "tiled", "edge_bf16", "edge_pair_bytes", "tok_chunk", "tok_lw", "tok_chunks", "pair_family", "pair_np", "l5_jobs5", "xcd_lanes",
                       "xcd_lanes5", "dec_actor", "dec_np", "fp32_dec", "split_dec", "want_mw", "mw_blocks", "cls_on_side", "tgt_wait_first",
-                      "dec_head_ra")
+                      "dec_head_ra", "dec_chain_g")
 PAIR_PREC = ("f32", "bf16x3", "bf16", "bf16x6")
 
 
@@ -409,9 +410,21 @@
     if n == MIND_EINVAL:
         return None
     assert 0 < n <= cap and out[0] == 32 and n == 32 + 6 * out[1], n
-    d = dict(zip(PRED_CHOICE_FIELDS, out[:31]))
+    d = dict(zip(PRED_CHOICE_FIELDS, out[:32]))
     d["runs"] = [tuple(out[32 + 6 * i:38 + 6 * i]) for i in range(out[1])]
     return d
+
+
+def dec_scene(lib, ctx, rows, form, reps=1, timed=False):
+    import numpy as np
+    rows = np.ascontiguousarray(rows, np.float32)
+    B = rows.shape[0]
+    assert rows.shape == (B, 128)
+    fp = C.POINTER(C.c_float)
+    cout, cls, ms = np.empty((B, 6, 128), np.float32), np.empty((B, 6), np.float32), np.zeros(reps, np.float32)
+    check(lib, ctx, lib.mind_debug_dec_scene(ctx, rows.ctypes.data_as(fp), B, int(form), cout.ctypes.data_as(fp), cls.ctypes.data_as(fp), reps,
+                                             ms.ctypes.data_as(fp) if timed else None), "mind_debug_dec_scene")
+    return (cout, cls, ms) if timed else (cout, cls)
 
 
 def knobs():
diff --git a/mind_amd/csrc/dec_chain.h b/mind_amd/csrc/dec_chain.h
--- /dev/null
+++ b/mind_amd/csrc/dec_chain.h
@@ -0,0 +1,51 @@
+#pragma once
+
+#define DC_THREADS 1024
+#define DC_PART_FLOATS 24576
+#define DC_ROWS 6
+
+struct DcStage { int K, NOUT, R, KP, Kc; };
+
+constexpr int dc_quads_kp(int R, int K, int NOUT, int nthr, int part_floats) {
+  int KP = 1;
+  while (KP * 2 * (NOUT >> 2) <= nthr && KP * 2 * R * NOUT <= part_floats && KP * 2 <= (K >> 2)) KP *= 2;
+  return KP;
+}
+constexpr int dc_quads_kc(int K, int KP) { return ((K / 4 + KP - 1) / KP) * 4; }
+
+constexpr DcStage DC_C3 = {384, 768, 1, 4, 96};
+constexpr DcStage DC_L1 = {128, 1536, DC_ROWS, 2, 64};
+constexpr DcStage DC_L2 = {1536, 128, DC_ROWS, 32, 48};
+constexpr bool dc_stage_ok(const DcStage &s) {
+  return s.KP == dc_quads_kp(s.R, s.K, s.NOUT, DC_THREADS, DC_PART_FLOATS) && s.Kc == dc_quads_kc(s.K, s.KP) && s.KP * s.Kc == s.K;
+}
+static_assert(dc_stage_ok(DC_C3) && dc_stage_ok(DC_L1) && dc_stage_ok(DC_L2), "the chain restates dense_quads' K split of the three big stages");
+static_assert(DC_L2.K == DC_L1.NOUT && DC_L1.NOUT == DC_L2.KP * DC_L2.Kc, "an l2 part reads a 48-wide slice of l1's outputs");
+
+constexpr int dc_choose_g(int n_scenes, int n_cu) {
+  if (n_scenes <= 0) return 0;
+  for (int G = 32; G >= 8; G >>= 1)
+    if ((long long)n_scenes * G <= n_cu) return G;
+  return 0;
+}
+constexpr bool dc_valid_g(int G) { return G == 8 || G == 16 || G == 32; }
+
+struct DcSlice { int o_lo, no, kp_lo, nkp; };
+constexpr DcSlice dc_slice_c3(int wg, int G) { return {DC_C3.NOUT / G * wg, DC_C3.NOUT / G, 0, DC_C3.KP}; }
+constexpr DcSlice dc_slice_l1(int wg, int G) { return {DC_L1.NOUT / G * wg, DC_L1.NOUT / G, 0, DC_L1.KP}; }
+constexpr DcSlice dc_slice_l2(int wg, int G) { return {0, DC_L2.NOUT, DC_L2.KP / G * wg, DC_L2.KP / G}; }
+
+constexpr int dc_rows_per_thread(int R, int nkp, int no) {
+  for (int rpt = 1; rpt < R; ++rpt)
+    if (R % rpt == 0 && nkp * (R / rpt) * no <= DC_THREADS) return rpt;
+  return R;
+}
+constexpr int dc_items(int R, int rpt, int nkp, int no) { return nkp * (R / rpt) * no; }
+
+struct DcItem { int kpl, r0, ol; };
+constexpr DcItem dc_item(int item, int R, int rpt, int no) { return {item / (no * (R / rpt)), (item / no) % (R / rpt) * rpt, item % no}; }
+
+#define DC_Y_FLOATS 768
+#define DC_C_FLOATS (DC_ROWS * 128)
+#define DC_P_FLOATS (32 * DC_ROWS * 128)
+#define DC_SCENE_FLOATS (DC_Y_FLOATS + 2 * DC_C_FLOATS + 2 * DC_P_FLOATS)
diff --git a/mind_amd/csrc/encdec_kernels.hip b/mind_amd/csrc/encdec_kernels.hip
--- a/mind_amd/csrc/encdec_kernels.hip
+++ b/mind_amd/csrc/encdec_kernels.hip
@@ -4,6 +4,7 @@
 #include "weight_tables.h"
 #include "dec_curve.h"
 #include "launch_clock.h"
+#include "dec_chain.h"
 
 typedef float f32x4 __attribute__((ext_vector_type(4)));
 
@@ -714,6 +715,7 @@
 
 #define DEC_SCENE_PART 24576
 #define DEC_SCENE_LDS_FLOATS (256 + 768 + 768 + 2304 + 768 + 9216 + 768 + 144 + DEC_SCENE_PART)
+static_assert(DT == DC_THREADS && DEC_SCENE_PART == DC_PART_FLOATS, "dec_chain.h restates the workgroup the K splits are taken for");
 __global__ __launch_bounds__(DT) void k_dec_tgt(const float *__restrict__ tgt_feat , const float *__restrict__ tgt_rpe ,
                                                 float *__restrict__ tgt_out , DecW W) {
   extern __shared__ __attribute__((aligned(16))) float dsm[];
@@ -748,6 +750,132 @@
 #else
 #define DEC_MARK() do {} while (0)
 #endif
+struct DecSm {
+  float (*v0)[256];
+  float (*v1)[768];
+  float (*C)[128];
+  float (*qkv)[384];
+  float (*att)[128];
+  float (*ff)[1536];
+  float (*t2)[128];
+  float (*sc)[6][6];
+  float *part;
+};
+__device__ __forceinline__ DecSm dec_carve(float *dsm) {
+  DecSm S;
+  S.v0 = (float (*)[256])(dsm);
+  S.v1 = (float (*)[768])(dsm + 256);
+  S.C = (float (*)[128])(dsm + 1024);
+  S.qkv = (float (*)[384])(dsm + 1792);
+  S.att = (float (*)[128])(dsm + 4096);
+  S.ff = (float (*)[1536])(dsm + 4864);
+  S.t2 = (float (*)[128])(dsm + 14080);
+  S.sc = (float (*)[6][6])(dsm + 14848);
+  S.part = dsm + 14992;
+  return S;
+}
+__device__ __forceinline__ void dec_ctx0(const DecSm &S, const float *__restrict__ x, const int *__restrict__ cls_row, int b, const DecW &W) {
+  const int tid = threadIdx.x;
+  if (tid < 128) S.v0[0][tid] = x[(size_t)cls_row[b] * 128 + tid];
+  __syncthreads();
+  dense<1>(&S.v0[0][0], 256, 128, W.c0W, W.c0b, 384, &S.v1[0][0], 768, S.part, DEC_SCENE_PART);
+  DEC_MARK();
+  __syncthreads();
+  ln_rows(&S.v1[0][0], 768, 1, 384, W.c0g, W.c0be, true);
+  DEC_MARK();
+  __syncthreads();
+}
+__device__ __forceinline__ void dec_ctx3_norm(const DecSm &S, const DecW &W) {
+  const int tid = threadIdx.x;
+  ln_rows(&S.ff[0][0], 1536, 1, 768, W.c3g, W.c3be, true);
+  DEC_MARK();
+  __syncthreads();
+  for (int i = tid; i < 768; i += blockDim.x) S.C[i / 128][i % 128] = S.ff[0][i];
+  __syncthreads();
+}
+__device__ __forceinline__ void dec_attn(const DecSm &S, const DecW &W, int L) {
+  const int tid = threadIdx.x;
+  float (*C)[128] = S.C;
+  float (*qkv)[384] = S.qkv;
+  float (*att)[128] = S.att;
+  float (*t2)[128] = S.t2;
+  float (*sc)[6][6] = S.sc;
+  dense<6>(&C[0][0], 128, 128, W.inW[L], W.inb[L], 384, &qkv[0][0], 384, S.part, DEC_SCENE_PART);
+  DEC_MARK();
+  __syncthreads();
+  if (tid < 4 * 36) {
+    const int hd = tid / 36, s = (tid % 36) / 6, t = tid % 6;
+    float d = 0.f;
+    for (int k = 0; k < 32; ++k) d = fmaf(qkv[s][hd * 32 + k], qkv[t][128 + hd * 32 + k], d);
+    sc[hd][s][t] = d / sqrtf(32.0f);
+  }
+  __syncthreads();
+  if (tid < 24) {
+    const int hd = tid / 6, s = tid % 6;
+    float m = -INFINITY;
+    for (int t = 0; t < 6; ++t) m = fmaxf(m, sc[hd][s][t]);
+    float e[6], sum = 0.f;
+    for (int t = 0; t < 6; ++t) { e[t] = expf(sc[hd][s][t] - m); sum += e[t]; }
+    for (int t = 0; t < 6; ++t) sc[hd][s][t] = e[t] / sum;
+  }
+  __syncthreads();
+  for (int i = tid; i < 6 * 128; i += blockDim.x) {
+    const int s = i / 128, c = i % 128, hd = c / 32;
+    float o = 0.f;
+    for (int t = 0; t < 6; ++t) o = fmaf(sc[hd][s][t], qkv[t][256 + c], o);
+    att[s][c] = o;
+  }
+  __syncthreads();
+  dense<6>(&att[0][0], 128, 128, W.outW[L], W.outb[L], 128, &t2[0][0], 128, S.part, DEC_SCENE_PART);
+  DEC_MARK();
+  __syncthreads();
+  for (int i = tid; i < 768; i += blockDim.x) C[i / 128][i % 128] += t2[i / 128][i % 128];
+  __syncthreads();
+  ln_rows(&C[0][0], 128, 6, 128, W.n1g[L], W.n1b[L], false);
+  DEC_MARK();
+  __syncthreads();
+}
+__device__ __forceinline__ void dec_ffn_close(const DecSm &S, const DecW &W, int L) {
+  const int tid = threadIdx.x;
+  for (int i = tid; i < 768; i += blockDim.x) S.C[i / 128][i % 128] += S.t2[i / 128][i % 128];
+  __syncthreads();
+  ln_rows(&S.C[0][0], 128, 6, 128, W.n2g[L], W.n2b[L], false);
+  DEC_MARK();
+  __syncthreads();
+}
+__device__ __forceinline__ void dec_cls_head(const DecSm &S, const DecW &W, int b, float *__restrict__ cls_out, bool write) {
+  const int tid = threadIdx.x;
+  float (*att)[128] = S.att;
+  float (*t2)[128] = S.t2;
+  float (*sc)[6][6] = S.sc;
+  dense<6>(&S.C[0][0], 128, 128, W.k0W, W.k0b, 128, &att[0][0], 128, S.part, DEC_SCENE_PART);
+  DEC_MARK();
+  __syncthreads();
+  ln_rows(&att[0][0], 128, 6, 128, W.k0g, W.k0be, true);
+  DEC_MARK();
+  __syncthreads();
+  dense<6>(&att[0][0], 128, 128, W.k3W, W.k3b, 128, &t2[0][0], 128, S.part, DEC_SCENE_PART);
+  DEC_MARK();
+  __syncthreads();
+  ln_rows(&t2[0][0], 128, 6, 128, W.k3g, W.k3be, true);
+  DEC_MARK();
+  __syncthreads();
+  for (int k = tid >> 6; k < 6; k += (int)(blockDim.x >> 6)) {
+    const int lane = tid & 63;
+    float s = t2[k][lane] * W.k6W[lane] + t2[k][lane + 64] * W.k6W[lane + 64];
+    s = wave_sum(s);
+    if (lane == 0) sc[0][0][k] = s + W.k6b[0];
+  }
+  __syncthreads();
+  if (tid == 0 && write) {
+    float m = -INFINITY;
+    for (int k = 0; k < 6; ++k) m = fmaxf(m, sc[0][0][k]);
+    float e[6], sum = 0.f;
+    for (int k = 0; k < 6; ++k) { e[k] = expf(sc[0][0][k] - m); sum += e[k]; }
+    for (int k = 0; k < 6; ++k) cls_out[(size_t)b * 6 + k] = e[k] / sum;
+  }
+  DEC_MARK();
+}
 template <bool MW, int PART = 0>
 __device__ __forceinline__ void k_dec_scene_body(const float *__restrict__ x ,
                                                  const int *__restrict__ cls_row ,
@@ -755,15 +883,12 @@
                                                  float *__restrict__ cls_out , const DecW &W, int b, int wg, int G,
                                                  float *xbuf, unsigned *bar, unsigned *abort_word) {
   extern __shared__ __attribute__((aligned(16))) float dsm[];
-  float (*v0)[256] = (float (*)[256])(dsm);
-  float (*v1)[768] = (float (*)[768])(dsm + 256);
-  float (*C)[128] = (float (*)[128])(dsm + 1024);
-  float (*qkv)[384] = (float (*)[384])(dsm + 1792);
-  float (*att)[128] = (float (*)[128])(dsm + 4096);
-  float (*ff)[1536] = (float (*)[1536])(dsm + 4864);
-  float (*t2)[128] = (float (*)[128])(dsm + 14080);
-  float (*sc)[6][6] = (float (*)[6][6])(dsm + 14848);
-  float *part = dsm + 14992;
+  const DecSm S = dec_carve(dsm);
+  float (*v1)[768] = S.v1;
+  float (*C)[128] = S.C;
+  float (*ff)[1536] = S.ff;
+  float (*t2)[128] = S.t2;
+  float *part = S.part;
   const int PF = DEC_SCENE_PART;
   const int tid = threadIdx.x;
   int xstage = 0;
@@ -777,14 +902,7 @@
     __syncthreads();
   }
   if (PART != 2) {
-  if (tid < 128) v0[0][tid] = x[(size_t)cls_row[b] * 128 + tid];
-  __syncthreads();
-  dense<1>(&v0[0][0], 256, 128, W.c0W, W.c0b, 384, &v1[0][0], 768, part, PF);
-  DEC_MARK();
-  __syncthreads();
-  ln_rows(&v1[0][0], 768, 1, 384, W.c0g, W.c0be, true);
-  DEC_MARK();
-  __syncthreads();
+  dec_ctx0(S, x, cls_row, b, W);
   if (MW) {
     dense_quads_part<1>(&v1[0][0], 768, 384, W.c3W, W.c3b, 768, &ff[0][0], 1536, part, PF, wg, G);
     if (dec_exchange<1>(&ff[0][0], 1536, 768, wg, G, (xstage++ & 1) ? xb1 : xb0, bar, abort_word)) return;
@@ -792,46 +910,9 @@
     dense<1>(&v1[0][0], 768, 384, W.c3W, W.c3b, 768, &ff[0][0], 1536, part, PF);
   DEC_MARK();
   __syncthreads();
-  ln_rows(&ff[0][0], 1536, 1, 768, W.c3g, W.c3be, true);
-  DEC_MARK();
-  __syncthreads();
-  for (int i = tid; i < 768; i += blockDim.x) C[i / 128][i % 128] = ff[0][i];
-  __syncthreads();
+  dec_ctx3_norm(S, W);
   for (int L = 0; L < 2; ++L) {
-    dense<6>(&C[0][0], 128, 128, W.inW[L], W.inb[L], 384, &qkv[0][0], 384, part, PF);
-  DEC_MARK();
-    __syncthreads();
-    if (tid < 4 * 36) {
-      const int hd = tid / 36, s = (tid % 36) / 6, t = tid % 6;
-      float d = 0.f;
-      for (int k = 0; k < 32; ++k) d = fmaf(qkv[s][hd * 32 + k], qkv[t][128 + hd * 32 + k], d);
-      sc[hd][s][t] = d / sqrtf(32.0f);
-    }
-    __syncthreads();
-    if (tid < 24) {
-      const int hd = tid / 6, s = tid % 6;
-      float m = -INFINITY;
-      for (int t = 0; t < 6; ++t) m = fmaxf(m, sc[hd][s][t]);
-      float e[6], sum = 0.f;
-      for (int t = 0; t < 6; ++t) { e[t] = expf(sc[hd][s][t] - m); sum += e[t]; }
-      for (int t = 0; t < 6; ++t) sc[hd][s][t] = e[t] / sum;
-    }
-    __syncthreads();
-    for (int i = tid; i < 6 * 128; i += blockDim.x) {
-      const int s = i / 128, c = i % 128, hd = c / 32;
-      float o = 0.f;
-      for (int t = 0; t < 6; ++t) o = fmaf(sc[hd][s][t], qkv[t][256 + c], o);
-      att[s][c] = o;
-    }
-    __syncthreads();
-    dense<6>(&att[0][0], 128, 128, W.outW[L], W.outb[L], 128, &t2[0][0], 128, part, PF);
-  DEC_MARK();
-    __syncthreads();
-    for (int i = tid; i < 768; i += blockDim.x) C[i / 128][i % 128] += t2[i / 128][i % 128];
-    __syncthreads();
-    ln_rows(&C[0][0], 128, 6, 128, W.n1g[L], W.n1b[L], false);
-  DEC_MARK();
-    __syncthreads();
+    dec_attn(S, W, L);
     if (MW) {
       dense_quads_part<6>(&C[0][0], 128, 128, W.l1W[L], W.l1b[L], 1536, &ff[0][0], 1536, part, PF, wg, G);
       if (dec_exchange<6>(&ff[0][0], 1536, 1536, wg, G, (xstage++ & 1) ? xb1 : xb0, bar, abort_word)) return;
@@ -848,43 +929,13 @@
       dense<6>(&ff[0][0], 1536, 1536, W.l2W[L], W.l2b[L], 128, &t2[0][0], 128, part, PF);
   DEC_MARK();
     __syncthreads();
-    for (int i = tid; i < 768; i += blockDim.x) C[i / 128][i % 128] += t2[i / 128][i % 128];
-    __syncthreads();
-    ln_rows(&C[0][0], 128, 6, 128, W.n2g[L], W.n2b[L], false);
-  DEC_MARK();
-    __syncthreads();
+    dec_ffn_close(S, W, L);
   }
   if (!MW || wg == 0)
     for (int i = tid; i < 768; i += blockDim.x) Cout[(size_t)b * 768 + i] = C[i / 128][i % 128];
   }
   if (PART == 1) return;
-  dense<6>(&C[0][0], 128, 128, W.k0W, W.k0b, 128, &att[0][0], 128, part, PF);
-  DEC_MARK();
-  __syncthreads();
-  ln_rows(&att[0][0], 128, 6, 128, W.k0g, W.k0be, true);
-  DEC_MARK();
-  __syncthreads();
-  dense<6>(&att[0][0], 128, 128, W.k3W, W.k3b, 128, &t2[0][0], 128, part, PF);
-  DEC_MARK();
-  __syncthreads();
-  ln_rows(&t2[0][0], 128, 6, 128, W.k3g, W.k3be, true);
-  DEC_MARK();
-  __syncthreads();
-  for (int k = tid >> 6; k < 6; k += (int)(blockDim.x >> 6)) {
-    const int lane = tid & 63;
-    float s = t2[k][lane] * W.k6W[lane] + t2[k][lane + 64] * W.k6W[lane + 64];
-    s = wave_sum(s);
-    if (lane == 0) sc[0][0][k] = s + W.k6b[0];
-  }
-  __syncthreads();
-  if (tid == 0 && (!MW || wg == 0)) {
-    float m = -INFINITY;
-    for (int k = 0; k < 6; ++k) m = fmaxf(m, sc[0][0][k]);
-    float e[6], sum = 0.f;
-    for (int k = 0; k < 6; ++k) { e[k] = expf(sc[0][0][k] - m); sum += e[k]; }
-    for (int k = 0; k < 6; ++k) cls_out[(size_t)b * 6 + k] = e[k] / sum;
-  }
-  DEC_MARK();
+  dec_cls_head(S, W, b, cls_out, !MW || wg == 0);
 #ifdef MIND_DEC_TRACE
   if (blockIdx.x == 0 && tid == 0) {
     printf("[k_dec_scene] cycles between marks (dense / LayerNorm stages in program order):");
@@ -912,6 +963,128 @@
   const int b = 8 * ((int)blockIdx.x / (8 * DEC_MW_G)) + (r & 7), wg = r >> 3;
   if (b >= n_scenes) return;
   k_dec_scene_body<true>(x, cls_row, Cout, cls_out, W, b, wg, DEC_MW_G, xbuf + (size_t)b * 2 * 6 * 1536, bars + 4 * (size_t)b, abort_word);
+}
+
+template <int R, int RPT, int NB>
+__device__ __forceinline__ void dc_slice_parts(const float *in, int ldi, int k_base, const float *__restrict__ WT, int NOUT, int Kc, const DcSlice sl,
+                                               float *dst, int kp_dst, int ldd) {
+  static_assert(R % RPT == 0 && NB % 4 == 0, "rows per thread divide the rows; inputs are read four at a time");
+  const int n_items = dc_items(R, RPT, sl.nkp, sl.no);
+  for (int item = threadIdx.x; item < n_items; item += blockDim.x) {
+    const DcItem it = dc_item(item, R, RPT, sl.no);
+    const int k0 = (sl.kp_lo + it.kpl) * Kc;
+    const float *w = WT + (size_t)k0 * NOUT + sl.o_lo + it.ol;
+    const float *xi = in + it.r0 * ldi + (k0 - k_base);
+    float acc[RPT];
+#pragma unroll
+    for (int j = 0; j < RPT; ++j) acc[j] = 0.f;
+    for (int k = 0; k < Kc; k += NB) {
+      float wv[NB];
+#pragma unroll
+      for (int q = 0; q < NB; ++q) wv[q] = w[(size_t)(k + q) * NOUT];
+#pragma unroll
+      for (int j = 0; j < RPT; ++j) {
+#pragma unroll
+        for (int q4 = 0; q4 < NB / 4; ++q4) {
+          const f32x4 xv = *(const f32x4 *)(xi + j * ldi + k + 4 * q4);
+          acc[j] = fmaf(wv[4 * q4 + 0], xv[0], acc[j]);
+          acc[j] = fmaf(wv[4 * q4 + 1], xv[1], acc[j]);
+          acc[j] = fmaf(wv[4 * q4 + 2], xv[2], acc[j]);
+          acc[j] = fmaf(wv[4 * q4 + 3], xv[3], acc[j]);
+        }
+        DENSE_ROW_FENCE();
+      }
+    }
+#pragma unroll
+    for (int j = 0; j < RPT; ++j) dst[((size_t)(kp_dst + it.kpl) * R + it.r0 + j) * ldd + it.ol] = acc[j];
+  }
+}
+
+template <int G>
+__device__ __forceinline__ void dc_ffn_parts(const DecSm &S, const DecW &W, int L, int wg, float *__restrict__ c_out, float *__restrict__ p_out) {
+  constexpr DcSlice s1 = dc_slice_l1(0, G), s2 = dc_slice_l2(0, G);
+  constexpr int RPT1 = dc_rows_per_thread(DC_ROWS, s1.nkp, s1.no), RPT2 = dc_rows_per_thread(DC_ROWS, s2.nkp, s2.no);
+  static_assert(s1.no * G == DC_L1.NOUT && s2.nkp * G == DC_L2.KP && s1.no == s2.nkp * DC_L2.Kc, "slices are exact and an l2 part reads the workgroup's own l1 slice");
+  static_assert(DC_L1.KP * DC_ROWS * s1.no <= DC_PART_FLOATS && DC_ROWS * s1.no <= DC_ROWS * 1536, "the slice's partials and outputs fit their LDS areas");
+  const int tid = threadIdx.x;
+  const DcSlice l1 = dc_slice_l1(wg, G), l2 = dc_slice_l2(wg, G);
+  if (wg == 0)
+    for (int i = tid; i < 768; i += blockDim.x) c_out[i] = S.C[i / 128][i % 128];
+  dc_slice_parts<DC_ROWS, RPT1, 32>(&S.C[0][0], 128, 0, W.l1W[L], DC_L1.NOUT, DC_L1.Kc, l1, S.part, 0, l1.no);
+  __syncthreads();
+  float *ffs = &S.ff[0][0];
+  for (int i = tid; i < DC_ROWS * l1.no; i += blockDim.x) {
+    const int r = i / l1.no, ol = i % l1.no;
+    float v = W.l1b[L][l1.o_lo + ol];
+    for (int q = 0; q < DC_L1.KP; ++q) v += S.part[(q * DC_ROWS + r) * l1.no + ol];
+    ffs[i] = fmaxf(v, 0.f);
+  }
+  __syncthreads();
+  dc_slice_parts<DC_ROWS, RPT2, 24>(ffs, l1.no, l1.o_lo, W.l2W[L], DC_L2.NOUT, DC_L2.Kc, l2, p_out, l2.kp_lo, DC_L2.NOUT);
+}
+
+__device__ __forceinline__ void dc_ffn_gather(const DecSm &S, const DecW &W, int L, const float *__restrict__ c_in, const float *__restrict__ p_in) {
+  const int tid = threadIdx.x;
+  for (int i = tid; i < 768; i += blockDim.x) S.C[i / 128][i % 128] = c_in[i];
+  if (tid < DC_ROWS * 128) {
+    float pv[DC_L2.KP];
+#pragma unroll
+    for (int q = 0; q < DC_L2.KP; ++q) pv[q] = p_in[(size_t)q * DC_ROWS * 128 + tid];
+    float v = W.l2b[L][tid % 128];
+#pragma unroll
+    for (int q = 0; q < DC_L2.KP; ++q) v += pv[q];
+    S.t2[tid / 128][tid % 128] = v;
+  }
+  __syncthreads();
+  dec_ffn_close(S, W, L);
+}
+
+#define DC_Y(buf, b) ((buf) + (size_t)(b) * DC_SCENE_FLOATS)
+#define DC_C(buf, b, L) (DC_Y(buf, b) + DC_Y_FLOATS + (L) * DC_C_FLOATS)
+#define DC_P(buf, b, L) (DC_Y(buf, b) + DC_Y_FLOATS + 2 * DC_C_FLOATS + (size_t)(L) * DC_P_FLOATS)
+template <int G>
+__global__ __launch_bounds__(DT) void k_dec_chain1(const float *__restrict__ x, const int *__restrict__ cls_row, float *__restrict__ buf, DecW W) {
+  extern __shared__ __attribute__((aligned(16))) float dsm[];
+  const DecSm S = dec_carve(dsm);
+  const int b = (int)blockIdx.x / G, wg = (int)blockIdx.x % G, tid = threadIdx.x;
+  dec_ctx0(S, x, cls_row, b, W);
+  const DcSlice c3 = dc_slice_c3(wg, G);
+  static_assert(dc_slice_c3(0, G).no * G == DC_C3.NOUT && dc_slice_c3(0, G).no * DC_C3.KP <= DT, "slices are exact; one pass over the threads");
+  dc_slice_parts<1, 1, 32>(&S.v1[0][0], 768, 0, W.c3W, DC_C3.NOUT, DC_C3.Kc, c3, S.part, 0, c3.no);
+  __syncthreads();
+  if (tid < c3.no) {
+    float v = W.c3b[c3.o_lo + tid];
+    for (int q = 0; q < DC_C3.KP; ++q) v += S.part[q * c3.no + tid];
+    DC_Y(buf, b)[c3.o_lo + tid] = v;
+  }
+}
+template <int G>
+__global__ __launch_bounds__(DT) void k_dec_chain2(float *__restrict__ buf, DecW W) {
+  extern __shared__ __attribute__((aligned(16))) float dsm[];
+  const DecSm S = dec_carve(dsm);
+  const int b = (int)blockIdx.x / G, wg = (int)blockIdx.x % G, tid = threadIdx.x;
+  if (tid < 768 / 4) *(f32x4 *)(&S.ff[0][4 * tid]) = *(const f32x4 *)(DC_Y(buf, b) + 4 * tid);
+  __syncthreads();
+  dec_ctx3_norm(S, W);
+  dec_attn(S, W, 0);
+  dc_ffn_parts<G>(S, W, 0, wg, DC_C(buf, b, 0), DC_P(buf, b, 0));
+}
+template <int G>
+__global__ __launch_bounds__(DT) void k_dec_chain3(float *__restrict__ buf, DecW W) {
+  extern __shared__ __attribute__((aligned(16))) float dsm[];
+  const DecSm S = dec_carve(dsm);
+  const int b = (int)blockIdx.x / G, wg = (int)blockIdx.x % G;
+  dc_ffn_gather(S, W, 0, DC_C(buf, b, 0), DC_P(buf, b, 0));
+  dec_attn(S, W, 1);
+  dc_ffn_parts<G>(S, W, 1, wg, DC_C(buf, b, 1), DC_P(buf, b, 1));
+}
+__global__ __launch_bounds__(DT) void k_dec_chain4(const float *__restrict__ buf, float *__restrict__ Cout, float *__restrict__ cls_out, DecW W) {
+  extern __shared__ __attribute__((aligned(16))) float dsm[];
+  const DecSm S = dec_carve(dsm);
+  const int b = (int)blockIdx.x, tid = threadIdx.x;
+  dc_ffn_gather(S, W, 1, DC_C(buf, b, 1), DC_P(buf, b, 1));
+  for (int i = tid; i < 768; i += blockDim.x) Cout[(size_t)b * 768 + i] = S.C[i / 128][i % 128];
+  dec_cls_head(S, W, b, cls_out, true);
 }
 
 #define RA 4
diff --git a/mind_amd/csrc/mind_hip.hip b/mind_amd/csrc/mind_hip.hip
--- a/mind_amd/csrc/mind_hip.hip
+++ b/mind_amd/csrc/mind_hip.hip
@@ -162,6 +162,7 @@
   } plan;
   DevBuf pl_flat;
   DevBuf dec_xbuf, dec_bars;
+  DevBuf dec_chain;
   Pinned dec_abort;
   int rb_cur = 0, rb_gen = 0;
   size_t rb_S = 0, rb_a = 0;
@@ -249,6 +250,8 @@
       {k_dec_actor_mfma<1>, dec_m}, {k_dec_actor_mfma<3>, dec_m}, {k_dec_actor_mfma<6>, dec_m}, {k_actor_f32<1>, mind_actor_f32_lds_bytes(1)}, {k_actor_f32<2>, mind_actor_f32_lds_bytes(2)},
       {k_ilqr<true, 0>, il}, {k_ilqr<false, 1>, il}, {k_ilqr<false, 0>, il}, {k_ilqr<false, 2>, il}, {k_token_mfma<0>, tok_m}, {k_token_mfma<1>, tok_m},
       {k_dec_scene, dec_s}, {k_dec_scene_mw, dec_s}, {k_dec_scene_c, dec_s}, {k_dec_cls, dec_s}, {k_dec_tgt, dec_s},
+      {k_dec_chain1<8>, dec_s}, {k_dec_chain2<8>, dec_s}, {k_dec_chain3<8>, dec_s}, {k_dec_chain1<16>, dec_s}, {k_dec_chain2<16>, dec_s}, {k_dec_chain3<16>, dec_s},
+      {k_dec_chain1<32>, dec_s}, {k_dec_chain2<32>, dec_s}, {k_dec_chain3<32>, dec_s}, {k_dec_chain4, dec_s},
       {k_dec_actor<0>, dec_a}, {k_dec_actor<1>, dec_a}, {k_dec_actor<2>, dec_a}, {k_dec_actor<2, 1>, dec_a}, {k_dec_actor<2, 2>, dec_a},
   };
   for (const KernelLds &k : lds) (void)hipFuncSetAttribute(k.kernel, hipFuncAttributeMaxDynamicSharedMemorySize, (int)k.bytes);
@@ -1076,6 +1079,41 @@
   return MIND_OK;
 }
 
+extern "C" int mind_debug_dec_scene(mind_ctx *c, const float *rows, int n_scenes, int form, float *Cout, float *cls, int reps, float *ms) {
+  if (!c || !rows || !Cout || !cls || n_scenes <= 0 || n_scenes > 4096 || !(form == 0 || dc_valid_g(form)) || reps < 1 || reps > 1024) return MIND_EINVAL;
+  if (!c->have_weights) return fail(c, MIND_ESTATE, "weights not loaded");
+  HIPCHK(c, hipSetDevice(c->device));
+  const int B = n_scenes;
+  const size_t nx = (size_t)B * 128, nc = (size_t)B * 768, nk = (size_t)B * 6;
+  DevBuf d;
+  if (d.alloc((nx + nc + nk) * sizeof(float) + (size_t)B * sizeof(int)) != hipSuccess) return fail(c, MIND_ENOMEM, "mind_debug_dec_scene: hipMalloc failed");
+  float *dx = d.as<float>(), *dC = dx + nx, *dk = dC + nc;
+  int *drow = (int *)(dk + nk);
+  std::vector<int> row(B);
+  for (int b = 0; b < B; ++b) row[b] = b;
+  HIPCHK(c, hipMemcpy(dx, rows, nx * sizeof(float), hipMemcpyHostToDevice));
+  HIPCHK(c, hipMemcpy(drow, row.data(), (size_t)B * sizeof(int), hipMemcpyHostToDevice));
+  Event e0, e1;
+  if (ms && (e0.create() != hipSuccess || e1.create() != hipSuccess)) return fail(c, MIND_EHIP, "mind_debug_dec_scene: no events");
+  for (int it = 0; it < reps; ++it) {
+    if (ms) HIPCHK(c, hipEventRecord(e0, c->stream));
+    if (form == 0)
+      hipLaunchKernelGGL(k_dec_scene, dim3(B), dim3(DT), mind_dec_scene_lds_bytes(), c->stream, (const float *)dx, (const int *)drow, dC, dk, c->W.dec);
+    else if (int rc = dec_chain_run(c, form, B, dx, drow, dC, dk, c->stream))
+      return rc;
+    if (ms) {
+      HIPCHK(c, hipEventRecord(e1, c->stream));
+      HIPCHK(c, hipEventSynchronize(e1));
+      HIPCHK(c, hipEventElapsedTime(&ms[it], e0, e1));
+    }
+  }
+  HIPCHK(c, hipGetLastError());
+  HIPCHK(c, hipStreamSynchronize(c->stream));
+  HIPCHK(c, hipMemcpy(Cout, dC, nc * sizeof(float), hipMemcpyDeviceToHost));
+  HIPCHK(c, hipMemcpy(cls, dk, nk * sizeof(float), hipMemcpyDeviceToHost));
+  return MIND_OK;
+}
+
 extern "C" int mind_debug_set_layers(mind_ctx *c, int n) {
   if (!c || n < 0 || n > 6) return MIND_EINVAL;
   c->debug_layers = n;
diff --git a/mind_amd/csrc/pred_choice.h b/mind_amd/csrc/pred_choice.h
--- a/mind_amd/csrc/pred_choice.h
+++ b/mind_amd/csrc/pred_choice.h
@@ -2,6 +2,7 @@
 #include <vector>
 
 #include "tuning.h"
+#include "dec_chain.h"
 
 static inline int pred_mfma_parts(const PredTuning &t, int pair_prec) {
   return (pair_prec == 3 || (pair_prec == 1 && t.actor_np == 6)) ? 6 : (pair_prec == 1 ? 3 : 1);
@@ -37,6 +38,7 @@
   int dec_head_ra = RA;
   bool fp32_dec = true, split_dec = false, want_mw = false, cls_side = false;
   int mw_blocks = 0;
+  int dec_chain_g = 0;
   bool tgt_wait_first = false;
 };
 
@@ -103,6 +105,7 @@
   ch.mw_blocks = ((n_scenes + 7) / 8) * 8 * DEC_MW_G;
   ch.want_mw = t.dec_mw && ch.mw_blocks <= n_cu;
   ch.cls_side = ch.split_dec && t.dec_cls_side;
+  ch.dec_chain_g = (t.dec_mw || t.dec_cls_side) ? 0 : dc_choose_g(n_scenes, n_cu);
   ch.tgt_wait_first = have_side && !t.tgt_side;
   return ch;
 }
diff --git a/mind_amd/csrc/predict.hip b/mind_amd/csrc/predict.hip
--- a/mind_amd/csrc/predict.hip
+++ b/mind_amd/csrc/predict.hip
@@ -117,7 +117,7 @@
       PRED_CHOICE_HEADER, (long long)ch.tok_runs.size(), ch.np, ch.actor_form, ch.actor_arg, ch.actor_grid, ch.actor_chunk, ch.actor_chunks,
       ch.actor_launches, ch.qsplit, ch.qk_stride, ch.tiled, ch.edge_bf16, pred_edge_pair_bytes(t, pair_prec), ch.tok_chunk, ch.tok_lw,
       ch.last_tok_chunks, ch.pair_family, ch.pair_np, ch.l5_jobs5, ch.xcd_lanes, ch.xcd_lanes5, ch.dec_actor, mfma_dec ? ch.np : 0,
-      ch.fp32_dec, ch.split_dec, ch.want_mw, ch.mw_blocks, ch.cls_side && !ch.want_mw, ch.tgt_wait_first, ch.split_dec ? ch.dec_head_ra : 0, 0};
+      ch.fp32_dec, ch.split_dec, ch.want_mw, ch.mw_blocks, ch.cls_side && !ch.want_mw, ch.tgt_wait_first, ch.split_dec ? ch.dec_head_ra : 0, ch.dec_chain_g};
   std::vector<long long> rec(head, head + PRED_CHOICE_HEADER);
   for (const PredTokRun &r : ch.tok_runs) rec.insert(rec.end(), {r.t0, r.n, r.kind, r.layerwise, r.small, r.merged});
   for (size_t i = 0; i < rec.size() && (int)i < cap; ++i) out[i] = rec[i];
@@ -512,6 +512,26 @@
   return MIND_OK;
 }
 
+static int dec_chain_run(mind_ctx *c, int G, int Bn, const float *x, const int *d_cls_row, float *Cout, float *cls, hipStream_t st) {
+  if (!dc_valid_g(G) || Bn <= 0) return fail(c, MIND_EINVAL, "decoder chain: %d workgroups per scene, %d scenes", G, Bn);
+  int rc;
+  if ((rc = ensure(c, c->dec_chain, (size_t)std::max(Bn, c->n_cu / 8) * DC_SCENE_FLOATS * sizeof(float)))) return rc;
+  float *buf = (float *)c->dec_chain.p;
+  const size_t lds = mind_dec_scene_lds_bytes();
+#define DEC_CHAIN(GV)                                                                                                  \
+  do {                                                                                                                 \
+    hipLaunchKernelGGL(k_dec_chain1<GV>, dim3(Bn * GV), dim3(DT), lds, st, x, d_cls_row, buf, c->W.dec);                \
+    hipLaunchKernelGGL(k_dec_chain2<GV>, dim3(Bn * GV), dim3(DT), lds, st, buf, c->W.dec);                              \
+    hipLaunchKernelGGL(k_dec_chain3<GV>, dim3(Bn * GV), dim3(DT), lds, st, buf, c->W.dec);                              \
+  } while (0)
+  if (G == 32) DEC_CHAIN(32);
+  else if (G == 16) DEC_CHAIN(16);
+  else DEC_CHAIN(8);
+#undef DEC_CHAIN
+  hipLaunchKernelGGL(k_dec_chain4, dim3(Bn), dim3(DT), lds, st, (const float *)buf, Cout, cls, c->W.dec);
+  return MIND_OK;
+}
+
 static int pred_decoder(PredCall &p) {
   mind_ctx *c = p.c;
   const PredChoice &ch = p.ch;
@@ -550,8 +570,10 @@
       HIPCHK(c, hipMemsetAsync(c->dec_bars.p, 0, c->dec_bars.cap, st));
     }
   }
-  if (mw)
-    hipLaunchKernelGGL(k_dec_scene_mw, dim3(ch.mw_blocks), dim3(DT), mind_dec_scene_lds_bytes(), st, x, d_cls_row, (float *)c->cmode.p, out->cls, c->W.dec, Bn,
+  if (ch.dec_chain_g) {
+    if ((rc = dec_chain_run(c, ch.dec_chain_g, Bn, x, d_cls_row, (float *)c->cmode.p, out->cls, st))) return rc;
+  } else if (mw)
+    hipLaunchKernelGGL(k_dec_scene_mw,dim3(ch.mw_blocks), dim3(DT), mind_dec_scene_lds_bytes(), st, x, d_cls_row, (float *)c->cmode.p, out->cls, c->W.dec, Bn,
                        (float *)c->dec_xbuf.p, (unsigned *)c->dec_bars.p, c->dec_abort.as<unsigned>());
   else if (ch.cls_side) {
     hipLaunchKernelGGL(k_dec_scene_c, dim3(Bn), dim3(DT), mind_dec_scene_lds_bytes(), st, x, d_cls_row, (float *)c->cmode.p, c->W.dec);
```

New measurement: 1928 (median of 6 runs). 2.7% higher.
